# pashtari/factorizer

Measured on AMD Instinct MI355X. Metric: volumes/sec fwd+bwd, Swin Factorizer 128^3, higher is better.
Workload: dtype f32

## Files before the change

factorizer_amd/_native.py:

```python
from __future__ import annotations

import ctypes
import os
import threading

import torch

_HERE = os.path.dirname(os.path.abspath(__file__))
LIB_PATH = os.environ.get("FZ_LIB_PATH") or os.path.join(_HERE, "libfactorizer_hip.so")

FZ_OK = 0
FZ_E_UNSUPPORTED = -2
ABI_VERSION = 7
SOLVER_ID = {"mu": 0, "hals": 1, "cd": 2, "smu": 3}
STORE_F32, STORE_BF16 = 0, 1
PRODUCTS_DEFAULT, PRODUCTS_SPLIT_BF16, PRODUCTS_FP32_MFMA = 0, 1, 2
_products = threading.local()


def products() -> int:
    return getattr(_products, "value", PRODUCTS_DEFAULT)


class use_products:
# ... 89 lines not shown
            h.fz_abi_version.restype = ctypes.c_int
            abi = int(h.fz_abi_version())
        except AttributeError:
            abi = None
        if abi != ABI_VERSION:
            raise NativeError(f"{LIB_PATH} has ABI revision {abi}, this binding is written against {ABI_VERSION} "
                              "(include/factorizer_hip.h: FZ_ABI_VERSION): rebuild with `python -m factorizer_amd.build`")
        for name, (args, res) in _SIGS.items():
            fn = getattr(h, name)
            fn.argtypes = args
            fn.restype = res
        _lib = h
    return _lib


def launch_count() -> int:
    return int(lib().fz_launch_count())


def check(rc: int, what: str):
    if rc != FZ_OK:
        msg = lib().fz_last_error_string().decode()
        raise NativeError(f"{what} failed (code {rc}): {msg}")


def stream_ptr(t: torch.Tensor) -> int:
    return torch.cuda.current_stream(t.device).cuda_stream


def ptr(t):
    return None if t is None else t.data_ptr()


def shifts_array(shifts):
    flat = [int(v) for s in shifts for v in s]
    return (_i * len(flat))(*flat)


_fp = _c.POINTER(_c.c_float)


class GemmDesc(_c.Structure):
    _fields_ = [("x", _vp * 4), ("nsrc", _i), ("src_mode", _i), ("c0", _i), ("Cin", _i), ("Vin", _i64),
                ("Di", _i), ("Hi", _i), ("Wi", _i), ("w", _vp), ("w_t", _i), ("ldw", _i), ("M", _i), ("K", _i),
                ("bias", _vp), ("ln", _i), ("ln_g", _vp), ("ln_b", _vp), ("ln_eps", _f), ("stats_out", _vp),
                ("bact", _i), ("bmul", _vp), ("bmul_kind", _i), ("eact", _i), ("res", _vp), ("emul", _vp), ("emul_kind", _i), ("y", _vp),
                ("Ncol", _i64), ("Ho", _i), ("Wo", _i), ("B", _i), ("loader", _i), ("epilogue", _i), ("lnb_x", _vp), ("lnb_stats", _vp), ("lnb_g", _vp),
                ("lnb_gadd", _vp), ("lnb_part", _vp), ("act_dtype", _i), ("products", _i), ("tune", _i)]


class MlpDesc(_c.Structure):
    _fields_ = [("mode", _i), ("inp", _vp), ("w1", _vp), ("w2", _vp), ("b1", _vp), ("b2", _vp), ("ln_g", _vp),
                ("ln_b", _vp), ("ln_eps", _f), ("stats", _vp), ("z1", _vp), ("gz1", _vp), ("x1", _vp), ("out", _vp),
                ("part", _vp), ("B", _i), ("C", _i), ("H", _i), ("V", _i64), ("act_dtype", _i), ("wpart", _vp),
                ("gw1", _vp), ("gb1", _vp), ("gw2", _vp), ("gb2", _vp), ("gln", _vp), ("glp", _vp), ("products", _i),
                ("pre_in", _vp), ("pre_w", _vp), ("pre_b", _vp), ("pre_res", _vp), ("pre_out", _vp),
                ("post_w", _vp), ("post_b", _vp), ("post_out", _vp), ("post_m", _i)]


class MlpDropout(_c.Structure):
    _fields_ = [("m0", _vp), ("m1", _vp), ("m2", _vp), ("s0", _f), ("s1", _f), ("s2", _f)]


class BlockPrologue(_c.Structure):
    _fields_ = [("ln_g", _vp), ("ln_b", _vp), ("ln_eps", _f), ("w", _vp), ("t", _vp), ("stats", _vp)]


class GemmDwDesc(_c.Structure):
    _fields_ = [("g", _vp), ("q", _vp), ("w", _vp), ("ln", _i), ("stats", _vp), ("ln_g", _vp), ("ln_b", _vp), ("gadd", _vp),
                ("y", _vp), ("gln", _vp), ("wpart", _vp), ("gw", _vp), ("gb", _vp), ("B", _i), ("C", _i), ("V", _i64),
                ("act_dtype", _i), ("ldgw", _i), ("ldw", _i), ("drop_m", _vp), ("drop_s", _f)]


class WgradDesc(_c.Structure):
    _fields_ = [("p", _vp), ("M", _i), ("pmul", _vp), ("pmul_kind", _i), ("q", _vp * 4), ("nsrc", _i),
                ("src_mode", _i), ("c0", _i), ("Cin", _i), ("K", _i), ("Vq", _i64), ("D", _i), ("H", _i),
                ("W", _i), ("N", _i64), ("Ho", _i), ("Wo", _i), ("stats", _vp), ("qact", _i), ("ln_g", _vp),
                ("ln_b", _vp), ("gw", _vp), ("gbias", _vp), ("accumulate", _i), ("B", _i), ("loader", _i),
                ("act_dtype", _i), ("products", _i)]


class VolGeom(_c.Structure):
    _fields_ = [("nd", _i), ("size", _i * 3), ("start", _i * 3), ("end", _i * 3), ("pad", _i * 3), ("out", _i * 3)]


class RespaceGeom(_c.Structure):
    _fields_ = [("nd", _i), ("src_size", _i * 3), ("src_axis", _i * 3), ("flip", _i * 3), ("res_size", _i * 3), ("pad", _i * 3),
                ("out", _i * 3), ("orig_size", _i * 3), ("box_start", _i * 3), ("scale", _c.c_double * 3),
                ("inv_scale", _c.c_double * 3)]


_SIGS.update({
    "fz_gcorr_supported": ([_i] * 5, _i),
    "fz_gcorr": ([_vp] * 5 + [_i] * 11 + [_f, _vp], _i),
    "fz_gcorr_wgrad_workspace_bytes": ([_i] * 10, _i64),
    "fz_gcorr_wgrad": ([_vp] * 4 + [_i] * 11 + [_vp], _i),
    "fz_gcorr_act": ([_vp] * 5 + [_i] * 11 + [_f, _i, _vp], _i),
    "fz_gcorr_wgrad_act": ([_vp] * 4 + [_i] * 12 + [_vp], _i),
    "fz_gcorr_mu_bwd": ([_vp] * 8 + [_i] * 11 + [_f, _i, _vp], _i),
    "fz_gnmf_supported": ([_i, _i64, _i, _i, _i], _i),
    "fz_gnmf_workspace_bytes": ([_i64, _i, _i64, _i, _i, _i], _i64),
    "fz_gnmf_launches": ([_i, _i, _i], _i),
    "fz_gnmf_fwd": ([_vp] * 6 + [_i64, _i, _i64, _i, _i, _i, _f, _vp, _vp], _i),
    "fz_gnmf_bwd": ([_vp] * 7 + [_i64, _i, _i64, _i, _i, _i, _i, _f, _vp, _vp], _i),
    "fz_gnmfx_supported": ([_i, _i64, _i, _i, _i], _i),
    "fz_gnmfx_workspace_bytes": ([_i64, _i, _i64, _i, _i, _i], _i64),
    "fz_gnmfx_launches": ([_i, _i64, _i, _i, _i, _i], _i),
    "fz_gnmfx_fwd": ([_vp] * 6 + [_i64, _i, _i64, _i, _i, _i, _f, _vp, _vp], _i),
    "fz_gnmfx_bwd": ([_vp] * 7 + [_i64, _i, _i64, _i, _i, _i, _i, _f, _vp, _vp], _i),
    "fz_nmf_cf_supported": ([_i] * 11, _i),
    "fz_nmf_cf_fwd": ([_vp] * 4 + [_i] * 5 + [_c.POINTER(_i)] + [_i] * 5 + [_f, _i, _vp], _i),
    "fz_nmf_cf_bwd": ([_vp] * 5 + [_i] * 5 + [_c.POINTER(_i)] + [_i] * 7 + [_f, _i, _vp], _i),
    "fz_nmf_cf_factors_supported": ([_i] * 12 + [_c.POINTER(_i)], _i),
    "fz_nmf_cf_fwd_store_factors": ([_vp] * 5 + [_i] * 5 + [_c.POINTER(_i)] + [_i] * 3 + [_f, _i, _vp], _i),
    "fz_nmf_cf_fwd_from_factors": ([_vp] * 6 + [_i] * 5 + [_c.POINTER(_i)] * 2 + [_i] * 4 + [_f, _i, _vp], _i),
    "fz_nmf_cf_bwd_factors_supported": ([_i] * 14 + [_c.POINTER(_i)], _i),
    "fz_nmf_cf_bwd_store_factors": ([_vp] * 5 + [_i] * 5 + [_c.POINTER(_i)] + [_i] * 3 + [_f, _i, _vp], _i),
    "fz_nmf_cf_bwd_from_factors": ([_vp] * 6 + [_i] * 5 + [_c.POINTER(_i)] * 2 + [_i] * 3 + [_f, _i, _vp], _i),
    "fz_nmf_pcf_supported": ([_i] * 11, _i),
    "fz_nmf_pcf_fwd": ([_vp] * 4 + [_i] * 8 + [_c.POINTER(_i)] + [_i] * 5 + [_f, _i, _vp], _i),
    "fz_nmf_pcf_bwd": ([_vp] * 5 + [_i] * 8 + [_c.POINTER(_i)] + [_i] * 7 + [_f, _i, _vp], _i),
    "fz_nmf_pcf_bwd_prefers_separate": ([_i] * 4, _i),
    "fz_act_add": ([_vp, _vp, _i64, _i, _vp], _i),
    "fz_mlp_pre_supported": ([_i, _i, _i64, _i], _i),
    "fz_mlp_drop_supported": ([_i, _i, _i64, _i], _i),
    "fz_mlp_chain_drop": ([_c.POINTER(MlpDesc), _c.POINTER(MlpDropout), _vp], _i),
    "fz_conv3_prologue_supported": ([_i] * 4, _i),
    "fz_conv3_fwd2": ([_vp] * 4 + [_i] * 8 + [_c.POINTER(BlockPrologue), _vp], _i),
    "fz_upcat2": ([_vp, _vp, _vp, _i, _vp, _vp, _vp] + [_i] * 7 + [_c.POINTER(BlockPrologue), _vp], _i),
    "fz_gemm": ([_c.POINTER(GemmDesc), _vp], _i),
    "fz_gemm_plan": ([_c.POINTER(GemmDesc), _c.c_char_p, _i], _i),
    "fz_gemm_bx_enable": ([_i], _i),
    "fz_gemm_lnbwd_partials": ([_c.POINTER(GemmDesc)], _i64),
    "fz_reduce_rows": ([_vp, _i64, _i, _vp, _vp, _vp], _i),
    "fz_adamw_step": ([_vp, _vp, _vp, _vp, _i64, _f, _f, _f, _f, _f, _i, _f, _vp], _i),
    "fz_sw_gather": ([_vp, _vp] + [_i] * 10 + [_vp], _i),
    "fz_sw_accumulate": ([_vp] * 6 + [_f] + [_i] * 10 + [_vp], _i),
    "fz_sw_finalize": ([_vp, _vp, _i, _i64, _vp], _i),
    "fz_sw_gather2": ([_vp, _vp] + [_i] * 11 + [_vp], _i),
    "fz_sw_accumulate2": ([_vp] * 6 + [_f] + [_i] * 11 + [_vp], _i),
    "fz_sw_finalize2": ([_vp, _vp, _vp, _i, _i64, _i, _vp], _i),
    "fz_mlp_supported": ([_i, _i, _i64], _i),
    "fz_mlp_partials": ([_i, _i64], _i64),
    "fz_mlp_wgrad_rows": ([_i, _i64], _i),
    "fz_gemm_dw_rows": ([_i, _i64], _i),
    "fz_gemm_dw_workspace_bytes": ([_i, _i64], _i64),
    "fz_gemm_dw": ([_c.POINTER(GemmDwDesc), _vp], _i),
    "fz_mlp_wgrad_workspace_bytes": ([_i, _i64], _i64),
    "fz_mlp_chain": ([_c.POINTER(MlpDesc), _vp], _i),
    "fz_head_bwd_rows": ([], _i),
    "fz_head_bwd_workspace_bytes": ([], _i64),
    "fz_head_bwd": ([_vp, _vp, _vp, _vp, _vp, _i, _i, _i, _i64, _i, _vp], _i),
    "fz_head_fwd": ([_vp, _vp, _vp, _vp, _i, _i, _i, _i64, _i, _vp], _i),
    "fz_upcat_supported": ([_i] * 5, _i),
    "fz_upcat_compose": ([_vp, _vp, _i, _vp, _vp, _vp, _vp, _vp, _i, _i, _i, _vp], _i),
    "fz_upcat_wgrads": ([_vp, _vp, _vp, _i, _vp, _vp, _vp, _vp, _i, _vp, _i, _i, _i, _vp], _i),
    "fz_upcat": ([_vp, _vp, _vp, _i, _vp, _vp, _vp] + [_i] * 7 + [_vp], _i),
    "fz_upcat_bwd_supported": ([_i] * 6, _i),
    "fz_upcat_bwd_workspace_bytes": ([_i] * 4, _i64),
    "fz_upcat_bwd": ([_vp, _vp, _vp, _vp, _i, _vp, _vp, _vp, _vp, _vp, _i, _vp, _vp] + [_i] * 7 + [_vp], _i),
    "fz_wgrad": ([_c.POINTER(WgradDesc), _vp, _vp], _i),
    "fz_wgrad_group": ([_c.POINTER(_c.POINTER(WgradDesc)), _c.POINTER(_vp), _i, _vp], _i),
    "fz_wgrad_workspace_bytes": ([_c.POINTER(WgradDesc)], _i64),
    "fz_conv3_fwd": ([_vp] * 4 + [_i] * 8 + [_vp], _i),
    "fz_conv3_wgrad_chunks": ([_i] * 4, _i),
    "fz_conv3_wgrad_partials": ([_vp] * 4 + [_i] * 8 + [_vp], _i),
    "fz_chunk_reduce": ([_vp, _i, _i64, _vp, _i, _vp], _i),
    "fz_chunk_reduce_ld": ([_vp, _i, _i64, _i64, _vp, _i, _vp], _i),
    "fz_finish_defer": ([_i], _i),
    "fz_finish_pending": ([], _i),
    "fz_finish_flush": ([_vp], _i),
    "fz_finish_flush_all": ([_vp], _i),
    "fz_dice_bce_chunks": ([_i64], _i),
    "fz_dice_bce_sums": ([_vp, _vp, _vp, _i, _i64, _vp], _i),
    "fz_dice_bce_grad": ([_vp, _vp, _vp, _vp, _i, _i64, _f, _f, _vp, _vp], _i),
    "fz_dice_ce_sums": ([_vp, _vp, _vp, _i, _i, _i64, _vp], _i),
    "fz_dice_ce_grad": ([_vp, _vp, _vp, _vp, _i, _i, _i64, _f, _f, _vp, _vp], _i),
    "fz_dice_ce_finish": ([_vp, _i, _i, _i64, _f, _vp, _vp, _vp], _i),
    "fz_dice_bce_ds_sums": ([_vp, _vp, _vp, _i] + [_i] * 6 + [_i, _vp], _i),
    "fz_dice_bce_ds_grad": ([_vp, _vp, _vp, _vp, _i] + [_i] * 6 + [_i, _f, _f, _vp, _vp], _i),
    "fz_dice_ce_ds_sums": ([_vp, _vp, _vp, _i, _i] + [_i] * 6 + [_i, _vp], _i),
    "fz_dice_ce_ds_grad": ([_vp, _vp, _vp, _vp, _i, _i] + [_i] * 6 + [_i, _f, _f, _vp, _vp], _i),
    "fz_rowsum_chunks": ([_i64], _i),
    "fz_rowsum": ([_vp, _vp, _vp, _i, _i, _i64, _i, _vp], _i),
    "fz_ln_fwd": ([_vp] * 5 + [_i, _i, _i64, _f, _i, _vp], _i),
    "fz_ln_bwd": ([_vp] * 8 + [_i, _i, _i64, _i, _vp], _i),
    "fz_ln_bwd_workspace_bytes": ([_i], _i64),
    "fz_ln_bwd_workspace_bytes2": ([_i, _i, _i64], _i64),
    "fz_dropout_bits_words": ([_i, _i, _i64], _i64),
    "fz_dropout_keep_bits": ([_vp, _i, _i, _i, _i64, _f, _vp, _vp], _i),
    "fz_dropout_apply": ([_i, _vp, _f, _vp, _vp, _vp, _i, _i, _i64, _i, _vp], _i),
    "fz_seg_counts_chunks": ([_i64], _i),
    "fz_seg_counts_workspace_bytes": ([_i, _i64], _i64),
    "fz_seg_counts": ([_vp, _i, _vp, _i, _f, _vp, _vp, _vp, _i, _i64, _vp], _i),
    "fz_mask_edges": ([_vp, _vp, _vp, _i, _i, _i, _i, _i, _vp], _i),
    "fz_edge_min_dist2_splits": ([_i64, _i64], _i),
    "fz_edge_min_dist2_workspace_bytes": ([_i64, _i64], _i64),
    "fz_edge_min_dist2": ([_vp, _i64, _vp, _i64, _f, _f, _f, _vp, _vp, _vp], _i),
    "fz_aug_record_floats": ([], _i),
    "fz_aug_resample": ([_vp, _vp, _i, _i, _vp, _vp, _i, _vp, _vp, _vp] + [_i] * 6 + [_vp], _i),
    "fz_aug_smooth": ([_vp, _vp, _i, _i, _vp, _vp] + [_i] * 6 + [_vp], _i),
    "fz_aug_noise_field": ([_vp, _vp, _i, _i, _i64, _vp], _i),
    "fz_aug_source_words": ([], _i),
    "fz_aug_crop_resample": ([_vp, _vp, _i, _i, _vp, _i, _vp, _vp, _vp] + [_i] * 6 + [_vp], _i),
    "fz_vol_kind_ok": ([_i, _i], _i),
    "fz_vol_bbox": ([_vp, _i, _i, _i, _i, _i, _i, _vp, _vp], _i),
    "fz_vol_workspace_bytes": ([_i, _c.POINTER(VolGeom)], _i64),
    "fz_vol_stats": ([_vp, _i, _i, _c.POINTER(VolGeom), _i, _i, _vp, _vp], _i),
    "fz_vol_write": ([_vp, _i, _vp, _i, _i, _vp, _i, _i, _c.POINTER(_i), _c.POINTER(_i), _i, _vp, _c.POINTER(VolGeom), _i, _i,
                      _vp, _vp, _vp, _vp], _i),
    "fz_vol_restore": ([_c.POINTER(_vp), _i, _i, _i, _c.POINTER(VolGeom), _f, _c.POINTER(_c.c_ubyte), _vp, _vp], _i),
    "fz_vol_respace": ([_vp, _i, _vp, _i, _vp, _i, _vp, _c.POINTER(RespaceGeom), _i, _vp], _i),
    "fz_vol_unspace": ([_c.POINTER(_vp), _i, _i, _i, _c.POINTER(RespaceGeom), _i, _i, _f, _vp, _vp], _i),
    "fz_inorm_one_pass_max": ([], _i),
    "fz_inorm_chunks": ([_i64], _i),
    "fz_inorm_workspace_bytes": ([_i64, _i64], _i64),
    "fz_inorm_fwd": ([_vp] * 5 + [_i64, _i, _i64, _c.c_double, _i, _vp, _vp], _i),
    "fz_inorm_bwd": ([_vp] * 7 + [_i64, _i, _i64, _i, _vp, _vp], _i),
})
SEG_F32, SEG_BF16, SEG_U8 = 0, 1, 2
VOL_F32, VOL_BF16, VOL_U8, VOL_I16 = 0, 1, 2, 3
VOL_IMAGE_IN, VOL_IMAGE_OUT, VOL_LABEL_IN, VOL_LOGITS = 0, 1, 2, 3
RESPACE_BILINEAR, RESPACE_NEAREST = 0, 1
DROP_RES, DROP_GELU, DROP_GELU_BWD = 0, 1, 2
```

factorizer_amd/blocks.py:

```python
from __future__ import annotations

import os

import torch
from torch import nn

from . import functional as Fn
from . import pointwise as PW
from .layers import MLP, LayerNorm, Linear
from .matricize import Matricize, SWMatricize
from .nmf import NMF, MatrixFactorization, RandomInit
from .utils import partialize


def _env_int(name, default):
    v = os.environ.get(name)
    if v is None:
        return default
    try:
        return int(v, 0)
    except ValueError:
        raise ValueError(f"{name}={v!r}: expected an integer") from None


_UP_FUSED = _env_int("FZ_UP_FUSED", 1) != 0
_UP_FUSED_MIN = _env_int("FZ_UP_FUSED_MIN", 1 << 18)


class FactMixer(nn.Module):

    def __init__(self, in_channels, out_channels, spatial_size,
                 reshape=(Matricize, {"num_heads": 1, "grid_size": 1}), act=nn.ReLU, factorize=NMF,
                 dropout=0.0, **kwargs):
        super().__init__()
        self.in_proj = Linear(in_channels, out_channels, bias=False)
        self.reshape = partialize(reshape)((None, out_channels, *spatial_size))
        self.act = partialize(act)()
        self.reshaped_size = self.reshape.output_size[2:]
        self.factorize = partialize(factorize)(self.reshaped_size, **kwargs)
        self.out_proj = Linear(in_channels, out_channels, True)
        self.dropout = nn.Dropout(dropout)

    def forward(self, x):
        out = self.in_proj(x)
        out = self.reshape(out)
        out = self.act(out)
        out = self.factorize(out)
        out = self.reshape.inverse_forward(out)
        out = self.out_proj(out)
        if self.dropout.p > 0:
            out = self.dropout(out)
        return out


class FactorizerBlock(nn.Module):

    def __init__(self, channels, spatial_size, norm=LayerNorm, dropout=0.0, mlp_ratio=2, **kwargs):
        super().__init__()
        self.norm1 = partialize(norm)(channels)
        self.fact = FactMixer(channels, channels, spatial_size, dropout=dropout, **kwargs)
        self.norm2 = partialize(norm)(channels)
        self.mlp = MLP(channels, ratio=mlp_ratio, dropout=dropout)

    def _fusable(self, x) -> bool:
        f, m = self.fact, self.mlp
        if not (x.is_cuda and x.numel() and x.dtype in (torch.float32, torch.bfloat16) and PW._vox(x) % 4 == 0
                and x.shape[1] % 2 == 0):
            return False
        if any(p.dtype != torch.float32 for p in self.parameters()):
            return False
        if not (isinstance(self.norm1, LayerNorm) and isinstance(self.norm2, LayerNorm)
                and self.norm1.norm.elementwise_affine and self.norm2.norm.elementwise_affine
                and self.norm1.norm.bias is not None and self.norm2.norm.bias is not None):
            return False
        if not (isinstance(f.act, nn.ReLU) and isinstance(f.in_proj, Linear) and isinstance(f.out_proj, Linear)):
            return False
        blk = m.block
        if not (len(blk) == 5 and isinstance(blk[1], nn.GELU) and blk[1].approximate == "none"
                and blk[0].linear.weight.shape[0] % 2 == 0):
            return False
        drops = (f.dropout, blk[2], blk[4])
        if self.training and any(d.p > 0 for d in drops):
            return all(type(d) is nn.Dropout and 0 <= d.p < 1 for d in drops)
        return True

    def _dropout_ps(self):
        ps = (float(self.fact.dropout.p), float(self.mlp.block[2].p), float(self.mlp.block[4].p))
        return ps if self.training and any(p > 0 for p in ps) else None

    def _modular_native_cfg(self, x) -> bool:
        f = self.fact
        mf = f.factorize
        if not (isinstance(f.reshape, SWMatricize) and isinstance(mf, MatrixFactorization)):
            return False
        t_like = x.new_empty((1, *f.reshape.output_size[1:]))
        return mf._native_solver(t_like) is not None and not mf._wide and len(f.reshape.geometry.spatial) <= 3

    def _core_cfg(self):
        f = self.fact
        mf = f.factorize
        if not (isinstance(f.reshape, SWMatricize) and isinstance(mf, MatrixFactorization)):
            return None
        sid = getattr(mf.solver, "native_id", None)
        if sid is None or not isinstance(mf.init, RandomInit) or mf.solver.factor != (0, 1) or mf.verbose:
            return None
        G = min(max(mf.num_grad_steps, 0), mf.num_iters)
        geo = f.reshape.geometry
        if tuple(mf.size) != (8, geo.P) or not Fn.nmf_core_supported(geo, mf.rank, mf.num_iters, G):
            return None
        return G, sid

    def prologue_params(self, like):
        f, blk = self.fact, self.mlp.block
        n1 = self.norm1.norm
        if not (like.is_cuda and like.shape[1] == 32 and self._fusable(like) and self._core_cfg() is not None
                and f.in_proj.linear.bias is None and blk[0].linear.bias is not None and blk[3].linear.bias is not None
                and f.out_proj.linear.bias is not None and f.in_proj.linear.weight.dtype == torch.float32
                and n1.weight is not None and n1.bias is not None
                and not (self.norm1._forward_hooks or f.in_proj._forward_hooks or f._forward_hooks)):
            return None
        return n1.weight, n1.bias, n1.eps, f.in_proj.linear.weight

    def forward(self, x):
        if self._fusable(x):
            f, blk = self.fact, self.mlp.block
            n1, n2 = self.norm1.norm, self.norm2.norm
            core = self._core_cfg()
            mf = f.factorize
            nat = core is not None or self._modular_native_cfg(x)
            drop = self._dropout_ps()
            one_node = nat and f.in_proj.linear.bias is None and blk[0].linear.bias is not None \
                and blk[3].linear.bias is not None and f.out_proj.linear.bias is not None
            if one_node:
                if core is not None:
                    G, sid = core
                else:
                    G, sid = min(max(mf.num_grad_steps, 0), mf.num_iters), mf.solver.native_id
                cfg = dict(geo=f.reshape.geometry, T=mf.num_iters, G=G, solver=sid, nmf_eps=mf.solver.eps,
                           eps1=n1.eps, eps2=n2.eps, core=core is not None)
                if drop is not None:
                    cfg["drop"] = drop
                args = (x, n1.weight, n1.bias, f.in_proj.linear.weight, mf.init.u0, mf.init.v0,
                        f.out_proj.linear.weight, f.out_proj.linear.bias, n2.weight, n2.bias,
                        blk[0].linear.weight, blk[0].linear.bias, blk[3].linear.weight, blk[3].linear.bias, cfg)
                pre = PW.BlockPrologue.take(x) if core is not None else None
                t_pre, st_pre = pre if pre is not None else (None, None)
                slot = PW.head_fusion_slot()
                if slot is not None and slot.block is self and core is not None and drop is None:
                    hw, hb = slot.head_params
                    C, Hd = x.shape[1], blk[0].linear.weight.shape[0]
                    if PW.block_head_fusable(C, Hd, x[0, 0].numel(), hw, x):
                        y, raw = PW.FactorizerBlockFn.apply(*args, hw, hb, t_pre, st_pre)
                        slot.logits = PW.HeadOfBlockFn.apply(y, hw, hb, raw)
                        return y
                return PW.FactorizerBlockFn.apply(*args, None, None, t_pre, st_pre)
            if drop is None:
                return self._per_layer(x)
        x = x + self.fact(self.norm1(x))
        x = x + self.mlp(self.norm2(x))
        return x

    def _per_layer(self, x):
        f, blk = self.fact, self.mlp.block
        n1, n2 = self.norm1.norm, self.norm2.norm
        t = PW.ln_linear(x, n1.weight, n1.bias, n1.eps, f.in_proj.linear.weight, f.in_proj.linear.bias, "relu")
        a = f.reshape.inverse_forward(f.factorize(f.reshape(t)))
        x = PW.act_linear_res(a, f.out_proj.linear.weight, f.out_proj.linear.bias, x, "none")
        z = PW.ln_linear(x, n2.weight, n2.bias, n2.eps, blk[0].linear.weight, blk[0].linear.bias, "none")
        return PW.act_linear_res(z, blk[3].linear.weight, blk[3].linear.bias, x, "gelu")


class FactorizerStage(nn.Module):

    def __init__(self, in_channels, out_channels, spatial_size, depth=1,
                 adapter=(Linear, {"bias": False}), pos_embed=nn.Identity, dropout=0.0, **subblocks):
        super().__init__()
        if in_channels != out_channels:
            self.adapter = partialize(adapter)(in_channels, out_channels)
        self.pos_embed = partialize(pos_embed)(out_channels, spatial_size)
        if len(list(self.pos_embed.parameters())) > 0:
            self.pos_drop = nn.Dropout(dropout)
        self.blocks = nn.ModuleList()
        for _ in range(depth):
            self.blocks.append(FactorizerBlock(out_channels, spatial_size, **subblocks))

    def forward_pair(self, skip, up):
        if hasattr(self, "adapter") and isinstance(self.adapter, Linear):
            out = PW.cat_linear(skip, up, self.adapter.linear.weight, self.adapter.linear.bias)
            return self._after_adapter(out)
        return self.forward(torch.cat([skip, up], dim=1))

    def forward_up_pair(self, skip, deep, upsample):
        from . import convs as _convs
        ok = (hasattr(self, "adapter") and isinstance(self.adapter, Linear) and type(upsample) is _convs.ConvTranspose3d
              and upsample.native_ok(deep) and skip.is_cuda and skip.dtype == deep.dtype and skip.dim() == 5
              and skip.shape[1] % 16 == 0 and upsample.out_channels % 16 == 0 and deep.shape[1] % 16 == 0
              and self.adapter.linear.weight.dtype == torch.float32
              and tuple(skip.shape[2:]) == tuple(2 * d for d in deep.shape[2:])
              and self.adapter.linear.weight.shape[1] == skip.shape[1] + upsample.out_channels
              and _UP_FUSED and skip.shape[0] * skip[0, 0].numel() >= _UP_FUSED_MIN
              and not (upsample._forward_hooks or upsample._forward_pre_hooks
                       or self.adapter._forward_hooks or self.adapter._forward_pre_hooks
                       or self.adapter.linear._forward_hooks or self.adapter.linear._forward_pre_hooks))
        if not ok:
            return None
        pro = self._first_block_prologue(skip) if PW.upcat_prologue_ok(skip, deep, upsample.weight, self.adapter.linear.weight) else None
        if pro is not None:
            out, t, st = PW.up_cat_linear(skip, deep, upsample.weight, upsample.bias, self.adapter.linear.weight, self.adapter.linear.bias, pro)
            with PW.BlockPrologue(out, t, st):
                return self._after_adapter(out)
        out = PW.up_cat_linear(skip, deep, upsample.weight, upsample.bias, self.adapter.linear.weight, self.adapter.linear.bias)
        return self._after_adapter(out)

    def _first_block_prologue(self, like):
        if not isinstance(self.pos_embed, nn.Identity) or (hasattr(self, "pos_drop") and self.pos_drop.p > 0) or len(self.blocks) == 0:
            return None
        blk = self.blocks[0]
        if type(blk).__name__ != "FactorizerBlock" or blk._forward_hooks or blk._forward_pre_hooks:
            return None
        return blk.prologue_params(like)

    def forward(self, x):
        out = self.adapter(x) if hasattr(self, "adapter") else x
        return self._after_adapter(out)

    def _after_adapter(self, out):
        if not isinstance(self.pos_embed, nn.Identity):
            out = self.pos_embed(out)
        if hasattr(self, "pos_drop") and self.pos_drop.p > 0:
            out = self.pos_drop(out)
        for blk in self.blocks:
            out = blk(out)
        return out
```

factorizer_amd/csrc/headbwd.hip:

```cpp
#include "gemm_common.h"

namespace fz {

constexpr int kHeadRow = 4 * 33;

template <int M, typename AT>
__global__ __launch_bounds__(256, 2) void head_bwd_kernel(const AT* __restrict__ gy, const AT* __restrict__ x,
                                                          const float* __restrict__ w, AT* __restrict__ gx,
                                                          float* __restrict__ part, int B, int64_t V, int Mr) {
  __shared__ float red[4][kHeadRow];
  __shared__ float sW[M * 32];
  const int lane = threadIdx.x & 63, wave = threadIdx.x >> 6;
  for (int i = threadIdx.x; i < M * 32; i += 256) sW[i] = i < Mr * 32 ? w[i] : 0.f;
  __syncthreads();
  float gw[M][32];
  float gb[M];
#pragma unroll
  for (int m = 0; m < M; ++m) {
    gb[m] = 0.f;
#pragma unroll
    for (int c = 0; c < 32; ++c) gw[m][c] = 0.f;
  }
  const unsigned quads = (unsigned)(V / 4), total = quads * (unsigned)B;
  for (unsigned i = blockIdx.x * 256u + threadIdx.x; i < total; i += gridDim.x * 256u) {
    asm volatile("" ::: "memory");
    const int b = (int)(i / quads);
    const int64_t v = (int64_t)(i - (unsigned)b * quads) * 4;
    float g4[M][4];
#pragma unroll
    for (int m = 0; m < M; ++m) {
      vload<4>(gy + ((int64_t)b * Mr + (m < Mr ? m : Mr - 1)) * V + v, g4[m]);
#pragma unroll
      for (int e = 0; e < 4; ++e) {
        g4[m][e] = m < Mr ? g4[m][e] : 0.f;
        gb[m] += g4[m][e];
      }
    }
    const AT* xb = x + (int64_t)b * 32 * V + v;
    AT* ob = gx + (int64_t)b * 32 * V + v;
    constexpr int CB = 4;
#pragma unroll
    for (int c0 = 0; c0 < 32; c0 += CB) {
      float xv[CB][4];
#pragma unroll
      for (int u = 0; u < CB; ++u) vload<4>(xb + (int64_t)(c0 + u) * V, xv[u]);
      __builtin_amdgcn_sched_barrier(0);
#pragma unroll
      for (int u = 0; u < CB; ++u) {
        const int c = c0 + u;
        float o[4];
#pragma unroll
        for (int e = 0; e < 4; ++e) {
          float t = sW[c] * g4[0][e];
#pragma unroll
          for (int m = 1; m < M; ++m) t += sW[m * 32 + c] * g4[m][e];
          o[e] = t;
        }
        vstore<4>(ob + (int64_t)c * V, o);
#pragma unroll
        for (int m = 0; m < M; ++m)
          gw[m][c] += (g4[m][0] * xv[u][0] + g4[m][1] * xv[u][1]) + (g4[m][2] * xv[u][2] + g4[m][3] * xv[u][3]);
      }
    }
  }
#pragma unroll
  for (int m = 0; m < M; ++m) {
#pragma unroll
    for (int c0 = 0; c0 < 32; c0 += 8) {
      float t[8];
#pragma unroll
      for (int u = 0; u < 8; ++u) t[u] = gw[m][c0 + u];
      wave_sum8(t, lane);
      if (lane == 0) {
#pragma unroll
        for (int u = 0; u < 8; ++u) red[wave][m * 32 + c0 + u] = t[u];
      }
    }
    const float s = wave_sum(gb[m]);
    if (lane == 0) red[wave][128 + m] = s;
  }
  __syncthreads();
  for (int e = threadIdx.x; e < kHeadRow; e += 256) {
    const bool used = (e < 128) ? (e >> 5) < Mr : (e - 128) < Mr;
    part[(int64_t)blockIdx.x * kHeadRow + e] = used ? (red[0][e] + red[1][e]) + (red[2][e] + red[3][e]) : 0.f;
  }
}

template <int M, typename AT>
__global__ __launch_bounds__(256) void head_fwd_kernel(const AT* __restrict__ x, const float* __restrict__ w,
                                                       const float* __restrict__ bias, AT* __restrict__ y, int B, int64_t V, int Mr) {
  __shared__ float sW[M * 32];
  __shared__ float sB[M];
  for (int i = threadIdx.x; i < M * 32; i += 256) sW[i] = i < Mr * 32 ? w[i] : 0.f;
  if (threadIdx.x < M) sB[threadIdx.x] = (bias != nullptr && (int)threadIdx.x < Mr) ? bias[threadIdx.x] : 0.f;
  __syncthreads();
  const unsigned quads = (unsigned)(V / 4), stride = gridDim.x * 256u;
  unsigned first = blockIdx.x * 256u + threadIdx.x;
  int b = (int)(first / quads);
  unsigned qd = first - (unsigned)b * quads;
  for (; b < B; qd += stride) {
    while (qd >= quads) { qd -= quads; ++b; }
    if (b >= B) break;
    asm volatile("" ::: "memory");
    const int64_t v = (int64_t)qd * 4;
    const AT* xb = x + (int64_t)b * 32 * V + v;
    float acc[M][4];
#pragma unroll
    for (int m = 0; m < M; ++m)
#pragma unroll
      for (int e = 0; e < 4; ++e) acc[m][e] = sB[m];
    constexpr int CB = 8;
#pragma unroll
    for (int c0 = 0; c0 < 32; c0 += CB) {
      float xv[CB][4];
#pragma unroll
      for (int u = 0; u < CB; ++u) vload<4>(xb + (int64_t)(c0 + u) * V, xv[u]);
#pragma unroll
      for (int u = 0; u < CB; ++u)
#pragma unroll
        for (int m = 0; m < M; ++m) {
          const float wv = sW[m * 32 + c0 + u];
#pragma unroll
          for (int e = 0; e < 4; ++e) acc[m][e] += wv * xv[u][e];
        }
    }
#pragma unroll
    for (int m = 0; m < M; ++m)
      if (m < Mr) vstore<4>(y + ((int64_t)b * Mr + m) * V + v, acc[m]);
  }
}

}

using namespace fz;

extern "C" int fz_head_bwd_rows(void) { return 512; }
extern "C" int64_t fz_head_bwd_workspace_bytes(void) { return (int64_t)fz_head_bwd_rows() * kHeadRow * (int64_t)sizeof(float); }

template <typename AT>
static int head_bwd_launch(const void* gy, const void* x, const float* w, void* gx, float* part, int B, int M, int64_t V,
                           hipStream_t st) {
  const unsigned grid = (unsigned)fz_head_bwd_rows();
#define FZ_HEAD(MM) hipLaunchKernelGGL((head_bwd_kernel<MM, AT>), dim3(grid), dim3(256), 0, st, (const AT*)gy, (const AT*)x, w, (AT*)gx, part, B, V, M)
  if (M <= 2) FZ_HEAD(2); else FZ_HEAD(4);
#undef FZ_HEAD
  FZ_LAUNCH_CHECK();
  return FZ_OK;
}

extern "C" int fz_head_bwd(const void* gy, const void* x, const float* w, void* gx, float* part, int B, int M, int C, int64_t V,
                           int act_dtype, fz_stream_t stream) {
  if (!gy || !x || !w || !gx || !part) return fail(FZ_E_ARG, "fz_head_bwd: null pointer");
  if (C != 32 || M < 1 || M > 4 || V < 4 || V % 4 != 0) return fail(FZ_E_UNSUPPORTED, "fz_head_bwd: needs C == 32, 1 <= M <= 4, V % 4 == 0");
  if ((int64_t)B * (V / 4) >= ((int64_t)1 << 31)) return fail(FZ_E_UNSUPPORTED, "fz_head_bwd: 2^31 or more voxel quads");
  if (B <= 0) return B == 0 ? FZ_OK : fail(FZ_E_SHAPE, "fz_head_bwd: negative batch");
  if (act_dtype == FZ_STORE_F32) return head_bwd_launch<float>(gy, x, w, gx, part, B, M, V, (hipStream_t)stream);
  if (act_dtype == FZ_STORE_BF16) return head_bwd_launch<bf16>(gy, x, w, gx, part, B, M, V, (hipStream_t)stream);
  return fail(FZ_E_ARG, "fz_head_bwd: act_dtype must be FZ_STORE_F32 or FZ_STORE_BF16");
}

template <typename AT>
static int head_fwd_launch(const void* x, const float* w, const float* bias, void* y, int B, int M, int64_t V, hipStream_t st) {
  const unsigned grid = 512u;
  if (gemm_plan_only()) return gemm_plan_form("head m%d grid=%ux1", M <= 2 ? 2 : 4, grid);
#define FZ_HEADF(MM) hipLaunchKernelGGL((head_fwd_kernel<MM, AT>), dim3(grid), dim3(256), 0, st, (const AT*)x, w, bias, (AT*)y, B, V, M)
  if (M <= 2) FZ_HEADF(2); else FZ_HEADF(4);
#undef FZ_HEADF
  FZ_LAUNCH_CHECK();
  return FZ_OK;
}

extern "C" int fz_head_fwd(const void* x, const float* w, const float* bias, void* y, int B, int M, int C, int64_t V, int act_dtype,
                           fz_stream_t stream) {
  if (!x || !w || !y) return fail(FZ_E_ARG, "fz_head_fwd: null pointer");
  if (C != 32 || M < 1 || M > 4 || V < 4 || V % 4 != 0) return fail(FZ_E_UNSUPPORTED, "fz_head_fwd: needs C == 32, 1 <= M <= 4, V % 4 == 0");
  if (V / 4 >= ((int64_t)1 << 31) || (int64_t)B * (V / 4) >= ((int64_t)1 << 31)) return fail(FZ_E_UNSUPPORTED, "fz_head_fwd: 2^31 or more voxel quads");
  if (B <= 0) return B == 0 ? FZ_OK : fail(FZ_E_SHAPE, "fz_head_fwd: negative batch");
  if (act_dtype == FZ_STORE_F32) return head_fwd_launch<float>(x, w, bias, y, B, M, V, (hipStream_t)stream);
  if (act_dtype == FZ_STORE_BF16) return head_fwd_launch<bf16>(x, w, bias, y, B, M, V, (hipStream_t)stream);
  return fail(FZ_E_ARG, "fz_head_fwd: act_dtype must be FZ_STORE_F32 or FZ_STORE_BF16");
}
```

factorizer_amd/csrc/mlp_chain.h:

```cpp
#pragma once
#include "gemm_bx.h"
#include "gemm_shared.h"

namespace fz {

template <typename AT>
struct ChainArgsT {
  const float* wB;
  int wB_t, ldwB;
  const float* biasB;
  AT* side;
  const AT* preA;
  const float* preW;
  const float* preB;
  const AT* preRes;
  AT* preOut;
  const float* postW;
  const float* postB;
  AT* postOut;
  int postM;
  int stagger;
};

__device__ __forceinline__ void chain_stagger(int stagger) {
  const int n = stagger * (int)(blockIdx.x >> 8);
  for (int i = 0; i < n; ++i) __builtin_amdgcn_s_sleep(127);
}

constexpr int chain64_lds_floats(bool p512, bool pre) {
  return 2 * (p512 ? 12288 : 8192) + (pre ? 6144 + 64 : 0) + 128 + 64 + (p512 ? 2 : 1) * 512;
}
constexpr int chain_wg_lds_floats(bool bx, bool wgb) {
  return 2 * (bx ? 3072 : 2048) + 32 + 256 + 4 * (wgb ? 3072 : 48 * kTS);
}

template <typename... KArgs, typename... Args>
static int launch_lds(void (*kern)(KArgs...), dim3 grid, dim3 block, int lds_floats, hipStream_t st, Args... args) {
  const int lds = lds_floats * (int)sizeof(float);
  FZ_HIP_OK(hipFuncSetAttribute(reinterpret_cast<const void*>(kern), hipFuncAttributeMaxDynamicSharedMemorySize, lds));
  hipLaunchKernelGGL(kern, grid, block, lds, st, args...);
  FZ_LAUNCH_CHECK();
  return FZ_OK;
}

static int knob_chain64_p512() { return knob_pos(FZ_KNOB("FZ_CHAIN64_P512"), 1) == 1; }
static int knob_chain_fwd_bx() { const auto& k = FZ_KNOB("FZ_CHAIN_FWD_BX"); return k.set ? k.val : 1; }
static int knob_mlp_wgs(int dflt) { return knob_pos(FZ_KNOB("FZ_MLP_WGS"), dflt); }

template <typename AT>
int chain32_launch(const fz_mlp_desc* d, const fz_mlp_dropout* drop, const GemmArgsT<AT>& a, const ChainArgsT<AT>& c, fz_stream_t stream);
template <typename AT>
int chain64_launch(const fz_mlp_desc* d, const GemmArgsT<AT>& a, const ChainArgsT<AT>& c, fz_stream_t stream);
template <typename AT>
int chain_wg_launch(const fz_mlp_desc* d, const GemmArgsT<AT>& a, const ChainArgsT<AT>& c, fz_stream_t stream);

}
```

factorizer_amd/csrc/mlp_chain.hip:

```cpp
#include "mlp_chain.h"

using namespace fz;

static int mlp_nacc() { return 2; }

extern "C" int64_t fz_mlp_partials(int B, int64_t V) {
  const int64_t tw = 128 * mlp_nacc();
  return ((V + tw - 1) / tw) * (int64_t)B;
}

extern "C" int fz_mlp_pre_supported(int C, int H, int64_t V, int products) {
  if (!(V > 0 && (V % 4) == 0 && V <= ((int64_t)1 << 27) && products_split(products))) return 0;
  if (C == 32 && H == 64) return knob_chain_fwd_bx() ? 1 : 0;
  if (C == 64 && H == 128) return (((V + 255) / 256) % 2 == 0 && knob_chain64_p512()) ? 1 : 0;
  return 0;
}

extern "C" int fz_mlp_supported(int C, int H, int64_t V) {
  const bool shape = (C == 32 && (H == 64 || H == 128)) || (C == 64 && H == 128);
  return (shape && V > 0 && (V % 4) == 0 && V <= ((int64_t)1 << 27)) ? 1 : 0;
}

extern "C" int fz_mlp_drop_supported(int C, int H, int64_t V, int products) {
  return (C == 32 && H == 64 && fz_mlp_supported(C, H, V) && fz_mlp_pre_supported(C, H, V, products) && products_split(products)
          && knob_chain_fwd_bx()) ? 1 : 0;
}

template <typename AT>
static void forward_args(const fz_mlp_desc* d, int ldw, int ldwB, GemmArgsT<AT>& a, ChainArgsT<AT>& c) {
  a.w = d->w1; a.w_t = 0; a.ldw = ldw;
  a.bias = d->b1; a.ln = 1; a.ln_g = d->ln_g; a.ln_b = d->ln_b; a.ln_eps = d->ln_eps; a.stats_out = d->stats;
  a.res = (const AT*)d->in; a.y = (AT*)d->out;
  c.wB = d->w2; c.wB_t = 0; c.ldwB = ldwB; c.biasB = d->b2; c.side = (AT*)d->z1;
  if (d->pre_in) {
    c.preA = (const AT*)d->pre_in; c.preW = d->pre_w; c.preB = d->pre_b; c.preRes = (const AT*)d->pre_res; c.preOut = (AT*)d->pre_out;
    if (d->C == 64) a.res = (const AT*)d->pre_out;
    else { c.postW = d->post_w; c.postB = d->post_b; c.postOut = (AT*)d->post_out; c.postM = d->post_m; }
  }
}
template <typename AT>
static void backward_args(const fz_mlp_desc* d, int ldw, int ldwB, AT* side, GemmArgsT<AT>& a, ChainArgsT<AT>& c) {
  a.w = d->w2; a.w_t = 1; a.ldw = ldw;
  a.emul = (const AT*)d->z1; a.y = (AT*)d->out;
  a.lnb_x = (const AT*)d->x1; a.lnb_stats = d->stats; a.lnb_g = d->ln_g; a.lnb_gadd = (const AT*)d->in; a.lnb_part = d->part;
  c.wB = d->w1; c.wB_t = 1; c.ldwB = ldwB; c.side = side;
}

static int mlp_check(const fz_mlp_desc* d, const fz_mlp_dropout* dd, bool drop) {
  if (!fz_mlp_supported(d->C, d->H, d->V)) return fail(FZ_E_UNSUPPORTED, "fz_mlp_chain: needs (C, H) in {(32, 64), (32, 128), (64, 128)}, V % 4 == 0");
  if (drop) {
    if (!fz_mlp_drop_supported(d->C, d->H, d->V, d->products) || d->mode != 0 || !d->pre_in)
      return fail(FZ_E_UNSUPPORTED, "fz_mlp_chain: dropout needs (C, H) = (32, 64), split-bf16 products, mode 0 with pre_in (fz_mlp_drop_supported)");
    if (!drop_scale_ok(dd->m0, dd->s0) || !drop_scale_ok(dd->m1, dd->s1) || !drop_scale_ok(dd->m2, dd->s2))
      return fail(FZ_E_ARG, "fz_mlp_chain: a dropout scale 1 / (1 - p) must be >= 1 and finite");
  }
  if (d->C == 64 && d->mode == 2) return fail(FZ_E_UNSUPPORTED, "fz_mlp_chain: the fused weight gradients need C == 32, H == 64");
  if (d->B < 0) return fail(FZ_E_SHAPE, "fz_mlp_chain: negative batch");
  const bool pre = d->pre_in != nullptr;
  if (pre && (d->mode != 0 || !d->pre_w || !d->pre_res || !d->pre_out))
    return fail(FZ_E_ARG, "fz_mlp_chain: pre_in needs mode 0, pre_w, pre_res, pre_out (see fz_mlp_pre_supported)");
  if (pre && !fz_mlp_pre_supported(d->C, d->H, d->V, d->products))
    return fail(FZ_E_UNSUPPORTED, "fz_mlp_chain: the fused out-projection runs on split-bf16 products only (fz_mlp_pre_supported)");
  if (d->post_out && (!pre || d->C != 32 || !d->post_w || d->post_m < 1 || d->post_m > 4))
    return fail(FZ_E_ARG, "fz_mlp_chain: post_out needs pre_in, C == 32, post_w and 1 <= post_m <= 4");
  if ((!d->in && !pre) || !d->w1 || !d->w2 || !d->out || !d->z1 || !d->stats)
    return fail(FZ_E_ARG, "fz_mlp_chain: null pointer");
  if (d->mode == 0 && (!d->ln_g || !d->ln_b)) return fail(FZ_E_ARG, "fz_mlp_chain: forward needs the LayerNorm affine");
  if (d->mode == 1 && (!d->gz1 || !d->x1 || !d->ln_g || !d->part)) return fail(FZ_E_ARG, "fz_mlp_chain: backward needs gz1, x1, gamma, part");
  if (d->mode == 2 && (!d->x1 || !d->ln_g || !d->ln_b || !d->gln || !d->wpart || !d->gw1 || !d->gb1 || !d->gw2 || !d->gb2))
    return fail(FZ_E_ARG, "fz_mlp_chain: backward with weight gradients needs x1, gamma, beta, gln, wpart, gw1, gb1, gw2, gb2");
  if (d->mode == 2 && d->H == 128 && !d->glp) return fail(FZ_E_ARG, "fz_mlp_chain: the fused weight gradients at H == 128 need the glp buffer");
  if (d->mode < 0 || d->mode > 2) return fail(FZ_E_ARG, "fz_mlp_chain: bad mode");
  return FZ_OK;
}

template <typename AT>
static int mlp_launch(const fz_mlp_desc* d, const fz_mlp_dropout* dd, fz_stream_t stream) {
  const bool drop = dd && (dd->m0 || dd->m1 || dd->m2);
  const int rc = mlp_check(d, dd, drop);
  if (rc != FZ_OK) return rc;
  if (d->B == 0) {
    if (d->mode == 2) {
      hipStream_t s0 = (hipStream_t)stream;
      FZ_HIP_OK(hipMemsetAsync(d->gw1, 0, sizeof(float) * d->H * 32, s0));
      FZ_HIP_OK(hipMemsetAsync(d->gw2, 0, sizeof(float) * d->H * 32, s0));
      FZ_HIP_OK(hipMemsetAsync(d->gb1, 0, sizeof(float) * d->H, s0));
      FZ_HIP_OK(hipMemsetAsync(d->gb2, 0, sizeof(float) * 32, s0));
      FZ_HIP_OK(hipMemsetAsync(d->gln, 0, sizeof(float) * 64, s0));
    }
    return FZ_OK;
  }
  GemmArgsT<AT> a = {};
  ChainArgsT<AT> c = {};
  a.x[0] = (const AT*)d->in; a.nsrc = 1; a.c0 = d->C; a.Cin = d->C; a.Vin = d->V; a.M = d->H; a.K = d->C; a.Ncol = d->V; a.B = d->B;
  if (d->mode == 0) forward_args(d, d->C, d->H, a, c);
  else backward_args(d, d->H, d->C, d->mode == 1 ? (AT*)d->gz1 : (AT*)nullptr, a, c);
  if (d->C == 64) return chain64_launch(d, a, c, stream);
  if (d->mode == 2) return chain_wg_launch(d, a, c, stream);
  return chain32_launch(d, drop ? dd : nullptr, a, c, stream);
}

extern "C" int fz_mlp_chain(const fz_mlp_desc* d, fz_stream_t stream) {
  if (!d) return fail(FZ_E_ARG, "fz_mlp_chain: null descriptor");
  if (d->act_dtype == FZ_STORE_F32) return mlp_launch<float>(d, nullptr, stream);
  if (d->act_dtype == FZ_STORE_BF16) return mlp_launch<bf16>(d, nullptr, stream);
  return fail(FZ_E_ARG, "fz_mlp_chain: act_dtype must be FZ_STORE_F32 or FZ_STORE_BF16");
}

extern "C" int fz_mlp_chain_drop(const fz_mlp_desc* d, const fz_mlp_dropout* drop, fz_stream_t stream) {
  if (!d || !drop) return fail(FZ_E_ARG, "fz_mlp_chain_drop: null descriptor");
  if (d->act_dtype == FZ_STORE_F32) return mlp_launch<float>(d, drop, stream);
  if (d->act_dtype == FZ_STORE_BF16) return mlp_launch<bf16>(d, drop, stream);
  return fail(FZ_E_ARG, "fz_mlp_chain_drop: act_dtype must be FZ_STORE_F32 or FZ_STORE_BF16");
}
```

factorizer_amd/csrc/mlp_chain_wg.hip:

```cpp
#include "mlp_chain.h"
#include "finish.h"

namespace fz {


__device__ __forceinline__ void gelu_both(float x, float& g, float& dg) {
  const float ax = fabsf(x) * 0.70710678118654752f;
  const float E = __expf(-0.5f * x * x);
  const float t = __builtin_amdgcn_rcpf(1.0f + 0.3275911f * ax);
  const float poly = t * (0.254829592f + t * (-0.284496736f + t * (1.421413741f + t * (-1.453152027f + t * 1.061405429f))));
  const float r = 1.0f - poly * E;
  const float cdf = 0.5f * (1.0f + __builtin_copysignf(r, x));
  g = x * cdf;
  dg = cdf + x * (0.3989422804014327f * E);
}

typedef float f32x2 __attribute__((ext_vector_type(2)));
template <bool SEL = false>
__device__ __forceinline__ void gelu_both2(const float (&x)[2], float (&g)[2], float (&dg)[2]) {
  const f32x2 xv = {x[0], x[1]};
  const f32x2 ax = f32x2{fabsf(x[0]), fabsf(x[1])} * 0.70710678118654752f;
  const f32x2 xx = (xv * -0.5f) * xv;
  const f32x2 E = {__expf(xx[0]), __expf(xx[1])};
  const f32x2 den = ax * 0.3275911f + 1.0f;
  const f32x2 t = {__builtin_amdgcn_rcpf(den[0]), __builtin_amdgcn_rcpf(den[1])};
  const f32x2 poly = t * (t * (t * (t * (t * 1.061405429f + -1.453152027f) + 1.421413741f) + -0.284496736f) + 0.254829592f);
  const f32x2 r = 1.0f - poly * E;
  f32x2 rs;
  if constexpr (SEL) rs = f32x2{x[0] < 0.f ? -r[0] : r[0], x[1] < 0.f ? -r[1] : r[1]};
  else rs = f32x2{__builtin_copysignf(r[0], x[0]), __builtin_copysignf(r[1], x[1])};
  const f32x2 cdf = (rs + 1.0f) * 0.5f;
  const f32x2 gv = xv * cdf;
  const f32x2 dv = cdf + xv * (E * 0.3989422804014327f);
  g[0] = gv[0]; g[1] = gv[1];
  dg[0] = dv[0]; dg[1] = dv[1];
}

typedef __bf16 wg2 __attribute__((ext_vector_type(2)));
__device__ __forceinline__ void wg_split2(float x0, float x1, unsigned& hi, unsigned& lo) {
  fx2 v = {x0, x1};
  const wg2 a = __builtin_convertvector(v, wg2);
  v = v - __builtin_convertvector(a, fx2);
  const wg2 b = __builtin_convertvector(v, wg2);
  hi = __builtin_bit_cast(unsigned, a);
  lo = __builtin_bit_cast(unsigned, b);
}
__device__ __forceinline__ float2 wg_join2(unsigned hi, unsigned lo) {
  return make_float2(__uint_as_float(hi << 16) + __uint_as_float(lo << 16),
                     __uint_as_float(hi & 0xffff0000u) + __uint_as_float(lo & 0xffff0000u));
}
__device__ __forceinline__ float wg_sum8(const bx8& hi, const bx8& lo, float acc) {
  const wg2 one = {(__bf16)1.0f, (__bf16)1.0f};
  struct Q { wg2 p[4]; };
  const Q h = __builtin_bit_cast(Q, hi), l = __builtin_bit_cast(Q, lo);
#pragma unroll
  for (int i = 0; i < 4; ++i) {
    acc = __builtin_amdgcn_fdot2_f32_bf16(l.p[i], one, acc, false);
    acc = __builtin_amdgcn_fdot2_f32_bf16(h.p[i], one, acc, false);
  }
  return acc;
}
__device__ __forceinline__ void wg_mfma3(f32x4& acc, const bx8& ah, const bx8& al, const bx8& bh, const bx8& bl) {
  acc = __builtin_amdgcn_mfma_f32_16x16x32_bf16(al, bh, acc, 0, 0, 0);
  acc = __builtin_amdgcn_mfma_f32_16x16x32_bf16(ah, bl, acc, 0, 0, 0);
  acc = __builtin_amdgcn_mfma_f32_16x16x32_bf16(ah, bh, acc, 0, 0, 0);
}

template <typename AT, int HALVES = 1, int HALF = 0, bool BX = false, bool WGB = false>
__global__ __launch_bounds__(256, 2) void gemm_chain_bwd_wg_kernel(GemmArgsT<AT> p, ChainArgsT<AT> c, int ntiles, float* wpart,
                                                                   float* glp) {
  static_assert(!WGB || (BX && HALVES == 1), "WGB: the one-launch split-bf16 form");
  constexpr int NACC = 2, HB = 2, HID = 64 * HALVES, N1 = BX ? 3072 : 16 * HB * 64;
  constexpr int NTA = BxTerms<AT>::A, NTB = bx_terms_b<AT>(BXPRO_GELU);
  constexpr bool WGF = WGB && sizeof(AT) == 4;
  constexpr int half = HALF;
  constexpr int hoff = 64 * HALF;
  constexpr bool last = HALF == HALVES - 1;
  constexpr int kWave = WGB ? 3072 : 48 * kTS;
  extern __shared__ __attribute__((aligned(16))) float fz_lds_cw[];
  float* As1 = fz_lds_cw;
  float* As2 = As1 + N1;
  float* tB = As2 + N1;
  float* red = tB + 32;
  float* R = red + 256;
  static_assert(2 * N1 + 32 + 256 + 4 * kWave == chain_wg_lds_floats(BX, WGB), "the launcher's dynamic LDS ends where this carve-up does");
  const int lane = threadIdx.x & 63, wave = threadIdx.x >> 6;
  const int j = lane & 31, h = lane >> 5;
  const int l16 = lane & 15, k4 = lane >> 4;
  float* Bf = R + wave * kWave;
  float* T = Bf + 32 * kTS;
  char* const PL = reinterpret_cast<char*>(Bf);
  constexpr int kGL = 4096, kTH = 8192, kTL = 10240;
  unsigned wop[4], wac[4], rd[2];
  if constexpr (WGB) {
    const unsigned ob = (unsigned)h * 128u + ((((unsigned)j >> 2) ^ (unsigned)h) << 4) + ((unsigned)j & 3u) * 4u;
    const unsigned ab = (unsigned)h * 512u + ((((unsigned)j >> 2) ^ (4u * (unsigned)h)) << 4) + ((unsigned)j & 3u) * 4u;
#pragma unroll
    for (int q = 0; q < 4; ++q) { wop[q] = ob ^ ((unsigned)q << 5); wac[q] = ab ^ ((unsigned)q << 4); }
    rd[0] = (unsigned)l16 * 128u + ((((unsigned)k4) ^ ((unsigned)l16 & 7u)) << 4);
    rd[1] = rd[0] ^ 64u;
  }
  const int tiles_per_sample = (int)((p.Ncol + 128 * NACC - 1) / (128 * NACC));
  chain_stagger(c.stagger);

  if constexpr (BX) {
    for (int it = threadIdx.x; it < 512; it += 256) {
      float wv[8];
      const int l = it & 63;
      __bf16* dst;
      if (it < 256) {
        const int rb = (it >> 6) & 1, g = it >> 7;
#pragma unroll
        for (int e = 0; e < 8; ++e) wv[e] = weight_at(p, hoff + rb * 32 + (l & 31), 2 * (8 * g + e) + (l >> 5));
        dst = reinterpret_cast<__bf16*>(As1) + ((g * HB + rb) * NTA * 64 + l) * 8;
      } else {
        const int g = (it - 256) >> 6;
#pragma unroll
        for (int e = 0; e < 8; ++e) {
          const int s2 = 8 * g + e, r = s2 & 15, rb = s2 >> 4;
          const int k = hoff + rb * 32 + (r & 3) + 8 * (r >> 2) + 4 * (l >> 5), m = l & 31;
          wv[e] = c.wB_t ? c.wB[(int64_t)k * c.ldwB + m] : c.wB[(int64_t)m * c.ldwB + k];
        }
        dst = reinterpret_cast<__bf16*>(As2) + (g * NTA * 64 + l) * 8;
      }
      bx8 t3[NTA];
      bx_split<NTA>(wv, t3);
#pragma unroll
      for (int i = 0; i < NTA; ++i) *reinterpret_cast<bx8*>(dst + i * 64 * 8) = t3[i];
    }
  } else {
  for (int base = threadIdx.x; base < 2 * N1; base += 256 * 8) {
    float tmp[8];
#pragma unroll
    for (int uu = 0; uu < 8; ++uu) {
      const int idx = base + uu * 256;
      float wv;
      if (idx < N1) {
        const int l = idx & 63, rb = (idx >> 6) % HB, a = idx / (64 * HB);
        wv = weight_at(p, hoff + rb * 32 + (l & 31), 2 * a + (l >> 5));
      } else {
        const int i2 = idx - N1;
        const int l = i2 & 63, s2 = i2 >> 6;
        const int r = s2 & 15, rb = s2 >> 4;
        const int k = hoff + rb * 32 + (r & 3) + 8 * (r >> 2) + 4 * (l >> 5), m = l & 31;
        wv = c.wB_t ? c.wB[(int64_t)k * c.ldwB + m] : c.wB[(int64_t)m * c.ldwB + k];
      }
      tmp[uu] = wv;
    }
#pragma unroll
    for (int uu = 0; uu < 8; ++uu) {
      const int idx = base + uu * 256;
      if (idx < N1) As1[idx] = tmp[uu]; else As2[idx - N1] = tmp[uu];
    }
  }
  }
  if (threadIdx.x < 32) tB[threadIdx.x] = p.lnb_g[threadIdx.x];

  f32x4 dW2[2][4], dW1[4][2];
#pragma unroll
  for (int a = 0; a < 2; ++a)
#pragma unroll
    for (int b4 = 0; b4 < 4; ++b4)
#pragma unroll
      for (int v = 0; v < 4; ++v) { dW2[a][b4][v] = 0.f; dW1[b4][a][v] = 0.f; }
  float db2[2] = {0.f, 0.f}, db1[4] = {0.f, 0.f, 0.f, 0.f};
  float gln = 0.f;

  int tile = blockIdx.x;
  float bv[16][NACC];
  auto fetch_tile = [&](int t) {
    const int bt = t / tiles_per_sample;
    const int64_t ct = ((int64_t)(t % tiles_per_sample) * 4 + wave) * (32 * NACC) + NACC * j;
    const unsigned lo = (unsigned)h * (unsigned)p.Ncol + (unsigned)(ct < p.Ncol ? ct : 0);
    const AT* xb = p.x[0] + (int64_t)bt * 32 * p.Ncol;
#pragma unroll
    for (int s = 0; s < 16; ++s) vload<NACC>(xb + (int64_t)(2 * s) * p.Ncol + lo, bv[s]);
  };
  fetch_tile(tile);
  __syncthreads();

  for (; tile < ntiles; tile += gridDim.x) {
    asm volatile("" ::: "memory");
    const int b = tile / tiles_per_sample;
    const int64_t col_off = ((int64_t)(tile % tiles_per_sample) * 4 + wave) * (32 * NACC) + NACC * j;
    const bool col_ok = col_off < p.Ncol;
    const int64_t nc = col_ok ? col_off : 0;
    const unsigned lane_row = (unsigned)(4 * h) * (unsigned)p.Ncol + (unsigned)nc;
    const unsigned lane_par = (unsigned)h * (unsigned)p.Ncol + (unsigned)nc;
    const int64_t sample = (int64_t)b * 32 * p.Ncol;

    constexpr bool ZSEL = HALVES == 2;
    auto zs = [&](float v) { return (ZSEL && !col_ok) ? 0.f : v; };
    if (!ZSEL && __builtin_amdgcn_ballot_w64(!col_ok) != 0) {
#pragma unroll
      for (int s = 0; s < 16; ++s) { bv[s][0] = col_ok ? bv[s][0] : 0.f; bv[s][1] = col_ok ? bv[s][1] : 0.f; }
    }
    if constexpr (!WGB) {
#pragma unroll
    for (int s = 0; s < 16; ++s)
      *reinterpret_cast<float2*>(Bf + (2 * s + h) * kTS + 2 * j) = make_float2(zs(bv[s][0]), zs(bv[s][1]));
    }

    float e[2][8][NACC];
    auto fetch_z1 = [&](int g8, float (&dst)[8][NACC]) {
#pragma unroll
      for (int i = 0; i < 8; ++i) {
        const int rr = g8 * 8 + i, rb = rr >> 4, r = rr & 15;
        const int rbase = hoff + rb * 32 + (r & 3) + 8 * (r >> 2);
        vload<NACC>(p.emul + ((int64_t)b * HID + rbase) * p.Ncol + lane_row, dst[i]);
      }
    };
    float xv[2][8][NACC];
    auto fetch_x1 = [&](int hf, float (&dst)[8][NACC]) {
#pragma unroll
      for (int s8 = 0; s8 < 8; ++s8) vload<NACC>(p.lnb_x + sample + (int64_t)(2 * (hf * 8 + s8)) * p.Ncol + lane_par, dst[s8]);
    };
    const float* sp = p.lnb_stats + (int64_t)b * 2 * p.Ncol;
    float mu[NACC], rs[NACC];
    vload<NACC>(sp + nc, mu);
    vload<NACC>(sp + p.Ncol + nc, rs);
    fetch_z1(0, e[0]);

    f32x16 acc1[HB][NACC];
#pragma unroll
    for (int rb = 0; rb < HB; ++rb)
#pragma unroll
      for (int q = 0; q < NACC; ++q)
#pragma unroll
        for (int r = 0; r < 16; ++r) acc1[rb][q][r] = 0.f;
    if constexpr (BX) {
#pragma unroll
      for (int g = 0; g < 2; ++g) {
        bx8 bop[NACC][NTB];
#pragma unroll
        for (int q = 0; q < NACC; ++q) {
          float x8[8];
#pragma unroll
          for (int e = 0; e < 8; ++e) x8[e] = bv[8 * g + e][q];
          bx_split<NTB>(x8, bop[q]);
        }
        if constexpr (WGB) {
          static_assert(!WGB || NTB >= 2, "two levels of the column operand");
#pragma unroll
          for (int e = 0; e < 8; ++e) {
            const int s = 8 * g + e;
            const wg2 ph = {bop[0][0][e], bop[1][0][e]};
            const wg2 pl = {bop[0][NTB >= 2 ? 1 : 0][e], bop[1][NTB >= 2 ? 1 : 0][e]};
            *reinterpret_cast<wg2*>(PL + wop[s & 3] + s * 256) = ph;
            *reinterpret_cast<wg2*>(PL + kGL + wop[s & 3] + s * 256) = pl;
          }
        }
#pragma unroll
        for (int rb = 0; rb < HB; ++rb) {
          bx8 aop[NTA];
#pragma unroll
          for (int i = 0; i < NTA; ++i)
            aop[i] = *reinterpret_cast<const bx8*>(reinterpret_cast<const __bf16*>(As1) + (((g * HB + rb) * NTA + i) * 64 + lane) * 8);
#pragma unroll
          for (int q = 0; q < NACC; ++q) bx_mfma<NTA, NTB>(acc1[rb][q], aop, bop[q]);
        }
        __builtin_amdgcn_sched_barrier(0);
      }
    } else {
#pragma unroll
    for (int s = 0; s < 16; ++s)
#pragma unroll
      for (int rb = 0; rb < HB; ++rb) {
        const float av = As1[(s * HB + rb) * 64 + lane];
#pragma unroll
        for (int q = 0; q < NACC; ++q) acc1[rb][q] = __builtin_amdgcn_mfma_f32_32x32x2f32(av, bv[s][q], acc1[rb][q], 0, 0, 0);
        if (rb == HB - 1 && (s & 1) == 1) __builtin_amdgcn_sched_barrier(0);
      }
    }

#pragma unroll
    for (int g8 = 0; g8 < 4; ++g8) {
      asm volatile("" ::: "memory");
      if (g8 < 3) fetch_z1(g8 + 1, e[(g8 + 1) & 1]);
      else { fetch_x1(0, xv[0]); fetch_x1(1, xv[1]); }
#pragma unroll
      for (int i = 0; i < 8; ++i) {
        const int rr = g8 * 8 + i, rb = rr >> 4, r = rr & 15;
        float gl[NACC], dg[NACC];
        gelu_both2<HALVES == 2>(e[g8 & 1][i], gl, dg);
#pragma unroll
        for (int q = 0; q < NACC; ++q) {
          float gz = acc1[rb][q][r] * dg[q];
          asm volatile("" : "+v"(gz));
          acc1[rb][q][r] = gz;
        }
        if constexpr (WGB) {
          unsigned ph, pl;
          wg_split2(gl[0], gl[1], ph, pl);
          *reinterpret_cast<unsigned*>(PL + kTH + wac[i & 3] + (i & 3) * 128 + (i >> 2) * 1024) = ph;
          *reinterpret_cast<unsigned*>(PL + kTL + wac[i & 3] + (i & 3) * 128 + (i >> 2) * 1024) = pl;
        } else {
        const int loc = (i & 3) + 8 * (i >> 2) + 4 * h;
        *reinterpret_cast<float2*>(T + loc * kTS + 2 * j) = make_float2(zs(gl[0]), zs(gl[1]));
        }
      }
      if constexpr (WGB) {
#pragma unroll
        for (int ks = 0; ks < 2; ++ks) {
          const bx8 bh = *reinterpret_cast<const bx8*>(PL + kTH + rd[ks]);
          const bx8 bl = *reinterpret_cast<const bx8*>(PL + kTL + rd[ks]);
          const bx8 a0h = *reinterpret_cast<const bx8*>(PL + rd[ks]);
          const bx8 a0l = *reinterpret_cast<const bx8*>(PL + kGL + rd[ks]);
          const bx8 a1h = *reinterpret_cast<const bx8*>(PL + 2048 + rd[ks]);
          const bx8 a1l = *reinterpret_cast<const bx8*>(PL + kGL + 2048 + rd[ks]);
          wg_mfma3(dW2[0][g8], a0h, a0l, bh, bl);
          wg_mfma3(dW2[1][g8], a1h, a1l, bh, bl);
          if (g8 == 0) {
            db2[0] = wg_sum8(a0h, a0l, db2[0]);
            db2[1] = wg_sum8(a1h, a1l, db2[1]);
            asm volatile("" : "+v"(db2[0]), "+v"(db2[1]));
          }
          __builtin_amdgcn_sched_barrier(0);
        }
      } else {
#pragma unroll
      for (int tc = 0; tc < 2; ++tc) {
        float bq[8], a0[8], a1[8];
#pragma unroll
        for (int u = 0; u < 8; ++u) {
          const int t = tc * 8 + u;
          bq[u] = T[l16 * kTS + 4 * t + k4];
          a0[u] = Bf[l16 * kTS + 4 * t + k4];
          a1[u] = Bf[(16 + l16) * kTS + 4 * t + k4];
        }
#pragma unroll
        for (int u = 0; u < 8; ++u) {
          dW2[0][g8] = __builtin_amdgcn_mfma_f32_16x16x4f32(a0[u], bq[u], dW2[0][g8], 0, 0, 0);
          dW2[1][g8] = __builtin_amdgcn_mfma_f32_16x16x4f32(a1[u], bq[u], dW2[1][g8], 0, 0, 0);
        }
        if (g8 == 0 && (HALVES == 1 || half == 0)) {
          db2[0] += ((a0[0] + a0[1]) + (a0[2] + a0[3])) + ((a0[4] + a0[5]) + (a0[6] + a0[7]));
          db2[1] += ((a1[0] + a1[1]) + (a1[2] + a1[3])) + ((a1[4] + a1[5]) + (a1[6] + a1[7]));
          asm volatile("" : "+v"(db2[0]), "+v"(db2[1]));
        }
        __builtin_amdgcn_sched_barrier(0);
      }
      }
      __builtin_amdgcn_sched_barrier(0);
    }

    float ga[2][8][NACC];
    if (last && BX) {
#pragma unroll
      for (int r = 0; r < 16; ++r) {
        float2 gv;
        if constexpr (WGB)
          gv = wg_join2(*reinterpret_cast<const unsigned*>(PL + wac[r & 3] + (r & 3) * 128 + (r >> 2) * 1024),
                        *reinterpret_cast<const unsigned*>(PL + kGL + wac[r & 3] + (r & 3) * 128 + (r >> 2) * 1024));
        else
          gv = *reinterpret_cast<const float2*>(Bf + ((r & 3) + 8 * (r >> 2) + 4 * h) * kTS + 2 * j);
        ga[r >> 3][r & 7][0] = gv.x; ga[r >> 3][r & 7][1] = gv.y;
      }
      asm volatile("" ::: "memory");
    }

#pragma unroll
    for (int hf = 0; hf < 2; ++hf)
#pragma unroll
      for (int s8 = 0; s8 < 8; ++s8) {
        if constexpr (WGB) {
          const int s = hf * 8 + s8;
          unsigned ph, pl;
          wg_split2((xv[hf][s8][0] - mu[0]) * rs[0], (xv[hf][s8][1] - mu[1]) * rs[1], ph, pl);
          *reinterpret_cast<unsigned*>(PL + wop[s & 3] + s * 256) = ph;
          *reinterpret_cast<unsigned*>(PL + kGL + wop[s & 3] + s * 256) = pl;
        } else
        *reinterpret_cast<float2*>(Bf + (2 * (hf * 8 + s8) + h) * kTS + 2 * j) =
            make_float2(zs((xv[hf][s8][0] - mu[0]) * rs[0]), zs((xv[hf][s8][1] - mu[1]) * rs[1]));
      }

    f32x16 acc2[NACC];
    if constexpr (WGF) {
#pragma unroll
      for (int q = 0; q < NACC; ++q)
#pragma unroll
        for (int r = 0; r < 16; ++r) acc2[q][r] = 0.f;
    }
#pragma unroll
    for (int g8 = 0; g8 < 4; ++g8) {
      asm volatile("" ::: "memory");
#pragma unroll
      for (int i = 0; i < 8; ++i) {
        const int rr = g8 * 8 + i, rb = rr >> 4, r = rr & 15;
        if constexpr (WGF) {
        } else if constexpr (WGB) {
          unsigned ph, pl;
          wg_split2(acc1[rb][0][r], acc1[rb][1][r], ph, pl);
          *reinterpret_cast<unsigned*>(PL + kTH + wac[i & 3] + (i & 3) * 128 + (i >> 2) * 1024) = ph;
          *reinterpret_cast<unsigned*>(PL + kTL + wac[i & 3] + (i & 3) * 128 + (i >> 2) * 1024) = pl;
        } else {
        const int loc = (i & 3) + 8 * (i >> 2) + 4 * h;
        *reinterpret_cast<float2*>(T + loc * kTS + 2 * j) = make_float2(zs(acc1[rb][0][r]), zs(acc1[rb][1][r]));
        }
      }
      if constexpr (WGB) {
        if constexpr (WGF) {
          bx8 aop[NTA];
#pragma unroll
          for (int i = 0; i < NTA; ++i)
            aop[i] = *reinterpret_cast<const bx8*>(reinterpret_cast<const __bf16*>(As2) + ((g8 * NTA + i) * 64 + lane) * 8);
          bx8 bop[NACC][NTB];
#pragma unroll
          for (int q = 0; q < NACC; ++q) {
            float x8[8];
#pragma unroll
            for (int e = 0; e < 8; ++e) x8[e] = acc1[g8 >> 1][q][8 * (g8 & 1) + e];
            bx_split<NTB>(x8, bop[q]);
            bx_mfma<NTA, NTB>(acc2[q], aop, bop[q]);
          }
#pragma unroll
          for (int i = 0; i < 8; ++i) {
            const wg2 ph = {bop[0][0][i], bop[1][0][i]};
            const wg2 pl = {bop[0][1][i], bop[1][1][i]};
            *reinterpret_cast<wg2*>(PL + kTH + wac[i & 3] + (i & 3) * 128 + (i >> 2) * 1024) = ph;
            *reinterpret_cast<wg2*>(PL + kTL + wac[i & 3] + (i & 3) * 128 + (i >> 2) * 1024) = pl;
          }
        }
#pragma unroll
        for (int ks = 0; ks < 2; ++ks) {
          const bx8 ah = *reinterpret_cast<const bx8*>(PL + kTH + rd[ks]);
          const bx8 al = *reinterpret_cast<const bx8*>(PL + kTL + rd[ks]);
          const bx8 b0h = *reinterpret_cast<const bx8*>(PL + rd[ks]);
          const bx8 b0l = *reinterpret_cast<const bx8*>(PL + kGL + rd[ks]);
          const bx8 b1h = *reinterpret_cast<const bx8*>(PL + 2048 + rd[ks]);
          const bx8 b1l = *reinterpret_cast<const bx8*>(PL + kGL + 2048 + rd[ks]);
          wg_mfma3(dW1[g8][0], ah, al, b0h, b0l);
          wg_mfma3(dW1[g8][1], ah, al, b1h, b1l);
          db1[g8] = wg_sum8(ah, al, db1[g8]);
          asm volatile("" : "+v"(db1[g8]));
          __builtin_amdgcn_sched_barrier(0);
        }
      } else {
#pragma unroll
      for (int tc = 0; tc < 2; ++tc) {
        float aq[8], b0[8], b1[8];
#pragma unroll
        for (int u = 0; u < 8; ++u) {
          const int t = tc * 8 + u;
          aq[u] = T[l16 * kTS + 4 * t + k4];
          b0[u] = Bf[l16 * kTS + 4 * t + k4];
          b1[u] = Bf[(16 + l16) * kTS + 4 * t + k4];
        }
#pragma unroll
        for (int u = 0; u < 8; ++u) {
          dW1[g8][0] = __builtin_amdgcn_mfma_f32_16x16x4f32(aq[u], b0[u], dW1[g8][0], 0, 0, 0);
          dW1[g8][1] = __builtin_amdgcn_mfma_f32_16x16x4f32(aq[u], b1[u], dW1[g8][1], 0, 0, 0);
        }
        db1[g8] += ((aq[0] + aq[1]) + (aq[2] + aq[3])) + ((aq[4] + aq[5]) + (aq[6] + aq[7]));
        asm volatile("" : "+v"(db1[g8]));
        __builtin_amdgcn_sched_barrier(0);
      }
      }
      __builtin_amdgcn_sched_barrier(0);
    }


    if (last && !BX) {
#pragma unroll
      for (int r = 0; r < 16; ++r)
        vload<NACC>(p.lnb_gadd + sample + (int64_t)((r & 3) + 8 * (r >> 2)) * p.Ncol + lane_row, ga[r >> 3][r & 7]);
    }

    if constexpr (WGF) {
    } else if (HALVES == 2 && half == 1) {
#pragma unroll
      for (int r = 0; r < 16; ++r) {
        float v[NACC];
        vload<NACC>(glp + sample + (int64_t)((r & 3) + 8 * (r >> 2)) * p.Ncol + lane_row, v);
        acc2[0][r] = v[0]; acc2[1][r] = v[1];
      }
    } else {
#pragma unroll
      for (int q = 0; q < NACC; ++q)
#pragma unroll
        for (int r = 0; r < 16; ++r) acc2[q][r] = 0.f;
    }
    if constexpr (WGF) {
    } else if constexpr (BX) {
#pragma unroll
      for (int g = 0; g < 4; ++g) {
        bx8 aop[NTA];
#pragma unroll
        for (int i = 0; i < NTA; ++i)
          aop[i] = *reinterpret_cast<const bx8*>(reinterpret_cast<const __bf16*>(As2) + ((g * NTA + i) * 64 + lane) * 8);
#pragma unroll
        for (int q = 0; q < NACC; ++q) {
          float x8[8];
#pragma unroll
          for (int e = 0; e < 8; ++e) x8[e] = acc1[g >> 1][q][8 * (g & 1) + e];
          bx8 bop[NTB];
          bx_split<NTB>(x8, bop);
          bx_mfma<NTA, NTB>(acc2[q], aop, bop);
        }
        __builtin_amdgcn_sched_barrier(0);
      }
    } else {
#pragma unroll
    for (int rb = 0; rb < HB; ++rb)
#pragma unroll
      for (int r = 0; r < 16; ++r) {
        const float av = As2[(rb * 16 + r) * 64 + lane];
#pragma unroll
        for (int q = 0; q < NACC; ++q) acc2[q] = __builtin_amdgcn_mfma_f32_32x32x2f32(av, acc1[rb][q][r], acc2[q], 0, 0, 0);
        if ((r & 3) == 3) __builtin_amdgcn_sched_barrier(0);
      }
    }
    fetch_tile(tile + gridDim.x < ntiles ? tile + gridDim.x : tile);

    if (HALVES == 2 && !last) {
      if (col_ok) {
#pragma unroll
        for (int r = 0; r < 16; ++r) {
          float v[NACC] = {acc2[0][r], acc2[1][r]};
          vstore<NACC>(glp + sample + (int64_t)((r & 3) + 8 * (r >> 2)) * p.Ncol + lane_row, v);
        }
      }
      continue;
    }
    float m1[NACC] = {0.f, 0.f}, m2[NACC] = {0.f, 0.f};
    float xkeep[WGB ? 16 : 1][2];
#pragma unroll
    for (int r = 0; r < 16; ++r) {
      const int row = (r & 3) + 8 * (r >> 2) + 4 * h;
      const float gc = tB[row];
      float2 xh;
      if constexpr (WGB) {
        xh = wg_join2(*reinterpret_cast<const unsigned*>(PL + wac[r & 3] + (r & 3) * 128 + (r >> 2) * 1024),
                      *reinterpret_cast<const unsigned*>(PL + kGL + wac[r & 3] + (r & 3) * 128 + (r >> 2) * 1024));
        xkeep[r][0] = xh.x; xkeep[r][1] = xh.y;
      } else
        xh = *reinterpret_cast<const float2*>(Bf + row * kTS + 2 * j);
      const float a0 = acc2[0][r] * gc, a1 = acc2[1][r] * gc;
      m1[0] += a0; m1[1] += a1;
      m2[0] += a0 * xh.x; m2[1] += a1 * xh.y;
    }
#pragma unroll
    for (int q = 0; q < NACC; ++q) {
      m1[q] = (m1[q] + __shfl_xor(m1[q], 32, 64)) * (1.0f / 32.0f);
      m2[q] = (m2[q] + __shfl_xor(m2[q], 32, 64)) * (1.0f / 32.0f);
    }
#pragma unroll
    for (int r8 = 0; r8 < 2; ++r8) {
      float sgv[8], sbv[8];
#pragma unroll
      for (int i = 0; i < 8; ++i) {
        const int r = r8 * 8 + i;
        const int rbase = (r & 3) + 8 * (r >> 2);
        const int row = rbase + 4 * h;
        const float gc = tB[row];
        float2 xh;
        if constexpr (WGB)
          xh = make_float2(xkeep[r][0], xkeep[r][1]);
        else
          xh = *reinterpret_cast<const float2*>(Bf + row * kTS + 2 * j);
        float v[NACC];
        v[0] = rs[0] * (acc2[0][r] * gc - m1[0] - xh.x * m2[0]) + ga[r8][i][0];
        v[1] = rs[1] * (acc2[1][r] * gc - m1[1] - xh.y * m2[1]) + ga[r8][i][1];
        if (col_ok) vstore<NACC>(p.y + sample + (int64_t)rbase * p.Ncol + lane_row, v);
        float sg = acc2[0][r] * xh.x + acc2[1][r] * xh.y;
        float sb = acc2[0][r] + acc2[1][r];
        sg = zs(sg);
        sb = zs(sb);
        if constexpr (WGF) {
          sgv[i] = sg;
          sbv[i] = sb;
        } else {
        sg = half_sum32(sg);
        sb = half_sum32(sb);
        if ((lane & 31) == 31) {
          red[wave * 64 + row] = sg;
          red[wave * 64 + 32 + row] = sb;
        }
        }
        __builtin_amdgcn_sched_barrier(0);
      }
      if constexpr (WGF) {
        const float tg = half_sum8_dist(sgv, lane), tb = half_sum8_dist(sbv, lane);
        const int gi = (lane >> 2) & 7, rr = r8 * 8 + gi;
        if ((lane & 3) == 0) {
          const int rw = (rr & 3) + 8 * (rr >> 2) + 4 * h;
          red[wave * 64 + rw] = tg;
          red[wave * 64 + 32 + rw] = tb;
        }
      }
    }
    __syncthreads();
    if (threadIdx.x < 64) {
      const int e = threadIdx.x;
      gln += (red[e] + red[64 + e]) + (red[128 + e] + red[192 + e]);
    }
    __syncthreads();
  }

  float* row = wpart + (int64_t)blockIdx.x * kWgRow;
  __syncthreads();
#pragma unroll
  for (int a = 0; a < 2; ++a)
#pragma unroll
    for (int cb = 0; cb < 4; ++cb)
#pragma unroll
      for (int v = 0; v < 4; ++v) R[(wave * 32 + (a * 4 + cb) * 4 + v) * 64 + lane] = dW2[a][cb][v];
  __syncthreads();
  for (int e = threadIdx.x; e < 2048; e += 256) {
    const int idx = e >> 6, l = e & 63;
    const int a = idx >> 4, cb = (idx >> 2) & 3, v = idx & 3;
    const float t = (R[e] + R[2048 + e]) + (R[4096 + e] + R[6144 + e]);
    row[(16 * a + 4 * (l >> 4) + v) * 64 + 16 * cb + (l & 15)] = t;
  }
  __syncthreads();
#pragma unroll
  for (int cb = 0; cb < 4; ++cb)
#pragma unroll
    for (int kh = 0; kh < 2; ++kh)
#pragma unroll
      for (int v = 0; v < 4; ++v) R[(wave * 32 + (cb * 2 + kh) * 4 + v) * 64 + lane] = dW1[cb][kh][v];
  __syncthreads();
  for (int e = threadIdx.x; e < 2048; e += 256) {
    const int idx = e >> 6, l = e & 63;
    const int cb = idx >> 3, kh = (idx >> 2) & 1, v = idx & 3;
    const float t = (R[e] + R[2048 + e]) + (R[4096 + e] + R[6144 + e]);
    row[2048 + (16 * cb + 4 * (l >> 4) + v) * 32 + 16 * kh + (l & 15)] = t;
  }
  __syncthreads();
  R[(wave * 6 + 0) * 64 + lane] = db2[0];
  R[(wave * 6 + 1) * 64 + lane] = db2[1];
#pragma unroll
  for (int cb = 0; cb < 4; ++cb) R[(wave * 6 + 2 + cb) * 64 + lane] = db1[cb];
  __syncthreads();
  if (threadIdx.x < 96) {
    const int e = threadIdx.x, slot = e >> 4, i16 = e & 15;
    float t = 0.f;
    for (int w = 0; w < 4; ++w)
      for (int kk = 0; kk < 4; ++kk) t += R[(w * 6 + slot) * 64 + kk * 16 + i16];
    row[4096 + e] = t;
  }
  if (threadIdx.x < 64) row[4096 + 96 + threadIdx.x] = gln;
}


static int knob_mlp_wg_wgs() { return knob_pos(FZ_KNOB("FZ_MLP_WG_WGS"), 512); }
static int knob_chain_wgb() { const auto& k = FZ_KNOB("FZ_CHAIN_WGB"); return k.set ? k.val : 1; }

}

using namespace fz;

extern "C" int fz_mlp_wgrad_rows(int B, int64_t V) {
  const int64_t nt = fz_mlp_partials(B, V);
  const int wgs = knob_mlp_wg_wgs();
  return (int)(nt < wgs ? nt : wgs);
}
extern "C" int64_t fz_mlp_wgrad_workspace_bytes(int B, int64_t V) {
  return 2 * (int64_t)fz_mlp_wgrad_rows(B, V) * kWgRow * (int64_t)sizeof(float);
}

namespace fz {

template <typename AT>
int chain_wg_launch(const fz_mlp_desc* d, const GemmArgsT<AT>& a, const ChainArgsT<AT>& c, fz_stream_t stream) {
  hipStream_t st = (hipStream_t)stream;
  const int ntiles = (int)fz_mlp_partials(d->B, d->V), rows = fz_mlp_wgrad_rows(d->B, d->V);
  const int halves = d->H / 64;
  const bool bx = products_split(d->products);
  const bool wgb = bx && halves == 1 && knob_chain_wgb();
  void (*kern[2])(GemmArgsT<AT>, ChainArgsT<AT>, int, float*, float*) = {
      halves == 2 ? (bx ? gemm_chain_bwd_wg_kernel<AT, 2, 0, true> : gemm_chain_bwd_wg_kernel<AT, 2, 0, false>)
      : wgb       ? gemm_chain_bwd_wg_kernel<AT, 1, 0, true, true>
                  : (bx ? gemm_chain_bwd_wg_kernel<AT, 1, 0, true> : gemm_chain_bwd_wg_kernel<AT, 1, 0, false>),
      bx ? gemm_chain_bwd_wg_kernel<AT, 2, 1, true> : gemm_chain_bwd_wg_kernel<AT, 2, 1, false>};
  for (int half = 0; half < halves; ++half) {
    float* wp = (float*)d->wpart + (int64_t)half * rows * kWgRow;
    int rc = launch_lds(kern[half], dim3((unsigned)rows), dim3(256), chain_wg_lds_floats(bx, wgb), st, a, c, ntiles, wp,
                        halves == 2 ? d->glp : (float*)nullptr);
    if (rc != FZ_OK) return rc;
    FinishJob fj = finish_job(FK_CHAIN_WG, kWgRow / 16);
    fj.u.cw = FinChainWg{(const float*)wp, d->ln_g, d->ln_b, d->gw1 + half * 64 * 32, d->gb1 + half * 64, d->gw2 + half * 64,
                         half == 0 ? d->gb2 : (float*)nullptr, half == halves - 1 ? d->gln : (float*)nullptr, rows, d->H};
    rc = finish_run(&fj, 1, st);
    if (rc != FZ_OK) return rc;
  }
  return FZ_OK;
}
template int chain_wg_launch<float>(const fz_mlp_desc*, const GemmArgsT<float>&, const ChainArgsT<float>&, fz_stream_t);
template int chain_wg_launch<bf16>(const fz_mlp_desc*, const GemmArgsT<bf16>&, const ChainArgsT<bf16>&, fz_stream_t);

}
```

factorizer_amd/pointwise.py:

```python
from __future__ import annotations

import collections
import ctypes
import functools
import os
import threading as _threading
import weakref

import torch
import torch.nn.functional as F

from . import _native as N
from . import gradbuf as _GB
from . import functional as Fn

ACT = {"none": 0, "relu": 1, "gelu": 2}
LOAD_PLAIN, LOAD_S2D, LOAD_K3, LOAD_S2D_2D, LOAD_K3_2D = 0, 1, 2, 3, 4
EPI_PLAIN, EPI_D2S, EPI_LNBWD, EPI_D2S_2D = 0, 1, 2, 3
QL_S2D_2D, QL_K3_2D = LOAD_S2D_2D, LOAD_K3_2D
_D2S_FINE = {EPI_D2S: 8, EPI_D2S_2D: 4}


_p = N.ptr

# ... 136 lines not shown
    d.lnb_part = part.data_ptr()
    with torch.cuda.device(x.device):
        _gemm_launch(gz, d, *timed)
        ggamma, gbeta = _reduce_affine_rows(part, rows, C, x)
    return gx, ggamma, gbeta


def _dw_fused_ok(C, V):
    return C == 32 and V % 4 == 0 and V <= (1 << 27) and os.environ.get("FZ_DW_FUSED", "1") != "0"


def _gemm_dw(g, w2, q, ln=None, stats=None, gadd=None, want_bias=False, name="dgrad_wgrad", gw_out=None, gb_out=None, drop=None):
    B, C = q.shape[:2]
    V = _vox(q)
    dev = q.device
    y = torch.empty_like(q)
    gw = _GB.out_like(w2, (C, C), torch.float32) if gw_out is None else gw_out
    gb = (gb_out if gb_out is not None else torch.empty(C, dtype=torch.float32, device=dev)) if want_bias else None
    wpart = torch.empty(N.lib().fz_gemm_dw_workspace_bytes(B, V) // 4, dtype=torch.float32, device=dev)
    d = N.GemmDwDesc()
    d.g, d.q, d.w, d.y = g.data_ptr(), q.data_ptr(), w2.data_ptr(), y.data_ptr()
    d.wpart, d.gw, d.gb = wpart.data_ptr(), gw.data_ptr(), _p(gb)
    d.B, d.C, d.V, d.act_dtype = B, C, V, N.act_dtype(q)
    d.ldgw = gw.stride(0)
    d.ldw = w2.stride(0)
    if drop is not None:
        d.drop_m, d.drop_s = drop[0].data_ptr(), _drop_scale(drop[1])
    gpar = None
    if ln is not None:
        gpar = torch.empty(64, dtype=torch.float32, device=dev)
        d.ln, d.stats, d.ln_g, d.ln_b, d.gadd, d.gln = 1, stats.data_ptr(), ln[0].data_ptr(), ln[1].data_ptr(), _p(gadd), gpar.data_ptr()
    nbytes = q.element_size() * (3 * q.numel() + (gadd.numel() if gadd is not None else 0))
    with torch.cuda.device(dev), _finish_scope(wpart, gw, gb, gpar):
        rc = Fn._timed(f"{name}_{C}", nbytes, lambda: N.lib().fz_gemm_dw(ctypes.byref(d), N.stream_ptr(q)),
                       cols=B * V, flops=4 * B * V * C * C)
        N.check(rc, "fz_gemm_dw")
    if ln is not None:
        return y, gw, gb, gpar[:32], gpar[32:]
    return y, gw, gb, None, None


def _drop_scale(p):
    return 1.0 / (1.0 - float(ctypes.c_float(p).value))


def _mlp_dropout(drop):
    bits, ps = drop
    dd = N.MlpDropout()
    for s in range(3):
        if bits[s] is not None:
            setattr(dd, f"m{s}", bits[s].data_ptr())
            setattr(dd, f"s{s}", _drop_scale(ps[s]))
    return dd


def _mlp_drop_ok(C, Hd, V):
    return (_outproj_mlp_ok(C, Hd, V)
            and bool(N.lib().fz_mlp_drop_supported(C, Hd, V, N.products())))


def _mlp_chain_ok(C, Hd, V):
    return os.environ.get("FZ_MLP_CHAIN", "1") != "0" and bool(N.lib().fz_mlp_supported(C, Hd, V))


def _mlp_desc(mode, like, w12, w22, *, B, C, Hd, V, inp=None, b1=None, b2=None, ln_w=None, ln_b=None, eps=0.0, stats=None, z1=None,
              x1=None, out=None):
    d = N.MlpDesc()
    d.products = N.products()
    d.mode, d.inp, d.w1, d.w2, d.b1, d.b2 = mode, _p(inp), w12.data_ptr(), w22.data_ptr(), _p(b1), _p(b2)
    d.ln_g, d.ln_b, d.ln_eps = _p(ln_w), _p(ln_b), float(eps)
    d.stats, d.z1, d.x1, d.out = _p(stats), _p(z1), _p(x1), _p(out)
    d.B, d.C, d.H, d.V = B, C, Hd, V
    d.act_dtype = N.act_dtype(like)
    return d


def _mlp_chain_fwd(timed, like, ln_w, ln_b, eps, w12, b1, w22, b2, inp=None, pre=None, head=None, drop=None):
    B, C = like.shape[:2]
    V = _vox(like)
    Hd = w12.shape[0]
    new = lambda ch: torch.empty((B, ch, *like.shape[2:]), dtype=like.dtype, device=like.device)
    z1, st, x2 = new(Hd), _ln_stats(B, V, like.device), torch.empty_like(like)
    d = _mlp_desc(0, like, w12, w22, B=B, C=C, Hd=Hd, V=V, inp=inp, b1=b1, b2=b2, ln_w=ln_w, ln_b=ln_b, eps=eps, stats=st, z1=z1, out=x2)
    x1 = logits = None
    if pre is not None:
        a, wout2, bout, x = pre
        x1 = torch.empty_like(like)
        d.pre_in, d.pre_w, d.pre_b, d.pre_res, d.pre_out = a.data_ptr(), wout2.data_ptr(), _p(bout), x.data_ptr(), x1.data_ptr()
    if head is not None:
        hw, hb = head
        logits = new(hw.shape[0])
        d.post_w, d.post_b, d.post_out, d.post_m = hw.data_ptr(), _p(hb), logits.data_ptr(), hw.shape[0]
    dd = _mlp_dropout(drop) if drop is not None else None
    key, nbytes, flops = timed
    with torch.cuda.device(like.device):
        rc = Fn._timed(key, nbytes,
                       lambda: (N.lib().fz_mlp_chain(ctypes.byref(d), N.stream_ptr(like)) if dd is None
                                else N.lib().fz_mlp_chain_drop(ctypes.byref(d), ctypes.byref(dd), N.stream_ptr(like))),
                       cols=B * V, flops=flops)
    N.check(rc, "fz_mlp_chain")
    return x1, x2, z1, st, logits


def _mlp_fwd_chain(x1, ln_w, ln_b, eps, w12, b1, w22, b2):
    B, C = x1.shape[:2]
    V = _vox(x1)
    Hd = w12.shape[0]
    timed = (f"mlp_chain_fwd_{C}", x1.element_size() * (2 * x1.numel() + B * Hd * V), 4 * B * V * C * Hd)
    _, x2, z1, st, _ = _mlp_chain_fwd(timed, x1, ln_w, ln_b, eps, w12, b1, w22, b2, inp=x1)
    return x2, z1, st


_OUTPROJ_MLP = os.environ.get("FZ_OUTPROJ_MLP", "1") != "0"


def _outproj_mlp_ok(C, Hd, V):
    return _OUTPROJ_MLP and _mlp_chain_ok(C, Hd, V) and bool(N.lib().fz_mlp_pre_supported(C, Hd, V, N.products()))


def _outproj_mlp_fwd_chain(a, wout2, bout, x, ln_w, ln_b, eps, w12, b1, w22, b2, head=None, drop=None):
    B, C = a.shape[:2]
    V = _vox(a)
    Hd = w12.shape[0]
    nlogits = B * head[0].shape[0] * V if head is not None else 0
    timed = (f"outproj_mlp_chain_fwd_{C}", a.element_size() * (4 * a.numel() + B * Hd * V + nlogits), 4 * B * V * C * Hd + 2 * B * V * C * C)
    x1, x2, z1, st, logits = _mlp_chain_fwd(timed, a, ln_w, ln_b, eps, w12, b1, w22, b2, pre=(a, wout2, bout, x), head=head, drop=drop)
    if head is not None:
        return x1, x2, z1, st, logits
    return x1, x2, z1, st


def _mlp_bwd_chain(g2, z1, w12, w22, x1, st, ln_w):
    B, C = x1.shape[:2]
    V = _vox(x1)
    Hd = w12.shape[0]
    gz1 = torch.empty_like(z1)
    gx1 = torch.empty_like(x1)
    rows = N.lib().fz_mlp_partials(B, V)
    part = torch.empty((rows, 2 * C), dtype=torch.float32, device=x1.device)
    d = _mlp_desc(1, x1, w12, w22, B=B, C=C, Hd=Hd, V=V, inp=g2, ln_w=ln_w, stats=st, z1=z1, x1=x1, out=gx1)
    d.gz1, d.part = gz1.data_ptr(), part.data_ptr()
    with torch.cuda.device(x1.device):
        rc = Fn._timed(f"mlp_chain_bwd_{C}", x1.element_size() * (3 * x1.numel() + 2 * z1.numel()),
                       lambda: N.lib().fz_mlp_chain(ctypes.byref(d), N.stream_ptr(x1)), cols=B * V, flops=4 * B * V * C * Hd)
        N.check(rc, "fz_mlp_chain")
        ggamma, gbeta = _reduce_affine_rows(part, rows, C, x1)
    return gz1, gx1, ggamma, gbeta


def _mlp_wgrad_fused_ok(C, Hd, V):
    return _mlp_chain_ok(C, Hd, V) and C == 32 and Hd in (64, 128) and os.environ.get("FZ_MLP_FUSED_WGRAD", "1") != "0"


def _mlp_bwd_chain_wgrad(g2, z1, w12, w22, x1, st, ln_w, ln_b):
    B, C = x1.shape[:2]
    V = _vox(x1)
    Hd = w12.shape[0]
    dev = x1.device
    gx1 = torch.empty_like(x1)
    gpar = torch.empty(64, dtype=torch.float32, device=dev)
    wpart = torch.empty(N.lib().fz_mlp_wgrad_workspace_bytes(B, V) // 4, dtype=torch.float32, device=dev)
    gw1 = _GB.out_like(w12, (Hd, C), torch.float32)
    gw2 = _GB.out_like(w22, (C, Hd), torch.float32)
    gb1 = torch.empty(Hd, dtype=torch.float32, device=dev)
    gb2 = torch.empty(C, dtype=torch.float32, device=dev)
    glp = torch.empty(x1.shape, dtype=torch.float32, device=dev) if Hd == 128 else None
    d = _mlp_desc(2, x1, w12, w22, B=B, C=C, Hd=Hd, V=V, inp=g2, ln_w=ln_w, ln_b=ln_b, stats=st, z1=z1, x1=x1, out=gx1)
    d.gln, d.wpart, d.glp = gpar.data_ptr(), wpart.data_ptr(), _p(glp)
    d.gw1, d.gb1, d.gw2, d.gb2 = gw1.data_ptr(), gb1.data_ptr(), gw2.data_ptr(), gb2.data_ptr()
    nbytes = x1.element_size() * (3 * x1.numel() + z1.numel()) + (0 if Hd == 64 else x1.element_size() * 2 * x1.numel() + 8 * x1.numel())
    with torch.cuda.device(dev), _finish_scope(wpart, gpar, gw1, gb1, gw2, gb2):
        rc = Fn._timed(f"mlp_chain_bwd_wgrad_{C}" + ("" if Hd == 64 else f"x{Hd}"), nbytes,
                       lambda: N.lib().fz_mlp_chain(ctypes.byref(d), N.stream_ptr(x1)), cols=B * V, flops=8 * B * V * C * Hd)
        N.check(rc, "fz_mlp_chain")
    return gx1, gpar[:32], gpar[32:], gw1, gb1, gw2, gb2


_SIDE = {}


def _side_stream(dev, ncols):
    lim = int(os.environ.get("FZ_SIDE_WGRAD", "0"))
    if lim <= 0 or ncols > lim:
        return None
    key = (dev.type, dev.index)
    if key not in _SIDE:
        _SIDE[key] = torch.cuda.Stream(device=dev)
    return _SIDE[key]


class _LateJoin:
    enabled = False
    keep = []
    owed = []
    devices = set()
    queued = False
    verified = 0


def _end_of_backward():
    _LateJoin.queued = False
    join_wgrad_streams()


def reset_late_join():
    d = _LateJoin
    if d.devices:
        wait_wgrad_streams()
    d.owed.clear()
    d.keep.clear()
    d.queued = False


def late_wgrad_join(flag: bool = True):
    if not flag:
        join_wgrad_streams()
    _LateJoin.enabled = bool(flag) and os.environ.get("FZ_LATE_JOIN", "1") != "0"


def wait_wgrad_streams():
    d = _LateJoin
    for key in list(d.devices):
        dev = torch.device(*key)
        torch.cuda.current_stream(dev).wait_stream(_SIDE[key])
    d.devices.clear()
    d.keep.clear()


def wait_wgrad_streams_all(dev):
    key = (dev.type, dev.index if dev.index is not None else torch.cuda.current_device())
    st = _SIDE.get(key)
    if st is not None:
        torch.cuda.current_stream(dev).wait_stream(st)


def join_wgrad_streams():
    d = _LateJoin
    wait_wgrad_streams()
    owed, d.owed = d.owed, []
    d.verified += len(owed)
    for ref, ptr in owed:
        prm = ref()
        if prm is not None and prm.is_leaf and prm.requires_grad and (prm.grad is None or prm.grad.data_ptr() != ptr):
            raise RuntimeError("late_wgrad_join: a weight gradient was copied or replaced before the kernel "
                               "writing it had finished (accumulating into an existing .grad?); call "
                               "factorizer_amd.pointwise.late_wgrad_join(False) for this training loop")


class _Defer:
    enabled = False
    armed = False
    suppress = 0
    owned = frozenset()
    seen = set()
    keep = {}
    lock = _threading.Lock()
    queued = False
    flushed = 0
    flushes = 0
    refused = 0
    own_hooks = weakref.WeakSet()


def defer_finishes(flag: bool = True):
    if not flag:
        flush_finishes(disarm=True)
    _Defer.enabled = bool(flag) and os.environ.get("FZ_DEFER_FINISH", "1") != "0"


def arm_deferred_finishes(params=()):
    flush_finishes(disarm=True)
    d = _Defer
    d.queued = False
    d.owned = params if isinstance(params, frozenset) else frozenset(id(p) for p in params)
    d.seen = set()
    d.armed = d.enabled and bool(d.owned)


def flush_finishes(disarm: bool = False):
    d = _Defer
    if disarm:
        d.armed = False
    with d.lock:
        devs, keep, d.keep = list(d.keep), d.keep, {}
    for idx in devs:
        with torch.cuda.device(idx):
            n = N.lib().fz_finish_pending()
            if n:
                rc = Fn._timed("finish_batch", 0, lambda: N.lib().fz_finish_flush_all(torch.cuda.current_stream(idx).cuda_stream), cols=0)
                if rc < 0:
                    N.check(rc, "fz_finish_flush_all")
                d.flushed += rc
                d.flushes += 1
    keep.clear()


def _end_of_backward_finishes():
    _Defer.queued = False
    _Defer.seen = set()
    flush_finishes(disarm=True)


class _finish_scope:

    def __init__(self, *tensors):
        self.tensors = tensors
        self.on = False

    def __enter__(self):
        d = _Defer
        if d.armed and d.suppress == 0:
            t0 = next((t for t in self.tensors if t is not None), None)
            if t0 is not None and t0.is_cuda:
                if not d.queued:
                    try:
                        torch.autograd.Variable._execution_engine.queue_callback(_end_of_backward_finishes)
                        d.queued = True
                    except RuntimeError:
                        return self
                held = [t.detach() for t in self.tensors if t is not None]
                with d.lock:
                    d.keep.setdefault(t0.device.index, []).extend(held)
                self.was = N.lib().fz_finish_defer(1)
                self.on = True
        return self

    def __exit__(self, *exc):
        if self.on:
            N.lib().fz_finish_defer(self.was)
        return False


class _no_defer:
    def __enter__(self):
        _Defer.suppress += 1

    def __exit__(self, *exc):
        _Defer.suppress -= 1
        return False


_VIEW_NODES = frozenset(("ViewBackward0", "ReshapeAliasBackward0", "UnsafeViewBackward0", "UnsqueezeBackward0", "SqueezeBackward0",
                         "SqueezeBackward1", "AliasBackward0", "DetachBackward0"))


def _fwd(fn):
    inner = N.capture_products(fn)

    @functools.wraps(fn)
    def wrapper(ctx, *a, **kw):
        if getattr(ctx, "_fz_slots", None) is None:
            k, slots = 0, []
            for v in a:
                if isinstance(v, torch.Tensor):
                    slots.append(k)
                    k += 1
                else:
                    slots.append(-1)
            ctx._fz_slots = tuple(slots)
        return inner(ctx, *a, **kw)
    return wrapper


def owner_hook(hook):
    _Defer.own_hooks.add(hook)
    return hook


def _own_hook(hook) -> bool:
    try:
        return hook in _Defer.own_hooks
    except TypeError:
        return False


def _refuse(ctx, why):
    if os.environ.get("FZ_DEFER_DEBUG"):
        print(f"[defer] {type(ctx).__name__}: {why}", flush=True)
    return False


def _param_sinks_ok(ctx) -> bool:
    d = _Defer
    if torch.is_grad_enabled():
        return False
    acts = getattr(getattr(ctx, "_forward_cls", None), "_fz_acts", (0,))
    slots = getattr(ctx, "_fz_slots", None)
    need_grad = ctx.needs_input_grad
    nexts = ctx.next_functions
    if slots is None or len(slots) != len(need_grad) or max(slots, default=-1) + 1 != len(nexts):
        return _refuse(ctx, f"argument map {slots} does not fit {len(need_grad)} arguments / {len(nexts)} tensor inputs")
    for i, need in enumerate(need_grad):
        if not need or i in acts:
            continue
        if slots[i] < 0:
            return _refuse(ctx, f"input {i} needs a gradient and is no tensor")
        fn = nexts[slots[i]][0]
        while fn is not None and type(fn).__name__ in _VIEW_NODES:
            fn = fn.next_functions[0][0]
        if fn is None or type(fn).__name__ != "AccumulateGrad":
            return _refuse(ctx, f"input {i} sink {type(fn).__name__}")
        v = fn.variable
        vid = id(v)
        if vid not in d.owned or v.grad is not None or v._backward_hooks:
            return _refuse(ctx, f"input {i} {tuple(v.shape)} owned={vid in d.owned} grad={v.grad is not None} hooks={bool(v._backward_hooks)}")
        post = v._post_accumulate_grad_hooks
        if post and not all(_own_hook(h) for h in post.values()):
            return _refuse(ctx, f"input {i} {tuple(v.shape)} has a post-accumulate-grad hook that is not the owner's")
        if vid in d.seen:
            flush_finishes()
            return _refuse(ctx, f"input {i} {tuple(v.shape)} already served in this backward")
        d.seen.add(vid)
    return True


def _bwd(fn):
    inner = N.with_products(fn)

    @functools.wraps(fn)
    def wrapper(ctx, *a, **kw):
        d = _Defer
        if d.armed and d.suppress == 0 and not getattr(ctx, "_fz_defer_checked", False):
            ctx._fz_defer_checked = True
            if not _param_sinks_ok(ctx):
                d.refused += 1
                with _no_defer():
                    return inner(ctx, *a, **kw)
        return inner(ctx, *a, **kw)
    return wrapper


def _native_ok(*ts):
    t0 = ts[0]
    if not (t0.is_cuda and t0.numel() > 0 and t0.dtype in (torch.float32, torch.bfloat16) and _vox(t0) % 4 == 0):
        return False
    for t in ts[1:]:
        if t is None:
            continue
        if t.dim() >= 4:
            if t.dtype != t0.dtype:
                return False
        elif t.dtype != torch.float32:
            return False
    return True


def _head_rows_reduce(part, rows, w2, M, like):
    lib = N.lib()
    gw = _GB.out_like(w2, (M, 32), torch.float32)
    gb = torch.empty(M, dtype=torch.float32, device=like.device)
    st = N.stream_ptr(like)
    with _finish_scope(part, gw, gb):
        N.check(lib.fz_chunk_reduce_ld(part.data_ptr(), rows, M * 32, 132, gw.data_ptr(), 0, st), "fz_chunk_reduce_ld")
        N.check(lib.fz_chunk_reduce_ld(part.data_ptr() + 128 * 4, rows, M, 132, gb.data_ptr(), 0, st), "fz_chunk_reduce_ld")
    return gw, gb


def _head_bwd(gy, z, w2):
    B, C = z.shape[:2]
    V = _vox(z)
    M = w2.shape[0]
    lib = N.lib()
    gz = torch.empty_like(z)
    rows = lib.fz_head_bwd_rows()
    part = torch.empty(lib.fz_head_bwd_workspace_bytes() // 4, dtype=torch.float32, device=z.device)
    with torch.cuda.device(z.device):
        rc = Fn._timed(f"head_bwd_{C}->{M}", z.element_size() * (gy.numel() + 2 * z.numel()),
                       lambda: lib.fz_head_bwd(gy.data_ptr(), z.data_ptr(), w2.data_ptr(), gz.data_ptr(), part.data_ptr(),
                                               B, M, C, V, N.act_dtype(z), N.stream_ptr(z)), cols=B * V)
        N.check(rc, "fz_head_bwd")
        gw, gb = _head_rows_reduce(part, rows, w2, M, z)
    return gz, gw, gb


class LNLinearFn(torch.autograd.Function):
    @staticmethod
    @_fwd
    def forward(ctx, x, ln_w, ln_b, eps, w, b, act):
        x = x.contiguous()
        B, C = x.shape[:2]
        V = _vox(x)
        M = w.shape[0]
        w2 = w.reshape(M, C)
        y = torch.empty((B, M, *x.shape[2:]), dtype=x.dtype, device=x.device)
        stats = _ln_stats(B, V, x.device)
        _gemm([x], w2, y, B=B, Cin=C, Vin=V, M=M, K=C, Ncol=V, bias=b, ln=(ln_w, ln_b, eps), stats_out=stats,
              eact=ACT["relu" if act == "relu_out" else act], name="ln_linear")
        ctx.save_for_backward(x, stats, ln_w, ln_b, w2, y if act == "relu" else None)
        ctx.act, ctx.has_bias, ctx.wshape = act, b is not None, w.shape
        return y

    @staticmethod
    @_bwd
    def backward(ctx, gy):
        x, stats, ln_w, ln_b, w2, y = ctx.saved_tensors
        gy = gy.contiguous()
        B, C = x.shape[:2]
        V = _vox(x)
        M = w2.shape[0]
        gate = y if ctx.act == "relu" else None
        gl = torch.empty_like(x)
        _gemm([gy], w2, gl, B=B, Cin=M, Vin=V, M=C, K=M, Ncol=V, w_t=True, ldw=C, bmul=gate,
              bmul_kind=ACT["relu"], name="linear_dgrad")
        gx, ggamma, gbeta = _ln_backward(gl, x, stats, ln_w)
        gw = _GB.out_like(w2)
        gb = torch.empty(M, dtype=torch.float32, device=x.device)
        _wgrad(gy, [x], gw, B=B, M=M, Cin=C, K=C, Vq=V, Ncols=V, gbias=gb, pmul=gate, pmul_kind=ACT["relu"],
               stats=stats, ln=(ln_w, ln_b), name="wgrad_ln_linear")
        return gx, ggamma, gbeta, None, gw.reshape(ctx.wshape), (gb if ctx.has_bias else None), None


class ActLinearResFn(torch.autograd.Function):
    _fz_acts = (0, 3)

    @staticmethod
    @_fwd
    def forward(ctx, z, w, b, res, bact):
        z = z.contiguous()
        B, C = z.shape[:2]
        V = _vox(z)
        M = w.shape[0]
        w2 = w.reshape(M, C)
        if res is not None:
            res = res.contiguous()
        y = torch.empty((B, M, *z.shape[2:]), dtype=z.dtype, device=z.device)
        _gemm([z], w2, y, B=B, Cin=C, Vin=V, M=M, K=C, Ncol=V, bias=b, bact=ACT[bact], res=res,
              name="act_linear_res")
        ctx.save_for_backward(z, w2)
        ctx.bact, ctx.has_bias, ctx.has_res, ctx.wshape = bact, b is not None, res is not None, w.shape
        return y

    @staticmethod
    @_bwd
    def backward(ctx, gy):
        z, w2 = ctx.saved_tensors
        gy = gy.contiguous()
        B, C = z.shape[:2]
        V = _vox(z)
        M = w2.shape[0]
        if M <= 4 and C == 32 and ctx.bact == "none" and V % 4 == 0 and _HEAD_BWD:
            gz, gw, gb = _head_bwd(gy, z, w2)
            return gz, gw.reshape(ctx.wshape), (gb if ctx.has_bias else None), (gy if ctx.has_res else None), None
        gz = torch.empty_like(z)
        _gemm([gy], w2, gz, B=B, Cin=M, Vin=V, M=C, K=M, Ncol=V, w_t=True, ldw=C,
              emul=(z if ctx.bact != "none" else None), emul_kind=ACT[ctx.bact], name="linear_dgrad")
        gw = _GB.out_like(w2)
        gb = torch.empty(M, dtype=torch.float32, device=z.device)
        _wgrad(gy, [z], gw, B=B, M=M, Cin=C, K=C, Vq=V, Ncols=V, gbias=gb, qact=ACT[ctx.bact], name="wgrad_linear")
        return gz, gw.reshape(ctx.wshape), (gb if ctx.has_bias else None), (gy if ctx.has_res else None), None


class CatLinearFn(torch.autograd.Function):
    _fz_acts = (0, 1)

    @staticmethod
    @_fwd
    def forward(ctx, x1, x2, w, b):
        x1, x2 = x1.contiguous(), x2.contiguous()
        B, C1 = x1.shape[:2]
        C2 = x2.shape[1]
        V = _vox(x1)
        M = w.shape[0]
        w2 = w.reshape(M, C1 + C2)
        y = torch.empty((B, M, *x1.shape[2:]), dtype=x1.dtype, device=x1.device)
        _gemm([x1, x2], w2, y, B=B, Cin=C1 + C2, Vin=V, M=M, K=C1 + C2, Ncol=V, bias=b, c0=C1, name="cat_linear")
        ctx.save_for_backward(x1, x2, w2)
        ctx.has_bias, ctx.wshape = b is not None, w.shape
        return y

    @staticmethod
    @_bwd
    def backward(ctx, gy):
        x1, x2, w2 = ctx.saved_tensors
        gy = gy.contiguous()
        B, C1 = x1.shape[:2]
        C2 = x2.shape[1]
        V = _vox(x1)
        M = w2.shape[0]
        C = C1 + C2
        if M == 32 and C1 == 32 and C2 == 32 and _dw_fused_ok(M, V):
            gw = _GB.out_like(w2)
            g1, _, gb, _, _ = _gemm_dw(gy, w2[:, :C1], x1, want_bias=ctx.has_bias, name="dgrad_wgrad", gw_out=gw[:, :C1])
            g2, _, _, _, _ = _gemm_dw(gy, w2[:, C1:], x2, name="dgrad_wgrad", gw_out=gw[:, C1:])
            return g1, g2, gw.reshape(ctx.wshape), gb
        g1 = torch.empty_like(x1)
        g2 = torch.empty_like(x2)
        _gemm([gy], w2, g1, B=B, Cin=M, Vin=V, M=C1, K=M, Ncol=V, w_t=True, ldw=C, name="linear_dgrad")
        _gemm([gy], w2[:, C1:], g2, B=B, Cin=M, Vin=V, M=C2, K=M, Ncol=V, w_t=True, ldw=C, name="linear_dgrad")
        gw = _GB.out_like(w2)
        gb = torch.empty(M, dtype=torch.float32, device=gy.device)
        _wgrad(gy, [x1, x2], gw, B=B, M=M, Cin=C, K=C, Vq=V, Ncols=V, gbias=gb, c0=C1, name="wgrad_cat_linear")
        return g1, g2, gw.reshape(ctx.wshape), (gb if ctx.has_bias else None)


class LinearFn(torch.autograd.Function):
    @staticmethod
    @_fwd
    def forward(ctx, x, w, b):
        return ActLinearResFn.forward(ctx, x, w, b, None, "none")

    @staticmethod
    @_bwd
    def backward(ctx, gy):
        return ActLinearResFn.backward(ctx, gy)[:3]


class LayerNormFn(torch.autograd.Function):
    @staticmethod
    @_fwd
    def forward(ctx, x, w, b, eps):
        x = x.contiguous()
        B, C = x.shape[:2]
        V = _vox(x)
        y = torch.empty_like(x)
        stats = _ln_stats(B, V, x.device)
        with torch.cuda.device(x.device):
            rc = Fn._timed(f"ln_fwd_{C}", 2 * x.element_size() * x.numel(), lambda: N.lib().fz_ln_fwd(
                x.data_ptr(), w.data_ptr(), b.data_ptr(), y.data_ptr(), stats.data_ptr(), B, C, V, eps,
                N.act_dtype(x), N.stream_ptr(x)), cols=B * V)
        N.check(rc, "fz_ln_fwd")
        ctx.save_for_backward(x, stats, w)
        return y

    @staticmethod
    @_bwd
# ... 254 lines not shown
        z = LinearFn.apply(x, w1, b1)
        return ActLinearResFn.apply(z, w2, b2, None, "gelu")
    _warn_composed("MLP", x, w1, b1, w2, b2)
    return linear_cf(F.gelu(linear_cf(x, w1, b1)), w2, b2)


def ln_linear(x, ln_w, ln_b, eps, w, b, act="none"):
    if _native_ok(x, ln_w, ln_b, w, b) and w.shape[1] % 2 == 0:
        return LNLinearFn.apply(x, ln_w, ln_b, eps, w, b, act)
    _warn_composed("LayerNorm+Linear", x, ln_w, ln_b, w, b)
    y = linear_cf(layernorm_cf(x, ln_w, ln_b, eps), w, b)
    return torch.relu(y) if act != "none" else y


def act_linear_res(z, w, b, res, act="none"):
    if _native_ok(z, w, b, res) and w.shape[1] % 2 == 0:
        return ActLinearResFn.apply(z, w, b, res, act)
    _warn_composed("Linear+residual", z, w, b, res)
    y = linear_cf(F.gelu(z) if act == "gelu" else z, w, b)
    return y if res is None else res + y


class UpCatLinearFn(torch.autograd.Function):

    _fz_acts = (0, 1, 6)

    @staticmethod
    @_fwd
    def forward(ctx, skip, deep, w_t, b_t, w_ad, b_ad, pro=None):
        skip, deep = skip.contiguous(), deep.contiguous()
        B, Cd, D, H, W = deep.shape
        O = w_t.shape[1]
        V = D * H * W
        C1 = skip.shape[1]
        M = w_ad.shape[0]
        w2 = w_ad.reshape(M, C1 + O)
        y = torch.empty((B, M, *skip.shape[2:]), dtype=skip.dtype, device=skip.device)
        if (M == 32 and C1 == 32 and O == 32 and _UPCAT_FWD and N.lib().fz_upcat_supported(C1, Cd, D, H, W)):
            w_b = w2[:, C1:]
            wbt = torch.empty((8, M, Cd), dtype=torch.float32, device=skip.device)
            bias = torch.empty(M, dtype=torch.float32, device=skip.device) if (b_t is not None or b_ad is not None) else None
            with torch.cuda.device(skip.device):
                N.check(N.lib().fz_upcat_compose(w_t.data_ptr(), w_b.data_ptr(), C1 + O, _p(b_t), _p(b_ad), None, wbt.data_ptr(),
                                                 _p(bias), Cd, O, M, N.stream_ptr(skip)), "fz_upcat_compose")
            es = skip.element_size()
            bp = None
            if pro is not None:
                ln_w, ln_b, eps, w_in = pro
                t_pro = torch.empty_like(y)
                st_pro = torch.empty((B, 2, 8 * V), dtype=torch.float32, device=skip.device)
                bp = N.BlockPrologue(ln_w.data_ptr(), ln_b.data_ptr(), float(eps), w_in.data_ptr(), t_pro.data_ptr(), st_pro.data_ptr())
            with torch.cuda.device(skip.device):
                rc = Fn._timed(f"upcat_{Cd}->{M}" + ("_ln_linear" if bp is not None else ""),
                               es * (skip.numel() + deep.numel() + y.numel() * (2 if bp is not None else 1)),
                               lambda: N.lib().fz_upcat2(skip.data_ptr(), deep.data_ptr(), w2.data_ptr(), C1 + O, wbt.data_ptr(),
                                                         _p(bias), y.data_ptr(), B, C1, Cd, D, H, W, N.act_dtype(skip),
                                                         ctypes.byref(bp) if bp is not None else None, N.stream_ptr(skip)),
                               cols=B * 8 * V, flops=2 * B * 8 * V * M * (C1 + Cd))
            N.check(rc, "fz_upcat")
        elif pro is not None:
            raise RuntimeError("UpCatLinearFn: a block prologue needs the one-pass forward (callers check upcat_prologue_ok)")
        else:
            up = torch.empty((B, O, 2 * D, 2 * H, 2 * W), dtype=deep.dtype, device=deep.device)
            _gemm([deep], w_t, up, B=B, Cin=Cd, Vin=V, M=8 * O, K=Cd, Ncol=V, w_t=True, ldw=8 * O, bias=b_t,
                  epilogue=EPI_D2S, Ho=H, Wo=W, name="tconv_k2s2")
            _gemm([skip, up], w2, y, B=B, Cin=C1 + O, Vin=8 * V, M=M, K=C1 + O, Ncol=8 * V, bias=b_ad, c0=C1, name="cat_linear")
        ctx.save_for_backward(skip, deep, w_t, w2, b_t)
        ctx.has_bt, ctx.has_bad, ctx.wshape = b_t is not None, b_ad is not None, w_ad.shape
        ctx.npro = 0 if pro is None else 1
        if pro is not None:
            ctx.mark_non_differentiable(t_pro, st_pro)
            ctx.set_materialize_grads(False)
            return y, t_pro, st_pro
        return y

    @staticmethod
    def _backward_three(ctx, g, skip, deep, w2, wc, gw_ad, gb_ad, gt):
        B, Cd, D, H, W = deep.shape
        V = D * H * W
        Vf = 8 * V
        C1 = skip.shape[1]
        M = w2.shape[0]
        O = w2.shape[1] - C1
        dev = g.device
        if M == 32 and C1 == 32 and _dw_fused_ok(M, Vf):
            g_skip, _, _, _, _ = _gemm_dw(g, w2[:, :C1], skip, want_bias=True, name="dgrad_wgrad",
                                          gw_out=gw_ad[:, :C1], gb_out=gb_ad)
        else:
            g_skip = torch.empty_like(skip)
            _gemm([g], w2, g_skip, B=B, Cin=M, Vin=Vf, M=C1, K=M, Ncol=Vf, w_t=True, ldw=C1 + O, name="linear_dgrad")
            gwa = torch.empty((M, C1), dtype=torch.float32, device=dev)
            with _no_defer():
                _wgrad(g, [skip], gwa, B=B, M=M, Cin=C1, K=C1, Vq=Vf, Ncols=Vf, gbias=gb_ad, name="wgrad_linear")
            gw_ad[:, :C1].copy_(gwa)
        g_deep = None
        if ctx.needs_input_grad[1]:
            g_deep = torch.empty_like(deep)
            _gemm([g], wc, g_deep, B=B, Cin=M, Vin=Vf, M=Cd, K=8 * M, Ncol=V, loader=LOAD_S2D,
                  Di=2 * D, Hi=2 * H, Wi=2 * W, Ho=H, Wo=W, name="tconv_k2s2_dgrad")
        _wgrad(deep, [g], gt, B=B, M=Cd, Cin=M, K=8 * M, Vq=Vf, Ncols=V, loader=LOAD_S2D, D=2 * D, H=2 * H,
               W=2 * W, Ho=H, Wo=W, name="wgrad_tconv_k2s2")
        return g_skip, g_deep

    @staticmethod
    @_bwd
    def backward(ctx, g, _gt=None, _gst=None):
        skip, deep, w_t, w2, b_t = ctx.saved_tensors
        if g is None:
            g = torch.zeros((skip.shape[0], w2.shape[0], *skip.shape[2:]), dtype=skip.dtype, device=skip.device)
        g = g.contiguous()
        B, Cd, D, H, W = deep.shape
        O = w_t.shape[1]
        V = D * H * W
        Vf = 8 * V
        C1 = skip.shape[1]
        M = w2.shape[0]
        dev = g.device
        gw_ad = _GB.out_like(w2)
        gb_ad = torch.empty(M, dtype=torch.float32, device=dev)
        w_b = w2[:, C1:]
        wc = torch.empty((Cd, M, 2, 2, 2), dtype=torch.float32, device=dev)
        with torch.cuda.device(dev):
            N.check(N.lib().fz_upcat_compose(w_t.data_ptr(), w_b.data_ptr(), C1 + O, None, None, wc.data_ptr(), None, None,
                                             Cd, O, M, N.stream_ptr(g)), "fz_upcat_compose")
        gt = torch.empty((Cd, M, 8), dtype=torch.float32, device=dev)
        if (M == 32 and ctx.needs_input_grad[1] and _UPCAT_BWD and skip.dtype == g.dtype == deep.dtype
                and N.lib().fz_upcat_bwd_supported(C1, Cd, D, H, W, N.act_dtype(g))
                and not ((g.data_ptr() | skip.data_ptr()) & 7 or deep.data_ptr() & 15)):
            g_skip, g_deep = torch.empty_like(skip), torch.empty_like(deep)
            ws = torch.empty(N.lib().fz_upcat_bwd_workspace_bytes(B, D, H, W) // 4, dtype=torch.float32, device=dev)
            es = g.element_size()
            with torch.cuda.device(dev), _finish_scope(ws, gt, gw_ad, gb_ad):
                rc = Fn._timed(f"upcat_bwd_{Cd}->{M}", es * (3 * g.numel() + 2 * deep.numel()),
                               lambda: N.lib().fz_upcat_bwd(g.data_ptr(), skip.data_ptr(), deep.data_ptr(), w2.data_ptr(), C1 + O,
                                                            wc.data_ptr(), g_skip.data_ptr(), g_deep.data_ptr(), ws.data_ptr(),
                                                            gw_ad.data_ptr(), C1 + O, gb_ad.data_ptr(), gt.data_ptr(), B, C1, Cd,
                                                            D, H, W, N.act_dtype(g), N.stream_ptr(g)),
                               cols=B * Vf, flops=4 * B * Vf * M * (C1 + Cd))
            N.check(rc, "fz_upcat_bwd")
        else:
            g_skip, g_deep = UpCatLinearFn._backward_three(ctx, g, skip, deep, w2, wc, gw_ad, gb_ad, gt)
        gw_t = _GB.out_like(w_t)
        gb_t = torch.empty(O, dtype=torch.float32, device=dev) if ctx.has_bt else None
        with torch.cuda.device(dev), _finish_scope(gt, gb_ad, gw_t, gw_ad, gb_t):
            N.check(N.lib().fz_upcat_wgrads(gt.data_ptr(), w_t.data_ptr(), w_b.data_ptr(), C1 + O, gb_ad.data_ptr(), _p(b_t),
                                            gw_t.data_ptr(), gw_ad[:, C1:].data_ptr(), C1 + O, _p(gb_t), Cd, O, M,
                                            N.stream_ptr(g)), "fz_upcat_wgrads")
        return (g_skip, g_deep, gw_t, gb_t, gw_ad.reshape(ctx.wshape), gb_ad if ctx.has_bad else None, None)[:len(ctx.needs_input_grad)]


_UPCAT_FWD = os.environ.get("FZ_UPCAT_FWD", "1") != "0"
_UPCAT_BWD = os.environ.get("FZ_UPCAT_BWD", "1") != "0"
_HEAD_BWD = os.environ.get("FZ_HEAD_BWD", "1") != "0"


def up_cat_linear(skip, deep, w_t, b_t, w_ad, b_ad=None, pro=None):
    return UpCatLinearFn.apply(skip, deep, w_t, b_t, w_ad, b_ad, pro)


_PRODUCER_PROLOGUE = os.environ.get("FZ_PRODUCER_PROLOGUE", "1") != "0"


def conv3_prologue_ok(x, w):
    return (_PRODUCER_PROLOGUE and x.is_cuda and x.dim() == 5 and x.shape[1] * 27 * 64 * 4 <= 65536 and x.dtype in (torch.float32, torch.bfloat16)
            and bool(N.lib().fz_conv3_prologue_supported(int(x.shape[1]), int(w.shape[0]), int(x.shape[-1]), N.products())))


def upcat_prologue_ok(skip, deep, w_t, w_ad):
    B, Cd, D, H, W = deep.shape
    O, C1, M = w_t.shape[1], skip.shape[1], w_ad.shape[0]
    return (_PRODUCER_PROLOGUE and M == 32 and C1 == 32 and O == 32 and _UPCAT_FWD and bool(N.lib().fz_upcat_supported(C1, Cd, D, H, W)))


class BlockPrologue:
    _tls = _threading.local()

    def __init__(self, x, t, st):
        self.x, self.t, self.st = x, t, st

    def __enter__(self):
        tls = BlockPrologue._tls
        self.prev = getattr(tls, "cur", None)
        tls.cur = self
        return self

    def __exit__(self, *exc):
        BlockPrologue._tls.cur = self.prev

    @staticmethod
    def take(x):
        cur = getattr(BlockPrologue._tls, "cur", None)
        if cur is not None and cur.x is x:
            return cur.t, cur.st
        return None


def cat_linear(x1, x2, w, b=None):
    if _native_ok(x1, x2, w, b) and x1.shape[1] % 2 == 0 and x2.shape[1] % 2 == 0:
        return CatLinearFn.apply(x1, x2, w, b)
    _warn_composed("cat+Linear", x1, x2, w, b)
    return linear_cf(torch.cat([x1, x2], dim=1), w, b)


def _block_dropout_bits(x, C, Hd, drop):
    B, V = x.shape[0], _vox(x)
    seed = Fn.dropout_seed(x.device)
    return tuple(None if p == 0 else Fn.dropout_keep_bits(seed, s, B, ch, V, p) for s, (ch, p) in enumerate(zip((C, Hd, C), drop)))


def _block_tail_fwd(a, wout2, bout, x, ln_w, ln_b, eps, w12, b1, w22, b2, drop=None, bits=(None, None, None)):
    B, C = x.shape[:2]
    V = _vox(x)
    Hd = w12.shape[0]
    new = lambda ch: torch.empty((B, ch, *x.shape[2:]), dtype=x.dtype, device=x.device)
    (p0, p1, p2), (m0, m1, m2) = drop or (0, 0, 0), bits
    if m0 is not None:
        o = new(C)
        _gemm([a], wout2, o, B=B, Cin=C, Vin=V, M=C, K=C, Ncol=V, bias=bout, name="linear")
        x1 = Fn.dropout_apply(N.DROP_RES, m0, p0, o, x)
        del o
    else:
        x1 = new(C)
        _gemm([a], wout2, x1, B=B, Cin=C, Vin=V, M=C, K=C, Ncol=V, bias=bout, res=x, name="act_linear_res")
    z1 = new(Hd)
    st2 = _ln_stats(B, V, x.device)
    _gemm([x1], w12, z1, B=B, Cin=C, Vin=V, M=Hd, K=C, Ncol=V, bias=b1, ln=(ln_w, ln_b, eps), stats_out=st2, name="ln_linear")
    h, bact = (Fn.dropout_apply(N.DROP_GELU, m1, p1, z1), ACT["none"]) if m1 is not None else (z1, ACT["gelu"])
    if m2 is not None:
        o = new(C)
        _gemm([h], w22, o, B=B, Cin=Hd, Vin=V, M=C, K=Hd, Ncol=V, bias=b2, bact=bact, name="linear")
        x2 = Fn.dropout_apply(N.DROP_RES, m2, p2, o, x1)
        del o
    else:
        x2 = new(C)
        _gemm([h], w22, x2, B=B, Cin=Hd, Vin=V, M=C, K=Hd, Ncol=V, bias=b2, bact=bact, res=x1, name="act_linear_res")
    return x1, x2, z1, st2


class FactorizerBlockFn(torch.autograd.Function):

    _fz_acts = (0, 4, 5, 14, 15, 16, 17, 18)

    @staticmethod
    @_fwd
    def forward(ctx, x, n1w, n1b, win, u0, v0, wout, bout, n2w, n2b, w1, b1, w2, b2, cfg, head_w=None, head_b=None,
                t_pre=None, st_pre=None):
        x = x.contiguous()
        B, C = x.shape[:2]
        V = _vox(x)
        sp = x.shape[2:]
        geo, T, G, solver, neps = cfg["geo"], cfg["T"], cfg["G"], cfg["solver"], cfg["nmf_eps"]
        win2, wout2 = win.reshape(C, C), wout.reshape(C, C)
        Hd = w1.shape[0]
        w12, w22 = w1.reshape(Hd, C), w2.reshape(C, Hd)
        u0c, v0c = u0.contiguous(), v0.contiguous()
        new = lambda ch: torch.empty((B, ch, *sp), dtype=x.dtype, device=x.device)
        drop = cfg.get("drop")
        bits = _block_dropout_bits(x, C, Hd, drop) if drop is not None else (None, None, None)
        if t_pre is not None:
            t, st1 = t_pre, st_pre
        else:
            t = new(C)
            st1 = _ln_stats(B, V, x.device)
            _gemm([x], win2, t, B=B, Cin=C, Vin=V, M=C, K=C, Ncol=V, ln=(n1w, n1b, cfg["eps1"]), stats_out=st1,
                  eact=ACT["relu"], name="ln_linear")
        m = None
        if cfg["core"]:
            a = Fn.FactCoreFn.forward(_Ctx(), t, u0c, v0c, geo, T, G, solver, neps, True)
        else:
            m = Fn._swm_fwd_raw(t, geo)
            ym, _, _ = Fn._nmf_fwd_raw(m, u0c, v0c, T, solver, neps)
            a = Fn._swm_inv_raw(ym, geo, average=True)
            del ym
        logits = None
        tail = (a, wout2, bout, x, n2w, n2b, cfg["eps2"], w12, b1, w22, b2)
        if (_mlp_drop_ok if drop is not None else _outproj_mlp_ok)(C, Hd, V) and a.is_contiguous():
            head = (head_w.reshape(head_w.shape[0], C), head_b) if head_w is not None and drop is None else None
            x1, x2, z1, st2, *logits = _outproj_mlp_fwd_chain(*tail, head=head, drop=(bits, drop) if drop is not None else None)
            logits = logits[0] if logits else None
        elif drop is None and _mlp_chain_ok(C, Hd, V):
            x1 = new(C)
            _gemm([a], wout2, x1, B=B, Cin=C, Vin=V, M=C, K=C, Ncol=V, bias=bout, res=x, name="act_linear_res")
            x2, z1, st2 = _mlp_fwd_chain(x1, n2w, n2b, cfg["eps2"], w12, b1, w22, b2)
        else:
            x1, x2, z1, st2 = _block_tail_fwd(*tail, drop, bits)
        ctx.save_for_backward(x, st1, t, a, x1, st2, z1, m, n1w, n1b, win2, u0c, v0c, wout2, n2w, n2b, w12, w22, *bits)
        ctx.cfg = cfg
        ctx.shapes = (win.shape, wout.shape, w1.shape, w2.shape)
        ctx.prm = tuple(weakref.ref(t) for t in (win, wout, bout, w1, b1, w2, b2))
        if head_w is not None:
            if logits is None:
                raise RuntimeError("FactorizerBlockFn: head fusion asked for a configuration outside fz_mlp_pre_supported "
                                   "(callers check block_head_fusable first)")
            ctx.mark_non_differentiable(logits)
            ctx.set_materialize_grads(False)
            return x2, logits
        return x2

    @staticmethod
    @_bwd
    def backward(ctx, g2, _g_logits=None):
        x, st1, t, a, x1, st2, z1, m, n1w, n1b, win2, u0c, v0c, wout2, n2w, n2b, w12, w22, *bits = ctx.saved_tensors
        cfg = ctx.cfg
        drop = cfg.get("drop")
        if g2 is None:
            g2 = torch.zeros_like(x)
        g2 = g2.contiguous()
        B, C = x.shape[:2]
        V = _vox(x)
        Hd = w12.shape[0]
        dev, dt = x.device, x.dtype
        geo, T, G, solver, neps = cfg["geo"], cfg["T"], cfg["G"], cfg["solver"], cfg["nmf_eps"]
        cur = torch.cuda.current_stream(dev)
        side = _side_stream(dev, B * V)
        keep = []

        pending = []

        def wgrad(*args, **kw):
            if _WGRAD_GROUP:
                kw.pop("name", None)
                pending.append((args[0], args[1], args[2], kw))
                return args[2]
            if side is None:
                return _wgrad(*args, **kw)
            side.wait_stream(cur)
            keep.extend(t for t in (args[0], *args[1], kw.get("stats")) if t is not None)
            with torch.cuda.stream(side):
                return _wgrad(*args, **kw)

        chain = _mlp_chain_ok(C, Hd, V) and drop is None
        (p0, p1, p2), (m0, m1, m2) = drop or (0, 0, 0), bits
        if drop is None and _mlp_wgrad_fused_ok(C, Hd, V):
            gx1, gg2, gbt2, gw1, gb1, gw2, gb2 = _mlp_bwd_chain_wgrad(g2, z1, w12, w22, x1, st2, n2w, n2b)
        else:
            gelu = ACT["gelu" if m1 is None else "none"]
            gf = Fn.dropout_apply(N.DROP_RES, m2, p2, g2) if m2 is not None else g2
            gw2 = _GB.out_like(w22)
            gb2 = torch.empty(C, dtype=torch.float32, device=dev)
            if chain:
                gz1, gx1, gg2, gbt2 = _mlp_bwd_chain(g2, z1, w12, w22, x1, st2, n2w)
            else:
                gz1 = torch.empty_like(z1)
                _gemm([gf], w22, gz1, B=B, Cin=C, Vin=V, M=Hd, K=C, Ncol=V, w_t=True, ldw=Hd, emul=(z1 if m1 is None else None),
                      emul_kind=gelu, name="linear_dgrad")
                if m1 is not None:
                    gz1 = Fn.dropout_apply(N.DROP_GELU_BWD, m1, p1, gz1, z1)
            h = Fn.dropout_apply(N.DROP_GELU, m1, p1, z1) if m1 is not None else z1
            wgrad(gf, [h], gw2, B=B, M=C, Cin=Hd, K=Hd, Vq=V, Ncols=V, gbias=gb2, qact=gelu, name="wgrad_linear")
            del h, gf
            if not chain:
                gx1, gg2, gbt2 = _dgrad_lnbwd(gz1, w12, x1, st2, n2w, g2)
            gw1 = _GB.out_like(w12)
            gb1 = torch.empty(Hd, dtype=torch.float32, device=dev)
            wgrad(gz1, [x1], gw1, B=B, M=Hd, Cin=C, K=C, Vq=V, Ncols=V, gbias=gb1, stats=st2, ln=(n2w, n2b),
                  name="wgrad_ln_linear")
            del gz1
        go, go_drop = gx1, None
        if m0 is not None:
            if _dw_fused_ok(C, V):
                go_drop = (m0, p0)
            else:
                go = Fn.dropout_apply(N.DROP_RES, m0, p0, gx1)
        dw = _dw_fused_ok(C, V)
        if dw:
            ga, gwo, gbo, _, _ = _gemm_dw(go, wout2, a, want_bias=True, name="dgrad_wgrad", drop=go_drop)
        else:
            ga = torch.empty_like(a)
            _gemm([go], wout2, ga, B=B, Cin=C, Vin=V, M=C, K=C, Ncol=V, w_t=True, ldw=C, name="linear_dgrad")
            gwo = _GB.out_like(wout2)
            gbo = torch.empty(C, dtype=torch.float32, device=dev)
            wgrad(go, [a], gwo, B=B, M=C, Cin=C, K=C, Vq=V, Ncols=V, gbias=gbo, name="wgrad_linear")
        del go
        if G <= 0:
            gt = torch.zeros_like(t)
        elif cfg["core"]:
            c2 = _Ctx()
            c2.saved_tensors = (t, u0c, v0c)
            c2.cfg = (geo, T, G, solver, neps, True)
            gt = Fn.FactCoreFn.backward(c2, ga)[0]
        else:
            gym = Fn._swm_fwd_raw(ga, geo, div=geo.nshift)
            gm = Fn._nmf_bwd_raw(m, u0c, v0c, gym, None, None, T, G, solver, neps)
            del gym
            gt = Fn._swm_inv_raw(gm, geo, average=False, gate=m)
            del gm
        del ga
        if dw:
            gx, gwi, _, gg1, gbt1 = _gemm_dw(gt, win2, x, ln=(n1w, n1b), stats=st1, gadd=gx1, name="dgrad_lnbwd_wgrad")
        else:
            gx, gg1, gbt1 = _dgrad_lnbwd(gt, win2, x, st1, n1w, gx1)
            gwi = _GB.out_like(win2)
            wgrad(gt, [x], gwi, B=B, M=C, Cin=C, K=C, Vq=V, Ncols=V, stats=st1, ln=(n1w, n1b), name="wgrad_ln_linear")
        if pending:
            if side is None:
                _wgrad_group(pending, f"wgrad_block_{C}x{Hd}")
            else:
                side.wait_stream(cur)
                for pr in pending:
                    keep.extend(t for t in (pr[0], *pr[1], pr[3].get("stats"), pr[3].get("pmul")) if t is not None)
                with torch.cuda.stream(side):
                    _wgrad_group(pending, f"wgrad_block_{C}x{Hd}")
            pending.clear()
        if side is not None:
            if _LateJoin.enabled:
                _LateJoin.keep.extend(keep)
                _LateJoin.devices.add((dev.type, dev.index))
                _LateJoin.owed.extend(zip(ctx.prm, (t.data_ptr() for t in (gwi, gwo, gbo, gw1, gb1, gw2, gb2))))
                if not _LateJoin.queued:
                    _LateJoin.queued = True
                    torch.autograd.Variable._execution_engine.queue_callback(_end_of_backward)
            else:
                cur.wait_stream(side)
            keep.clear()
        s_in, s_out, s_1, s_2 = ctx.shapes
        return (gx, gg1, gbt1, gwi.reshape(s_in), None, None, gwo.reshape(s_out), gbo, gg2, gbt2,
                gw1.reshape(s_1), gb1, gw2.reshape(s_2), gb2, None, None, None, None, None)[:len(ctx.needs_input_grad)]


_head_fusion = _threading.local()


class HeadFusion:

    def __init__(self, block, head_params):
        self.block, self.head_params, self.logits = block, head_params, None

    def __enter__(self):
        self.prev = getattr(_head_fusion, "slot", None)
        _head_fusion.slot = self
        return self

    def __exit__(self, *exc):
        _head_fusion.slot = self.prev


def head_fusion_slot():
    return getattr(_head_fusion, "slot", None)


def block_head_fusable(C, Hd, V, head_w, x):
    return (C == 32 and _outproj_mlp_ok(C, Hd, V) and head_w is not None and head_w.dtype == torch.float32 and head_w.numel() == head_w.shape[0] * C
            and 1 <= head_w.shape[0] <= 4 and x.is_cuda and _HEAD_BWD)


class HeadOfBlockFn(torch.autograd.Function):

    _fz_acts = (0, 3)

    @staticmethod
    @_fwd
    def forward(ctx, y, w, b, logits):
        ctx.save_for_backward(y, w)
        ctx.has_bias, ctx.wshape = b is not None, w.shape
        return logits.view_as(logits)

    @staticmethod
    @_bwd
    def backward(ctx, gl):
        y, w = ctx.saved_tensors
        B, C = y.shape[:2]
        V = _vox(y)
        M = w.shape[0]
        w2 = w.reshape(M, C)
        gl = gl.contiguous()
        if gl.dtype != y.dtype:
            gl = gl.to(y.dtype)
        gy, gw, gb = _head_bwd(gl, y, w2)
        return gy, gw.reshape(ctx.wshape), (gb if ctx.has_bias else None), None


class _Ctx:

    saved_tensors = ()

    def save_for_backward(self, *ts):
        self.saved_tensors = ts
```

include/factorizer_hip.h:

```cpp
#ifndef FACTORIZER_HIP_H
#define FACTORIZER_HIP_H

#include <stdint.h>

#ifdef __cplusplus
extern "C" {
#endif

#define FZ_OK 0
#define FZ_E_SHAPE (-1)
#define FZ_E_UNSUPPORTED (-2)
#define FZ_E_HIP (-3)
#define FZ_E_ARG (-4)

#define FZ_STORE_F32 0
#define FZ_STORE_BF16 1

#define FZ_SOLVER_MU 0
#define FZ_SOLVER_HALS 1
#define FZ_SOLVER_CD 2
#define FZ_SOLVER_SMU 3

typedef void* fz_stream_t;

// ... 70 lines not shown
                                int D, int H, int W, const int* shift, int nshift, int T, int Tgrad, float eps,
                                int act_dtype, fz_stream_t stream);
int fz_nmf_cf_bwd_from_factors(const void* t, const float* v0, const void* ga, const float* gcfac, const float* cofac,
                               void* gt, int B, int C, int D, int H, int W, const int* shift, const int* prev_shift,
                               int nshift, int T, int Tgrad, float eps, int act_dtype, fz_stream_t stream);

int fz_nmf_pcf_supported(int C, int D, int H, int W, int d, int pd, int ph, int pw, int R, int T, int Tgrad);
int fz_nmf_pcf_fwd(const void* t, const float* u0, const float* v0, void* out, int B, int C, int D, int H, int W,
                   int pd, int ph, int pw, const int* shift, int accumulate, int divisor, int R, int T, int solver,
                   float eps, int act_dtype, fz_stream_t stream);
int fz_nmf_pcf_bwd(const void* t, const float* u0, const float* v0, const void* ga, void* gt, int B, int C, int D,
                   int H, int W, int pd, int ph, int pw, const int* shift, int accumulate, int nshift, int relu_gate,
                   int R, int T, int Tgrad, int solver, float eps, int act_dtype, fz_stream_t stream);
int fz_nmf_pcf_bwd_prefers_separate(int pd, int ph, int pw, int act_dtype);
int fz_act_add(void* dst, const void* src, int64_t n, int act_dtype, fz_stream_t stream);

#define FZ_LOAD_PLAIN 0
#define FZ_LOAD_S2D 1
#define FZ_LOAD_K3 2
#define FZ_EPI_PLAIN 0
#define FZ_EPI_D2S 1
#define FZ_EPI_LNBWD 2
#define FZ_LOAD_S2D_2D 3
#define FZ_LOAD_K3_2D 4
#define FZ_EPI_D2S_2D 3
#define FZ_ACT_NONE 0
#define FZ_ACT_RELU 1
#define FZ_ACT_GELU 2

#define FZ_PRODUCTS_DEFAULT 0
#define FZ_PRODUCTS_SPLIT_BF16 1
#define FZ_PRODUCTS_FP32_MFMA 2

typedef struct fz_gemm_desc {
  const void* x[4];
  int nsrc;
  int src_mode;
  int c0;
  int Cin;
  int64_t Vin;
  int Di, Hi, Wi;
  const float* w;
  int w_t, ldw;
  int M, K;
  const float* bias;
  int ln;
  const float* ln_g;
  const float* ln_b;
  float ln_eps;
  float* stats_out;
  int bact;
  const void* bmul;
  int bmul_kind;
  int eact;
  const void* res;
  const void* emul;
  int emul_kind;
  void* y;
  int64_t Ncol;
  int Ho, Wo;
  int B;
  int loader, epilogue;
  const void* lnb_x;
  const float* lnb_stats;
  const float* lnb_g;
  const void* lnb_gadd;
  float* lnb_part;
  int act_dtype;
  int products;
  int tune;
} fz_gemm_desc;

int64_t fz_gemm_lnbwd_partials(const fz_gemm_desc* desc);
int fz_reduce_rows(const float* part, int64_t rows, int n, float* out, float* tmp, fz_stream_t stream);

int fz_gemm(const fz_gemm_desc* desc, fz_stream_t stream);
int fz_gemm_plan(const fz_gemm_desc* desc, char* form, int cap);
int fz_gemm_bx_enable(int on);

typedef struct fz_mlp_desc {
  int mode;
  const void* in;
  const float* w1;
  const float* w2;
  const float* b1;
  const float* b2;
  const float* ln_g;
  const float* ln_b;
  float ln_eps;
  float* stats;
  void* z1;
  void* gz1;
  const void* x1;
  void* out;
  float* part;
  int B, C, H;
  int64_t V;
  int act_dtype;
  void* wpart;
  float* gw1;
  float* gb1;
  float* gw2;
  float* gb2;
  float* gln;
  float* glp;
  int products;
  const void* pre_in;
  const float* pre_w;
  const float* pre_b;
  const void* pre_res;
  void* pre_out;
  const float* post_w;
  const float* post_b;
  void* post_out;
  int post_m;
} fz_mlp_desc;
typedef struct fz_mlp_dropout {
  const uint32_t* m0;
  const uint32_t* m1;
  const uint32_t* m2;
  float s0, s1, s2;
} fz_mlp_dropout;

typedef struct fz_gemm_dw_desc {
  const void* g;
  const void* q;
  const float* w;
  int ln;
  const float* stats;
  const float* ln_g;
  const float* ln_b;
  const void* gadd;
  void* y;
  float* gln;
  void* wpart;
  float* gw;
  float* gb;
  int B, C;
  int64_t V;
  int act_dtype;
  int ldgw;
  int ldw;
  const uint32_t* drop_m;
  float drop_s;
} fz_gemm_dw_desc;
int fz_gemm_dw_rows(int B, int64_t V);
int64_t fz_gemm_dw_workspace_bytes(int B, int64_t V);
int fz_gemm_dw(const fz_gemm_dw_desc* desc, fz_stream_t stream);

int fz_head_bwd_rows(void);
int64_t fz_head_bwd_workspace_bytes(void);
int fz_head_bwd(const void* gy, const void* x, const float* w, void* gx, float* part, int B, int M, int C, int64_t V,
                int act_dtype, fz_stream_t stream);
int fz_head_fwd(const void* x, const float* w, const float* bias, void* y, int B, int M, int C, int64_t V, int act_dtype,
                fz_stream_t stream);

int fz_upcat_compose(const float* w_t, const float* w_b, int ldb, const float* b_t, const float* b_ad, float* wc, float* wbt, float* bias,
                     int Cd, int O, int M, fz_stream_t stream);
int fz_upcat_wgrads(const float* gt, const float* w_t, const float* w_b, int ldb, const float* gb_ad, const float* b_t, float* gw_t,
                    float* gw_b, int ldg, float* gb_t, int Cd, int O, int M, fz_stream_t stream);
int fz_upcat_supported(int C, int Cd, int D, int H, int W);
int fz_upcat(const void* skip, const void* deep, const float* wa, int lda, const float* wbt, const float* bias, void* out,
             int B, int C, int Cd, int D, int H, int W, int act_dtype, fz_stream_t stream);
int fz_upcat_bwd_supported(int C1, int Cd, int D, int H, int W, int act_dtype);
int64_t fz_upcat_bwd_workspace_bytes(int B, int D, int H, int W);
int fz_upcat_bwd(const void* g, const void* skip, const void* deep, const float* wa, int lda, const float* wc, void* g_skip,
                 void* g_deep, void* workspace, float* gw_a, int ldg, float* gb, float* gt, int B, int C1, int Cd, int D, int H,
                 int W, int act_dtype, fz_stream_t stream);
typedef struct fz_block_prologue {
  const float* ln_g;
  const float* ln_b;
  float ln_eps;
  const float* w;
  void* t;
  float* stats;
} fz_block_prologue;
int fz_upcat2(const void* skip, const void* deep, const float* wa, int lda, const float* wbt, const float* bias, void* out,
              int B, int C, int Cd, int D, int H, int W, int act_dtype, const fz_block_prologue* pro, fz_stream_t stream);

int fz_mlp_supported(int C, int H, int64_t V);
int fz_mlp_pre_supported(int C, int H, int64_t V, int products);
int fz_mlp_drop_supported(int C, int H, int64_t V, int products);
int64_t fz_mlp_partials(int B, int64_t V);
int fz_mlp_wgrad_rows(int B, int64_t V);
int64_t fz_mlp_wgrad_workspace_bytes(int B, int64_t V);
int fz_mlp_chain(const fz_mlp_desc* desc, fz_stream_t stream);
int fz_mlp_chain_drop(const fz_mlp_desc* desc, const fz_mlp_dropout* drop, fz_stream_t stream);

#define FZ_QL_PLAIN 0
#define FZ_QL_S2D 1
#define FZ_QL_K3 2
#define FZ_QL_S2D_2D 3
#define FZ_QL_K3_2D 4

typedef struct fz_wgrad_desc {
  const void* p;
  int M;
  const void* pmul;
  int pmul_kind;
  const void* q[4];
  int nsrc, src_mode, c0;
  int Cin;
  int K;
  int64_t Vq;
  int D, H, W;
  int64_t N;
  int Ho, Wo;
  const float* stats;
  int qact;
  const float* ln_g;
  const float* ln_b;
  float* gw;
  float* gbias;
  int accumulate;
  int B;
  int loader;
  int act_dtype;
  int products;
} fz_wgrad_desc;

int64_t fz_wgrad_workspace_bytes(const fz_wgrad_desc* desc);
int fz_wgrad(const fz_wgrad_desc* desc, void* workspace, fz_stream_t stream);
int fz_wgrad_group(const fz_wgrad_desc* const* descs, void* const* workspaces, int n, fz_stream_t stream);

int fz_ln_fwd(const void* x , const float* gamma, const float* beta, void* y ,
              float* stats, int B, int C, int64_t V, float eps, int act_dtype, fz_stream_t stream);
int64_t fz_ln_bwd_workspace_bytes(int C);
int64_t fz_ln_bwd_workspace_bytes2(int B, int C, int64_t V);
int fz_ln_bwd(const void* gl, const void* x, const float* stats, const float* gamma,
              const void* gadd, void* gx , float* gparams, void* workspace,
              int B, int C, int64_t V, int act_dtype, fz_stream_t stream);

int fz_conv3_fwd(const void* x , const float* w, const float* bias, void* y ,
                 int B, int Cin, int M, int D, int H, int W, int act_dtype, int products, fz_stream_t stream);
struct fz_block_prologue;
int fz_conv3_prologue_supported(int Cin, int M, int W, int products);
int fz_conv3_fwd2(const void* x, const float* w, const float* bias, void* y, int B, int Cin, int M, int D, int H, int W,
                  int act_dtype, int products, const struct fz_block_prologue* pro, fz_stream_t stream);
int fz_conv3_wgrad_chunks(int B, int D, int H, int W);
int fz_conv3_wgrad_partials(const void* gy, const void* x , float* part, float* part_bias, int B,
                            int Cin, int M, int D, int H, int W, int act_dtype, int products, fz_stream_t stream);
int fz_chunk_reduce(const float* part, int nchunk, int64_t n, float* out, int accumulate, fz_stream_t stream);
int fz_chunk_reduce_ld(const float* part, int nchunk, int64_t n, int64_t ld, float* out, int accumulate, fz_stream_t stream);

int fz_rowsum_chunks(int64_t V);
int fz_rowsum(const void* x , float* part, float* out, int B, int C, int64_t V, int act_dtype,
              fz_stream_t stream);

int fz_gcorr_supported(int Ci, int Co, int kd, int kh, int kw);
int fz_gcorr(const float* in, const float* w, float* out, const float* mul_a, const float* mul_b, int B, int G,
             int Ci, int Co, int D, int H, int W, int kd, int kh, int kw, int w_batched, float add_eps,
             fz_stream_t stream);
int64_t fz_gcorr_wgrad_workspace_bytes(int B, int G, int Ci, int Co, int D, int H, int W, int kd, int kh, int kw);
int fz_gcorr_wgrad(const float* in, const float* gout, float* gw, void* ws, int B, int G, int Ci, int Co, int D, int H,
                   int W, int kd, int kh, int kw, int w_batched, fz_stream_t stream);
int fz_gcorr_act(const void* in, const float* w, void* out, const void* mul_a, const void* mul_b, int B, int G,
                 int Ci, int Co, int D, int H, int W, int kd, int kh, int kw, int w_batched, float add_eps,
                 int act_dtype, fz_stream_t stream);
int fz_gcorr_wgrad_act(const void* in, const void* gout, float* gw, void* ws, int B, int G, int Ci, int Co, int D, int H,
                       int W, int kd, int kh, int kw, int w_batched, int act_dtype, fz_stream_t stream);
int fz_gcorr_mu_bwd(const void* r, const float* wT, const void* g, const void* s, const void* num, void* ds, void* dnum,
                    void* dden, int B, int G, int Ci, int Co, int D, int H, int W, int kd, int kh, int kw, int w_batched,
                    float eps, int act_dtype, fz_stream_t stream);

int fz_dice_bce_chunks(int64_t V);
int fz_dice_bce_sums(const float* z, const float* t, float* part, int planes, int64_t V, fz_stream_t stream);
int fz_dice_bce_grad(const float* z, const float* t, const float* coef, float* gz, int planes, int64_t V,
                     float cd, float cb, const float* gscale, fz_stream_t stream);

int fz_dice_ce_sums(const float* z, const float* t, float* part, int B, int C, int64_t V, fz_stream_t stream);
int fz_dice_ce_finish(const float* part, int B, int C, int64_t V, float smooth, float* loss, float* coef, fz_stream_t stream);
int fz_dice_ce_grad(const float* z, const float* t, const float* coef, float* gz, int B, int C, int64_t V,
                    float cd, float cb, const float* gscale, fz_stream_t stream);

int fz_dice_bce_ds_sums(const float* z, const void* t, float* part, int planes, int Td, int Th, int Tw, int Ld, int Lh, int Lw,
                        int tkind, fz_stream_t stream);
int fz_dice_bce_ds_grad(const float* z, const void* t, const float* coef, float* gz, int planes, int Td, int Th, int Tw,
                        int Ld, int Lh, int Lw, int tkind, float cd, float cb, const float* gscale, fz_stream_t stream);
int fz_dice_ce_ds_sums(const float* z, const void* t, float* part, int B, int C, int Td, int Th, int Tw, int Ld, int Lh, int Lw,
                       int tkind, fz_stream_t stream);
int fz_dice_ce_ds_grad(const float* z, const void* t, const float* coef, float* gz, int B, int C, int Td, int Th, int Tw,
                       int Ld, int Lh, int Lw, int tkind, float cd, float cb, const float* gscale, fz_stream_t stream);

int fz_sw_gather(const float* vol, float* win, int C, int D, int H, int W, int rd, int rh, int rw, int z0, int y0,
                 int x0, fz_stream_t stream);
int fz_sw_accumulate(const float* prob, float* out, float* cnt, const float* gz, const float* gy, const float* gx,
                     float wmin, int C, int D, int H, int W, int rd, int rh, int rw, int z0, int y0, int x0,
                     fz_stream_t stream);
int fz_sw_finalize(float* out, const float* cnt, int C, int64_t V, fz_stream_t stream);
int fz_sw_gather2(const void* img, void* win, int C, int D, int H, int W, int rd, int rh, int rw, int z0, int y0, int x0,
                  int act_dtype, fz_stream_t stream);
int fz_sw_accumulate2(const void* prob, float* out, float* cnt, const float* gz, const float* gy, const float* gx,
                      float wmin, int C, int D, int H, int W, int rd, int rh, int rw, int z0, int y0, int x0, int act_dtype,
                      fz_stream_t stream);
int fz_sw_finalize2(const float* out, const float* cnt, void* res, int C, int64_t V, int act_dtype, fz_stream_t stream);

#define FZ_SEG_F32 0
#define FZ_SEG_BF16 1
#define FZ_SEG_U8 2
int fz_seg_counts_chunks(int64_t V);
int64_t fz_seg_counts_workspace_bytes(int planes, int64_t V);
int fz_seg_counts(const void* pred, int pred_kind, const void* label, int label_kind, float bound, uint8_t* mask,
                  void* workspace, int64_t* counts, int planes, int64_t V, fz_stream_t stream);
int fz_mask_edges(const uint8_t* mask, uint8_t* edges, int64_t* counts, int planes, int nd, int D, int H, int W,
                  fz_stream_t stream);
int fz_edge_min_dist2_splits(int64_t nq, int64_t nt);
int64_t fz_edge_min_dist2_workspace_bytes(int64_t nq, int64_t nt);
int fz_edge_min_dist2(const float* q, int64_t nq, const float* t, int64_t nt, float w0, float w1, float w2, float* out,
                      void* workspace, fz_stream_t stream);

int fz_aug_record_floats(void);
int fz_aug_resample(const void* img, void* img_out, int act_dtype, int C, const uint8_t* lab, uint8_t* lab_out, int L,
                    const float* table, const int64_t* seed, float* smooth_ws, int ns, int B, int nd, int D, int H, int W,
                    fz_stream_t stream);
int fz_aug_smooth(const float* smooth_ws, void* img_out, int act_dtype, int C, const float* table, const int32_t* list, int ns,
                  int B, int nd, int D, int H, int W, fz_stream_t stream);
int fz_aug_noise_field(float* out, const int64_t* seed, int B, int C, int64_t V, fz_stream_t stream);
int fz_aug_source_words(void);
int fz_aug_crop_resample(const int64_t* sources, void* img_out, int act_dtype, int C, uint8_t* lab_out, int L, const float* table,
                         const int64_t* seed, float* smooth_ws, int ns, int B, int nd, int D, int H, int W, fz_stream_t stream);

#define FZ_VOL_F32 0
#define FZ_VOL_BF16 1
#define FZ_VOL_U8 2
#define FZ_VOL_I16 3
#define FZ_VOL_ROLE_IMAGE_IN 0
#define FZ_VOL_ROLE_IMAGE_OUT 1
#define FZ_VOL_ROLE_LABEL_IN 2
#define FZ_VOL_ROLE_LOGITS 3
typedef struct fz_vol_geom {
  int nd;
  int size[3];
  int start[3];
  int end[3];
  int pad[3];
  int out[3];
} fz_vol_geom;
int fz_vol_kind_ok(int role, int kind);
int fz_vol_bbox(const void* image, int kind, int C, int nd, int D, int H, int W, int32_t* box, fz_stream_t stream);
int64_t fz_vol_workspace_bytes(int C, const fz_vol_geom* geom);
// ... 54 lines not shown
```

Baseline: 133.2.

## Fuse head input-gradient into final block MLP backward wgrad chain

Instead of materializing the head's input gradient (a 32-channel f32 volume), the head backward now computes only weight gradients and hands a zero-stride stand-in gradient to the final block. The block's fused MLP wgrad kernel recomputes g2 on the fly from the head logit gradient (M≤4 channels) via small fp32 MFMAs. This removes a full-volume write and read of g2. In exchange it adds autograd linking state, LDS for head weights and bias accumulators, and a fallback path when the stand-in is not claimed.

After: 133.8, median of 6. No clear change (+0.5%).

```diff
diff --git a/factorizer_amd/_native.py b/factorizer_amd/_native.py
--- a/factorizer_amd/_native.py
+++ b/factorizer_amd/_native.py
@@ -265,6 +265,9 @@
     "fz_head_bwd_workspace_bytes": ([], _i64),
     "fz_head_bwd": ([_vp, _vp, _vp, _vp, _vp, _i, _i, _i, _i64, _i, _vp], _i),
     "fz_head_fwd": ([_vp, _vp, _vp, _vp, _i, _i, _i, _i64, _i, _vp], _i),
+    "fz_head_wgrad": ([_vp, _vp, _vp, _i, _i, _i, _i64, _i, _vp], _i),
+    "fz_mlp_head_g2_supported": ([_i, _i, _i64, _i, _i, _i, _i], _i),
+    "fz_mlp_chain_head": ([_c.POINTER(MlpDesc), _vp, _vp, _i, _vp], _i),
     "fz_upcat_supported": ([_i] * 5, _i),
     "fz_upcat_compose": ([_vp, _vp, _i, _vp, _vp, _vp, _vp, _vp, _i, _i, _i, _vp], _i),
     "fz_upcat_wgrads": ([_vp, _vp, _vp, _i, _vp, _vp, _vp, _vp, _i, _vp, _i, _i, _i, _vp], _i),
diff --git a/factorizer_amd/blocks.py b/factorizer_amd/blocks.py
--- a/factorizer_amd/blocks.py
+++ b/factorizer_amd/blocks.py
@@ -152,6 +152,7 @@
                     if PW.block_head_fusable(C, Hd, x[0, 0].numel(), hw, x):
                         y, raw = PW.FactorizerBlockFn.apply(*args, hw, hb, t_pre, st_pre)
                         slot.logits = PW.HeadOfBlockFn.apply(y, hw, hb, raw)
+                        PW.link_head_g2(y, slot.logits, C, Hd, x[0, 0].numel(), hw.shape[0], drop)
                         return y
                 return PW.FactorizerBlockFn.apply(*args, None, None, t_pre, st_pre)
             if drop is None:
diff --git a/factorizer_amd/csrc/headbwd.hip b/factorizer_amd/csrc/headbwd.hip
--- a/factorizer_amd/csrc/headbwd.hip
+++ b/factorizer_amd/csrc/headbwd.hip
@@ -4,15 +4,17 @@
 
 constexpr int kHeadRow = 4 * 33;
 
-template <int M, typename AT>
+template <int M, typename AT, bool GX = true>
 __global__ __launch_bounds__(256, 2) void head_bwd_kernel(const AT* __restrict__ gy, const AT* __restrict__ x,
                                                           const float* __restrict__ w, AT* __restrict__ gx,
                                                           float* __restrict__ part, int B, int64_t V, int Mr) {
   __shared__ float red[4][kHeadRow];
   __shared__ float sW[M * 32];
   const int lane = threadIdx.x & 63, wave = threadIdx.x >> 6;
-  for (int i = threadIdx.x; i < M * 32; i += 256) sW[i] = i < Mr * 32 ? w[i] : 0.f;
-  __syncthreads();
+  if constexpr (GX) {
+    for (int i = threadIdx.x; i < M * 32; i += 256) sW[i] = i < Mr * 32 ? w[i] : 0.f;
+    __syncthreads();
+  }
   float gw[M][32];
   float gb[M];
 #pragma unroll
@@ -48,15 +50,17 @@
 #pragma unroll
       for (int u = 0; u < CB; ++u) {
         const int c = c0 + u;
-        float o[4];
+        if constexpr (GX) {
+          float o[4];
 #pragma unroll
-        for (int e = 0; e < 4; ++e) {
-          float t = sW[c] * g4[0][e];
+          for (int e = 0; e < 4; ++e) {
+            float t = sW[c] * g4[0][e];
 #pragma unroll
-          for (int m = 1; m < M; ++m) t += sW[m * 32 + c] * g4[m][e];
-          o[e] = t;
+            for (int m = 1; m < M; ++m) t += sW[m * 32 + c] * g4[m][e];
+            o[e] = t;
+          }
+          vstore<4>(ob + (int64_t)c * V, o);
         }
-        vstore<4>(ob + (int64_t)c * V, o);
 #pragma unroll
         for (int m = 0; m < M; ++m)
           gw[m][c] += (g4[m][0] * xv[u][0] + g4[m][1] * xv[u][1]) + (g4[m][2] * xv[u][2] + g4[m][3] * xv[u][3]);
@@ -141,8 +145,9 @@
 static int head_bwd_launch(const void* gy, const void* x, const float* w, void* gx, float* part, int B, int M, int64_t V,
                            hipStream_t st) {
   const unsigned grid = (unsigned)fz_head_bwd_rows();
-#define FZ_HEAD(MM) hipLaunchKernelGGL((head_bwd_kernel<MM, AT>), dim3(grid), dim3(256), 0, st, (const AT*)gy, (const AT*)x, w, (AT*)gx, part, B, V, M)
-  if (M <= 2) FZ_HEAD(2); else FZ_HEAD(4);
+#define FZ_HEAD(MM, GX) hipLaunchKernelGGL((head_bwd_kernel<MM, AT, GX>), dim3(grid), dim3(256), 0, st, (const AT*)gy, (const AT*)x, w, (AT*)gx, part, B, V, M)
+  if (gx) { if (M <= 2) FZ_HEAD(2, true); else FZ_HEAD(4, true); }
+  else    { if (M <= 2) FZ_HEAD(2, false); else FZ_HEAD(4, false); }
 #undef FZ_HEAD
   FZ_LAUNCH_CHECK();
   return FZ_OK;
@@ -157,6 +162,17 @@
   if (act_dtype == FZ_STORE_F32) return head_bwd_launch<float>(gy, x, w, gx, part, B, M, V, (hipStream_t)stream);
   if (act_dtype == FZ_STORE_BF16) return head_bwd_launch<bf16>(gy, x, w, gx, part, B, M, V, (hipStream_t)stream);
   return fail(FZ_E_ARG, "fz_head_bwd: act_dtype must be FZ_STORE_F32 or FZ_STORE_BF16");
+}
+
+extern "C" int fz_head_wgrad(const void* gy, const void* x, float* part, int B, int M, int C, int64_t V, int act_dtype,
+                             fz_stream_t stream) {
+  if (!gy || !x || !part) return fail(FZ_E_ARG, "fz_head_wgrad: null pointer");
+  if (act_dtype != FZ_STORE_F32 && act_dtype != FZ_STORE_BF16) return fail(FZ_E_ARG, "fz_head_wgrad: act_dtype must be FZ_STORE_F32 or FZ_STORE_BF16");
+  if (C != 32 || M < 1 || M > 4 || V < 4 || V % 4 != 0) return fail(FZ_E_UNSUPPORTED, "fz_head_wgrad: needs C == 32, 1 <= M <= 4, V % 4 == 0");
+  if ((int64_t)B * (V / 4) >= ((int64_t)1 << 31)) return fail(FZ_E_UNSUPPORTED, "fz_head_wgrad: 2^31 or more voxel quads");
+  if (B <= 0) return B == 0 ? FZ_OK : fail(FZ_E_SHAPE, "fz_head_wgrad: negative batch");
+  if (act_dtype == FZ_STORE_F32) return head_bwd_launch<float>(gy, x, nullptr, nullptr, part, B, M, V, (hipStream_t)stream);
+  return head_bwd_launch<bf16>(gy, x, nullptr, nullptr, part, B, M, V, (hipStream_t)stream);
 }
 
 template <typename AT>
diff --git a/factorizer_amd/csrc/mlp_chain.h b/factorizer_amd/csrc/mlp_chain.h
--- a/factorizer_amd/csrc/mlp_chain.h
+++ b/factorizer_amd/csrc/mlp_chain.h
@@ -30,8 +30,8 @@
 constexpr int chain64_lds_floats(bool p512, bool pre) {
   return 2 * (p512 ? 12288 : 8192) + (pre ? 6144 + 64 : 0) + 128 + 64 + (p512 ? 2 : 1) * 512;
 }
-constexpr int chain_wg_lds_floats(bool bx, bool wgb) {
-  return 2 * (bx ? 3072 : 2048) + 32 + 256 + 4 * (wgb ? 3072 : 48 * kTS);
+constexpr int chain_wg_lds_floats(bool bx, bool wgb, bool hg = false) {
+  return 2 * (bx ? 3072 : 2048) + 32 + 256 + 4 * (wgb ? 3072 : 48 * kTS) + (hg ? 128 + 6 * 256 + 64 : 0);
 }
 
 template <typename... KArgs, typename... Args>
@@ -52,6 +52,6 @@
 template <typename AT>
 int chain64_launch(const fz_mlp_desc* d, const GemmArgsT<AT>& a, const ChainArgsT<AT>& c, fz_stream_t stream);
 template <typename AT>
-int chain_wg_launch(const fz_mlp_desc* d, const GemmArgsT<AT>& a, const ChainArgsT<AT>& c, fz_stream_t stream);
+int chain_wg_launch(const fz_mlp_desc* d, const GemmArgsT<AT>& a, const ChainArgsT<AT>& c, fz_stream_t stream, bool head = false);
 
 }
diff --git a/factorizer_amd/csrc/mlp_chain.hip b/factorizer_amd/csrc/mlp_chain.hip
--- a/factorizer_amd/csrc/mlp_chain.hip
+++ b/factorizer_amd/csrc/mlp_chain.hip
@@ -26,6 +26,13 @@
           && knob_chain_fwd_bx()) ? 1 : 0;
 }
 
+extern "C" int fz_mlp_head_g2_supported(int C, int H, int64_t V, int mode, int products, int M, int act_dtype) {
+  return (C == 32 && H == 64 && mode == 2 && fz_mlp_supported(C, H, V) && products_split(products) && M >= 1 && M <= 4
+          && act_dtype == FZ_STORE_F32) ? 1 : 0;
+}
+
+struct MlpHead { const void* gy; const float* w; int M; };
+
 template <typename AT>
 static void forward_args(const fz_mlp_desc* d, int ldw, int ldwB, GemmArgsT<AT>& a, ChainArgsT<AT>& c) {
   a.w = d->w1; a.w_t = 0; a.ldw = ldw;
@@ -46,7 +53,7 @@
   c.wB = d->w1; c.wB_t = 1; c.ldwB = ldwB; c.side = side;
 }
 
-static int mlp_check(const fz_mlp_desc* d, const fz_mlp_dropout* dd, bool drop) {
+static int mlp_check(const fz_mlp_desc* d, const fz_mlp_dropout* dd, bool drop, const MlpHead* hd) {
   if (!fz_mlp_supported(d->C, d->H, d->V)) return fail(FZ_E_UNSUPPORTED, "fz_mlp_chain: needs (C, H) in {(32, 64), (32, 128), (64, 128)}, V % 4 == 0");
   if (drop) {
     if (!fz_mlp_drop_supported(d->C, d->H, d->V, d->products) || d->mode != 0 || !d->pre_in)
@@ -63,7 +70,9 @@
     return fail(FZ_E_UNSUPPORTED, "fz_mlp_chain: the fused out-projection runs on split-bf16 products only (fz_mlp_pre_supported)");
   if (d->post_out && (!pre || d->C != 32 || !d->post_w || d->post_m < 1 || d->post_m > 4))
     return fail(FZ_E_ARG, "fz_mlp_chain: post_out needs pre_in, C == 32, post_w and 1 <= post_m <= 4");
-  if ((!d->in && !pre) || !d->w1 || !d->w2 || !d->out || !d->z1 || !d->stats)
+  if (hd && (!fz_mlp_head_g2_supported(d->C, d->H, d->V, d->mode, d->products, hd->M, d->act_dtype) || pre))
+    return fail(FZ_E_UNSUPPORTED, "fz_mlp_chain_head: needs (C, H) = (32, 64), mode 2, split-bf16 products, 1 <= M <= 4, fp32 storage (fz_mlp_head_g2_supported)");
+  if ((!d->in && !pre && !hd) || !d->w1 || !d->w2 || !d->out || !d->z1 || !d->stats)
     return fail(FZ_E_ARG, "fz_mlp_chain: null pointer");
   if (d->mode == 0 && (!d->ln_g || !d->ln_b)) return fail(FZ_E_ARG, "fz_mlp_chain: forward needs the LayerNorm affine");
   if (d->mode == 1 && (!d->gz1 || !d->x1 || !d->ln_g || !d->part)) return fail(FZ_E_ARG, "fz_mlp_chain: backward needs gz1, x1, gamma, part");
@@ -75,9 +84,9 @@
 }
 
 template <typename AT>
-static int mlp_launch(const fz_mlp_desc* d, const fz_mlp_dropout* dd, fz_stream_t stream) {
+static int mlp_launch(const fz_mlp_desc* d, const fz_mlp_dropout* dd, fz_stream_t stream, const MlpHead* hd = nullptr) {
   const bool drop = dd && (dd->m0 || dd->m1 || dd->m2);
-  const int rc = mlp_check(d, dd, drop);
+  const int rc = mlp_check(d, dd, drop, hd);
   if (rc != FZ_OK) return rc;
   if (d->B == 0) {
     if (d->mode == 2) {
@@ -95,8 +104,9 @@
   a.x[0] = (const AT*)d->in; a.nsrc = 1; a.c0 = d->C; a.Cin = d->C; a.Vin = d->V; a.M = d->H; a.K = d->C; a.Ncol = d->V; a.B = d->B;
   if (d->mode == 0) forward_args(d, d->C, d->H, a, c);
   else backward_args(d, d->H, d->C, d->mode == 1 ? (AT*)d->gz1 : (AT*)nullptr, a, c);
+  if (hd) { a.x[0] = (const AT*)hd->gy; c.postW = hd->w; c.postM = hd->M; }
   if (d->C == 64) return chain64_launch(d, a, c, stream);
-  if (d->mode == 2) return chain_wg_launch(d, a, c, stream);
+  if (d->mode == 2) return chain_wg_launch(d, a, c, stream, hd != nullptr);
   return chain32_launch(d, drop ? dd : nullptr, a, c, stream);
 }
 
@@ -113,3 +123,11 @@
   if (d->act_dtype == FZ_STORE_BF16) return mlp_launch<bf16>(d, drop, stream);
   return fail(FZ_E_ARG, "fz_mlp_chain_drop: act_dtype must be FZ_STORE_F32 or FZ_STORE_BF16");
 }
+
+extern "C" int fz_mlp_chain_head(const fz_mlp_desc* d, const void* gy, const float* head_w, int M, fz_stream_t stream) {
+  if (!d || !gy || !head_w) return fail(FZ_E_ARG, "fz_mlp_chain_head: null pointer");
+  const MlpHead hd = {gy, head_w, M};
+  if (d->act_dtype == FZ_STORE_F32) return mlp_launch<float>(d, nullptr, stream, &hd);
+  if (d->act_dtype == FZ_STORE_BF16) return mlp_launch<bf16>(d, nullptr, stream, &hd);
+  return fail(FZ_E_ARG, "fz_mlp_chain_head: act_dtype must be FZ_STORE_F32 or FZ_STORE_BF16");
+}
diff --git a/factorizer_amd/csrc/mlp_chain_wg.hip b/factorizer_amd/csrc/mlp_chain_wg.hip
--- a/factorizer_amd/csrc/mlp_chain_wg.hip
+++ b/factorizer_amd/csrc/mlp_chain_wg.hip
@@ -66,10 +66,11 @@
   acc = __builtin_amdgcn_mfma_f32_16x16x32_bf16(ah, bh, acc, 0, 0, 0);
 }
 
-template <typename AT, int HALVES = 1, int HALF = 0, bool BX = false, bool WGB = false>
+template <typename AT, int HALVES = 1, int HALF = 0, bool BX = false, bool WGB = false, bool HG = false>
 __global__ __launch_bounds__(256, 2) void gemm_chain_bwd_wg_kernel(GemmArgsT<AT> p, ChainArgsT<AT> c, int ntiles, float* wpart,
                                                                    float* glp) {
   static_assert(!WGB || (BX && HALVES == 1), "WGB: the one-launch split-bf16 form");
+  static_assert(!HG || (WGB && sizeof(AT) == 4), "HG: the one-launch form on fp32 storage");
   constexpr int NACC = 2, HB = 2, HID = 64 * HALVES, N1 = BX ? 3072 : 16 * HB * 64;
   constexpr int NTA = BxTerms<AT>::A, NTB = bx_terms_b<AT>(BXPRO_GELU);
   constexpr bool WGF = WGB && sizeof(AT) == 4;
@@ -83,7 +84,9 @@
   float* tB = As2 + N1;
   float* red = tB + 32;
   float* R = red + 256;
-  static_assert(2 * N1 + 32 + 256 + 4 * kWave == chain_wg_lds_floats(BX, WGB), "the launcher's dynamic LDS ends where this carve-up does");
+  float* sHW = R + 4 * kWave;
+  float* sDB = sHW + 128 + threadIdx.x;
+  static_assert(2 * N1 + 32 + 256 + 4 * kWave + (HG ? 128 + 6 * 256 + 64 : 0) == chain_wg_lds_floats(BX, WGB, HG), "the launcher's dynamic LDS ends where this carve-up does");
   const int lane = threadIdx.x & 63, wave = threadIdx.x >> 6;
   const int j = lane & 31, h = lane >> 5;
   const int l16 = lane & 15, k4 = lane >> 4;
@@ -111,7 +114,10 @@
       if (it < 256) {
         const int rb = (it >> 6) & 1, g = it >> 7;
 #pragma unroll
-        for (int e = 0; e < 8; ++e) wv[e] = weight_at(p, hoff + rb * 32 + (l & 31), 2 * (8 * g + e) + (l >> 5));
+        for (int e = 0; e < 8; ++e) {
+          const int s = 8 * g + e;
+          wv[e] = weight_at(p, hoff + rb * 32 + (l & 31), HG ? (s & 3) + 8 * (s >> 2) + 4 * (l >> 5) : 2 * s + (l >> 5));
+        }
         dst = reinterpret_cast<__bf16*>(As1) + ((g * HB + rb) * NTA * 64 + l) * 8;
       } else {
         const int g = (it - 256) >> 6;
@@ -155,6 +161,9 @@
   }
   }
   if (threadIdx.x < 32) tB[threadIdx.x] = p.lnb_g[threadIdx.x];
+  if constexpr (HG) {
+    if (threadIdx.x < 128) sHW[threadIdx.x] = (int)(threadIdx.x >> 5) < c.postM ? c.postW[threadIdx.x] : 0.f;
+  }
 
   f32x4 dW2[2][4], dW1[4][2];
 #pragma unroll
@@ -165,16 +174,33 @@
       for (int v = 0; v < 4; ++v) { dW2[a][b4][v] = 0.f; dW1[b4][a][v] = 0.f; }
   float db2[2] = {0.f, 0.f}, db1[4] = {0.f, 0.f, 0.f, 0.f};
   float gln = 0.f;
+  if constexpr (HG) {
+#pragma unroll
+    for (int i = 0; i < 6; ++i) sDB[i * 256] = 0.f;
+    if (threadIdx.x < 64) sDB[6 * 256] = 0.f;
+  }
 
   int tile = blockIdx.x;
-  float bv[16][NACC];
+  float bv[HG ? 1 : 16][NACC];
+  float hg[2][NACC];
   auto fetch_tile = [&](int t) {
     const int bt = t / tiles_per_sample;
     const int64_t ct = ((int64_t)(t % tiles_per_sample) * 4 + wave) * (32 * NACC) + NACC * j;
+    if constexpr (HG) {
+      const int64_t cl = ct < p.Ncol ? ct : 0;
+      const int hm = c.postM;
+      const AT* gb = p.x[0] + (int64_t)bt * hm * p.Ncol;
+#pragma unroll
+      for (int k = 0; k < 2; ++k) {
+        const int m = 2 * k + h < hm ? 2 * k + h : hm - 1;
+        vload<NACC>(gb + (int64_t)m * p.Ncol + cl, hg[k]);
+      }
+    } else {
     const unsigned lo = (unsigned)h * (unsigned)p.Ncol + (unsigned)(ct < p.Ncol ? ct : 0);
     const AT* xb = p.x[0] + (int64_t)bt * 32 * p.Ncol;
 #pragma unroll
     for (int s = 0; s < 16; ++s) vload<NACC>(xb + (int64_t)(2 * s) * p.Ncol + lo, bv[s]);
+    }
   };
   fetch_tile(tile);
   __syncthreads();
@@ -191,7 +217,19 @@
 
     constexpr bool ZSEL = HALVES == 2;
     auto zs = [&](float v) { return (ZSEL && !col_ok) ? 0.f : v; };
-    if (!ZSEL && __builtin_amdgcn_ballot_w64(!col_ok) != 0) {
+    f32x16 g2a[HG ? NACC : 1];
+    if constexpr (HG) {
+#pragma unroll
+      for (int k = 0; k < 2; ++k) { hg[k][0] = col_ok ? hg[k][0] : 0.f; hg[k][1] = col_ok ? hg[k][1] : 0.f; }
+      const float hw0 = sHW[lane], hw1 = sHW[64 + lane];
+#pragma unroll
+      for (int q = 0; q < NACC; ++q) {
+#pragma unroll
+        for (int r = 0; r < 16; ++r) g2a[q][r] = 0.f;
+        g2a[q] = __builtin_amdgcn_mfma_f32_32x32x2f32(hw0, hg[0][q], g2a[q], 0, 0, 0);
+        g2a[q] = __builtin_amdgcn_mfma_f32_32x32x2f32(hw1, hg[1][q], g2a[q], 0, 0, 0);
+      }
+    } else if (!ZSEL && __builtin_amdgcn_ballot_w64(!col_ok) != 0) {
 #pragma unroll
       for (int s = 0; s < 16; ++s) { bv[s][0] = col_ok ? bv[s][0] : 0.f; bv[s][1] = col_ok ? bv[s][1] : 0.f; }
     }
@@ -236,7 +274,10 @@
         for (int q = 0; q < NACC; ++q) {
           float x8[8];
 #pragma unroll
-          for (int e = 0; e < 8; ++e) x8[e] = bv[8 * g + e][q];
+          for (int e = 0; e < 8; ++e) {
+            if constexpr (HG) x8[e] = g2a[q][8 * g + e];
+            else x8[e] = bv[8 * g + e][q];
+          }
           bx_split<NTB>(x8, bop[q]);
         }
         if constexpr (WGB) {
@@ -246,8 +287,9 @@
             const int s = 8 * g + e;
             const wg2 ph = {bop[0][0][e], bop[1][0][e]};
             const wg2 pl = {bop[0][NTB >= 2 ? 1 : 0][e], bop[1][NTB >= 2 ? 1 : 0][e]};
-            *reinterpret_cast<wg2*>(PL + wop[s & 3] + s * 256) = ph;
-            *reinterpret_cast<wg2*>(PL + kGL + wop[s & 3] + s * 256) = pl;
+            const unsigned at = HG ? wac[s & 3] + (s & 3) * 128 + (s >> 2) * 1024 : wop[s & 3] + s * 256;
+            *reinterpret_cast<wg2*>(PL + at) = ph;
+            *reinterpret_cast<wg2*>(PL + kGL + at) = pl;
           }
         }
 #pragma unroll
@@ -311,9 +353,11 @@
           wg_mfma3(dW2[0][g8], a0h, a0l, bh, bl);
           wg_mfma3(dW2[1][g8], a1h, a1l, bh, bl);
           if (g8 == 0) {
+            if constexpr (HG) { db2[0] = sDB[0]; db2[1] = sDB[256]; }
             db2[0] = wg_sum8(a0h, a0l, db2[0]);
             db2[1] = wg_sum8(a1h, a1l, db2[1]);
             asm volatile("" : "+v"(db2[0]), "+v"(db2[1]));
+            if constexpr (HG) { sDB[0] = db2[0]; sDB[256] = db2[1]; }
           }
           __builtin_amdgcn_sched_barrier(0);
         }
@@ -431,8 +475,10 @@
           const bx8 b1l = *reinterpret_cast<const bx8*>(PL + kGL + 2048 + rd[ks]);
           wg_mfma3(dW1[g8][0], ah, al, b0h, b0l);
           wg_mfma3(dW1[g8][1], ah, al, b1h, b1l);
+          if constexpr (HG) db1[g8] = sDB[(2 + g8) * 256];
           db1[g8] = wg_sum8(ah, al, db1[g8]);
           asm volatile("" : "+v"(db1[g8]));
+          if constexpr (HG) sDB[(2 + g8) * 256] = db1[g8];
           __builtin_amdgcn_sched_barrier(0);
         }
       } else {
@@ -592,13 +638,21 @@
     __syncthreads();
     if (threadIdx.x < 64) {
       const int e = threadIdx.x;
+      if constexpr (HG) gln = sDB[6 * 256];
       gln += (red[e] + red[64 + e]) + (red[128 + e] + red[192 + e]);
+      if constexpr (HG) sDB[6 * 256] = gln;
     }
     __syncthreads();
   }
 
   float* row = wpart + (int64_t)blockIdx.x * kWgRow;
   __syncthreads();
+  if constexpr (HG) {
+    db2[0] = sDB[0]; db2[1] = sDB[256];
+#pragma unroll
+    for (int cb = 0; cb < 4; ++cb) db1[cb] = sDB[(2 + cb) * 256];
+    if (threadIdx.x < 64) gln = sDB[6 * 256];
+  }
 #pragma unroll
   for (int a = 0; a < 2; ++a)
 #pragma unroll
@@ -662,7 +716,7 @@
 namespace fz {
 
 template <typename AT>
-int chain_wg_launch(const fz_mlp_desc* d, const GemmArgsT<AT>& a, const ChainArgsT<AT>& c, fz_stream_t stream) {
+int chain_wg_launch(const fz_mlp_desc* d, const GemmArgsT<AT>& a, const ChainArgsT<AT>& c, fz_stream_t stream, bool head) {
   hipStream_t st = (hipStream_t)stream;
   const int ntiles = (int)fz_mlp_partials(d->B, d->V), rows = fz_mlp_wgrad_rows(d->B, d->V);
   const int halves = d->H / 64;
@@ -673,9 +727,16 @@
       : wgb       ? gemm_chain_bwd_wg_kernel<AT, 1, 0, true, true>
                   : (bx ? gemm_chain_bwd_wg_kernel<AT, 1, 0, true> : gemm_chain_bwd_wg_kernel<AT, 1, 0, false>),
       bx ? gemm_chain_bwd_wg_kernel<AT, 2, 1, true> : gemm_chain_bwd_wg_kernel<AT, 2, 1, false>};
+  if (head) {
+    if constexpr (sizeof(AT) == 4) {
+      if (!wgb) return fail(FZ_E_UNSUPPORTED, "fz_mlp_chain_head: needs the one-launch split-bf16 form");
+      kern[0] = gemm_chain_bwd_wg_kernel<AT, 1, 0, true, true, true>;
+    } else
+      return fail(FZ_E_UNSUPPORTED, "fz_mlp_chain_head: fp32 storage only");
+  }
   for (int half = 0; half < halves; ++half) {
     float* wp = (float*)d->wpart + (int64_t)half * rows * kWgRow;
-    int rc = launch_lds(kern[half], dim3((unsigned)rows), dim3(256), chain_wg_lds_floats(bx, wgb), st, a, c, ntiles, wp,
+    int rc = launch_lds(kern[half], dim3((unsigned)rows), dim3(256), chain_wg_lds_floats(bx, wgb, head), st, a, c, ntiles, wp,
                         halves == 2 ? d->glp : (float*)nullptr);
     if (rc != FZ_OK) return rc;
     FinishJob fj = finish_job(FK_CHAIN_WG, kWgRow / 16);
@@ -686,7 +747,7 @@
   }
   return FZ_OK;
 }
-template int chain_wg_launch<float>(const fz_mlp_desc*, const GemmArgsT<float>&, const ChainArgsT<float>&, fz_stream_t);
-template int chain_wg_launch<bf16>(const fz_mlp_desc*, const GemmArgsT<bf16>&, const ChainArgsT<bf16>&, fz_stream_t);
-
-}
+template int chain_wg_launch<float>(const fz_mlp_desc*, const GemmArgsT<float>&, const ChainArgsT<float>&, fz_stream_t, bool);
+template int chain_wg_launch<bf16>(const fz_mlp_desc*, const GemmArgsT<bf16>&, const ChainArgsT<bf16>&, fz_stream_t, bool);
+
+}
diff --git a/factorizer_amd/pointwise.py b/factorizer_amd/pointwise.py
--- a/factorizer_amd/pointwise.py
+++ b/factorizer_amd/pointwise.py
@@ -312,7 +312,7 @@
     return _mlp_chain_ok(C, Hd, V) and C == 32 and Hd in (64, 128) and os.environ.get("FZ_MLP_FUSED_WGRAD", "1") != "0"
 
 
-def _mlp_bwd_chain_wgrad(g2, z1, w12, w22, x1, st, ln_w, ln_b):
+def _mlp_bwd_chain_wgrad(g2, z1, w12, w22, x1, st, ln_w, ln_b, head=None):
     B, C = x1.shape[:2]
     V = _vox(x1)
     Hd = w12.shape[0]
@@ -329,10 +329,15 @@
     d.gln, d.wpart, d.glp = gpar.data_ptr(), wpart.data_ptr(), _p(glp)
     d.gw1, d.gb1, d.gw2, d.gb2 = gw1.data_ptr(), gb1.data_ptr(), gw2.data_ptr(), gb2.data_ptr()
     nbytes = x1.element_size() * (3 * x1.numel() + z1.numel()) + (0 if Hd == 64 else x1.element_size() * 2 * x1.numel() + 8 * x1.numel())
+    if head is not None:
+        gl, hw2 = head
+        nbytes += x1.element_size() * (gl.numel() - x1.numel())
+        launch = lambda: N.lib().fz_mlp_chain_head(ctypes.byref(d), gl.data_ptr(), hw2.data_ptr(), hw2.shape[0], N.stream_ptr(x1))
+    else:
+        launch = lambda: N.lib().fz_mlp_chain(ctypes.byref(d), N.stream_ptr(x1))
     with torch.cuda.device(dev), _finish_scope(wpart, gpar, gw1, gb1, gw2, gb2):
-        rc = Fn._timed(f"mlp_chain_bwd_wgrad_{C}" + ("" if Hd == 64 else f"x{Hd}"), nbytes,
-                       lambda: N.lib().fz_mlp_chain(ctypes.byref(d), N.stream_ptr(x1)), cols=B * V, flops=8 * B * V * C * Hd)
-        N.check(rc, "fz_mlp_chain")
+        rc = Fn._timed(f"mlp_chain_bwd_wgrad_{C}" + ("" if Hd == 64 else f"x{Hd}"), nbytes, launch, cols=B * V, flops=8 * B * V * C * Hd)
+        N.check(rc, "fz_mlp_chain" if head is None else "fz_mlp_chain_head")
     return gx1, gpar[:32], gpar[32:], gw1, gb1, gw2, gb2
 
 
@@ -616,7 +621,7 @@
     return gw, gb
 
 
-def _head_bwd(gy, z, w2):
+def _head_bwd(gy, z, w2, reduce=True):
     B, C = z.shape[:2]
     V = _vox(z)
     M = w2.shape[0]
@@ -629,8 +634,24 @@
                        lambda: lib.fz_head_bwd(gy.data_ptr(), z.data_ptr(), w2.data_ptr(), gz.data_ptr(), part.data_ptr(),
                                                B, M, C, V, N.act_dtype(z), N.stream_ptr(z)), cols=B * V)
         N.check(rc, "fz_head_bwd")
+        gw, gb = _head_rows_reduce(part, rows, w2, M, z) if reduce else (None, None)
+    return gz, gw, gb
+
+
+def _head_wgrad(gy, z, w2):
+    B, C = z.shape[:2]
+    V = _vox(z)
+    M = w2.shape[0]
+    lib = N.lib()
+    rows = lib.fz_head_bwd_rows()
+    part = torch.empty(lib.fz_head_bwd_workspace_bytes() // 4, dtype=torch.float32, device=z.device)
+    with torch.cuda.device(z.device):
+        rc = Fn._timed(f"head_wgrad_{C}->{M}", z.element_size() * (gy.numel() + z.numel()),
+                       lambda: lib.fz_head_wgrad(gy.data_ptr(), z.data_ptr(), part.data_ptr(), B, M, C, V, N.act_dtype(z),
+                                                 N.stream_ptr(z)), cols=B * V)
+        N.check(rc, "fz_head_wgrad")
         gw, gb = _head_rows_reduce(part, rows, w2, M, z)
-    return gz, gw, gb
+    return gw, gb
 
 
 class LNLinearFn(torch.autograd.Function):
@@ -1191,6 +1212,7 @@
 _UPCAT_FWD = os.environ.get("FZ_UPCAT_FWD", "1") != "0"
 _UPCAT_BWD = os.environ.get("FZ_UPCAT_BWD", "1") != "0"
 _HEAD_BWD = os.environ.get("FZ_HEAD_BWD", "1") != "0"
+_HEAD_G2 = os.environ.get("FZ_HEAD_G2", "1") != "0"
 
 
 def up_cat_linear(skip, deep, w_t, b_t, w_ad, b_ad=None, pro=None):
@@ -1342,9 +1364,14 @@
         x, st1, t, a, x1, st2, z1, m, n1w, n1b, win2, u0c, v0c, wout2, n2w, n2b, w12, w22, *bits = ctx.saved_tensors
         cfg = ctx.cfg
         drop = cfg.get("drop")
-        if g2 is None:
+        head_g2 = None
+        link = getattr(ctx, "head_g2", None)
+        if link is not None and link.standin is not None:
+            g2, head_g2 = link.claim(g2)
+        if g2 is None and head_g2 is None:
             g2 = torch.zeros_like(x)
-        g2 = g2.contiguous()
+        if g2 is not None:
+            g2 = g2.contiguous()
         B, C = x.shape[:2]
         V = _vox(x)
         Hd = w12.shape[0]
@@ -1371,7 +1398,11 @@
         chain = _mlp_chain_ok(C, Hd, V) and drop is None
         (p0, p1, p2), (m0, m1, m2) = drop or (0, 0, 0), bits
         if drop is None and _mlp_wgrad_fused_ok(C, Hd, V):
-            gx1, gg2, gbt2, gw1, gb1, gw2, gb2 = _mlp_bwd_chain_wgrad(g2, z1, w12, w22, x1, st2, n2w, n2b)
+            if head_g2 is not None:
+                gx1, gg2, gbt2, gw1, gb1, gw2, gb2 = _mlp_bwd_chain_wgrad(None, z1, w12, w22, x1, st2, n2w, n2b, head=head_g2)
+                head_g2 = None
+            else:
+                gx1, gg2, gbt2, gw1, gb1, gw2, gb2 = _mlp_bwd_chain_wgrad(g2, z1, w12, w22, x1, st2, n2w, n2b)
         else:
             gelu = ACT["gelu" if m1 is None else "none"]
             gf = Fn.dropout_apply(N.DROP_RES, m2, p2, g2) if m2 is not None else g2
@@ -1478,6 +1509,40 @@
     return getattr(_head_fusion, "slot", None)
 
 
+def _head_g2_ok(C, Hd, V, M, x, drop):
+    return (_HEAD_G2 and drop is None and _mlp_wgrad_fused_ok(C, Hd, V)
+            and bool(N.lib().fz_mlp_head_g2_supported(C, Hd, V, 2, N.products(), M, N.act_dtype(x))))
+
+
+class HeadG2Link:
+
+    def __init__(self, like=None):
+        self.standin = self.gl = self.w2 = self.y = None
+        self.zero = None if like is None else torch.zeros(1, dtype=like.dtype, device=like.device)
+
+    def offer(self, gl, w2, y):
+        self.gl, self.w2, self.y = gl, w2, y
+        if self.zero is None:
+            self.zero = torch.zeros(1, dtype=y.dtype, device=y.device)
+        self.standin = self.zero.expand(y.shape)
+        return self.standin
+
+    def claim(self, g):
+        s, gl, w2, y = self.standin, self.gl, self.w2, self.y
+        self.standin = self.gl = self.w2 = self.y = None
+        if g is not None and g.data_ptr() == s.data_ptr() and g.shape == s.shape and not any(g.stride()):
+            return None, (gl, w2)
+        gz = _head_bwd(gl, y, w2, reduce=False)[0]
+        return (gz if g is None else gz.add_(g)), None
+
+
+def link_head_g2(y, logits, C, Hd, V, M, drop):
+    fb, fh = y.grad_fn, logits.grad_fn
+    if fb is None or fh is None or not _head_g2_ok(C, Hd, V, M, y, drop):
+        return
+    fb.head_g2 = fh.head_g2 = HeadG2Link(y)
+
+
 def block_head_fusable(C, Hd, V, head_w, x):
     return (C == 32 and _outproj_mlp_ok(C, Hd, V) and head_w is not None and head_w.dtype == torch.float32 and head_w.numel() == head_w.shape[0] * C
             and 1 <= head_w.shape[0] <= 4 and x.is_cuda and _HEAD_BWD)
@@ -1505,7 +1570,12 @@
         gl = gl.contiguous()
         if gl.dtype != y.dtype:
             gl = gl.to(y.dtype)
-        gy, gw, gb = _head_bwd(gl, y, w2)
+        link = getattr(ctx, "head_g2", None)
+        if link is not None and not getattr(y, "_backward_hooks", None) and not y.retains_grad:
+            gw, gb = _head_wgrad(gl, y, w2)
+            gy = link.offer(gl, w2, y)
+        else:
+            gy, gw, gb = _head_bwd(gl, y, w2)
         return gy, gw.reshape(ctx.wshape), (gb if ctx.has_bias else None), None
 
 
diff --git a/include/factorizer_hip.h b/include/factorizer_hip.h
--- a/include/factorizer_hip.h
+++ b/include/factorizer_hip.h
@@ -246,6 +246,7 @@
 int64_t fz_head_bwd_workspace_bytes(void);
 int fz_head_bwd(const void* gy, const void* x, const float* w, void* gx, float* part, int B, int M, int C, int64_t V,
                 int act_dtype, fz_stream_t stream);
+int fz_head_wgrad(const void* gy, const void* x, float* part, int B, int M, int C, int64_t V, int act_dtype, fz_stream_t stream);
 int fz_head_fwd(const void* x, const float* w, const float* bias, void* y, int B, int M, int C, int64_t V, int act_dtype,
                 fz_stream_t stream);
 
@@ -280,6 +281,8 @@
 int64_t fz_mlp_wgrad_workspace_bytes(int B, int64_t V);
 int fz_mlp_chain(const fz_mlp_desc* desc, fz_stream_t stream);
 int fz_mlp_chain_drop(const fz_mlp_desc* desc, const fz_mlp_dropout* drop, fz_stream_t stream);
+int fz_mlp_head_g2_supported(int C, int H, int64_t V, int mode, int products, int M, int act_dtype);
+int fz_mlp_chain_head(const fz_mlp_desc* desc, const void* gy, const float* head_w, int M, fz_stream_t stream);
 
 #define FZ_QL_PLAIN 0
 #define FZ_QL_S2D 1
```
